# zhoubin-me/agent0

Measured on AMD Instinct MI355X. Metric: env-frames/sec (learner FPS: transitions collected and saved to replay per second with the learner running, pre-frameskip), higher is better.
Workload: dtype f32

## Files before the change

agent0_amd/csrc/conv1_wgrad.hip:

```cpp
#include "a0_internal.h"

#include <cstdint>

typedef __bf16 a0w_bf16x8 __attribute__((ext_vector_type(8)));
typedef uint32_t a0w_u32x4 __attribute__((ext_vector_type(4)));
typedef float a0w_acc4 __attribute__((ext_vector_type(4)));

constexpr int A0W_THREADS = 512;
constexpr int A0W_XP_ROW = 24, A0W_XP_PLANE = 21 * 24;
constexpr int A0W_XP_ELEMS = 64 * A0W_XP_PLANE;
constexpr int A0W_T_PITCH = 488, A0W_T_TERM = 32 * A0W_T_PITCH;
constexpr int A0W_GROUPS = 60;
constexpr int A0W_STEPS = 15;

struct a0_c1w_args {
    const uint8_t* frames; const int* slot; long long sample_stride; int chan_off;
    const float* d1;
    float* slabs;
    int B;
};

A0_D uint32_t a0w_trunc(float f) { return __float_as_uint(f) >> 16; }
A0_D float a0w_up(uint32_t h) { return __uint_as_float(h << 16); }

__global__ __launch_bounds__(A0W_THREADS) void a0_conv1_wgrad_fused_kernel(a0_c1w_args P) {
    extern __shared__ __attribute__((aligned(16))) unsigned char smem[];
    uint16_t* Xp = (uint16_t*)smem;
    uint16_t* T = Xp + A0W_XP_ELEMS;
    const int tid = threadIdx.x, lane = tid & 63;
    const int wave = __builtin_amdgcn_readfirstlane(tid >> 6);
    const int q = lane >> 4, r16 = lane & 15;
    for (int i = tid; i < (A0W_XP_ELEMS + 3 * A0W_T_TERM) / 2; i += A0W_THREADS) ((uint32_t*)smem)[i] = 0u;
    int bbase[2], bshift[2];
#pragma unroll
    for (int t = 0; t < 2; ++t) {
        const int k = (2 * wave + t) * 16 + r16;
        const int c = k >> 6, kh = (k >> 3) & 7, kw = k & 7;
        const int plane = (c * 4 + (kh & 3)) * 4 + (kw & 3);
        bbase[t] = plane * A0W_XP_PLANE + (kh >> 2) * A0W_XP_ROW;
        bshift[t] = 2 * (kw >> 2);
    }
    a0w_acc4 acc[2][2];
#pragma unroll
    for (int i = 0; i < 2; ++i)
#pragma unroll
        for (int t = 0; t < 2; ++t) acc[i][t] = a0w_acc4{0.f, 0.f, 0.f, 0.f};
    float bsum = 0.f;
    __syncthreads();
    constexpr int NDW = 4 * 84 * 21, TR = (NDW + A0W_THREADS - 1) / A0W_THREADS;
    constexpr int GT = (A0W_GROUPS + A0W_THREADS / 32 - 1) / (A0W_THREADS / 32);
    uint32_t w[TR];
    float v[GT][8];
    auto load_raw = [&](int b) {
        const long long s = P.slot ? (long long)P.slot[b] : (long long)b;
        const uint32_t* src = (const uint32_t*)(P.frames + s * P.sample_stride + P.chan_off);
#pragma unroll
        for (int j = 0; j < TR; ++j) { const int i = tid + j * A0W_THREADS; w[j] = src[i < NDW ? i : NDW - 1]; }
        const float* g = P.d1 + (long long)b * 400 * 32 + (tid & 31);
#pragma unroll
        for (int t = 0; t < GT; ++t) {
            int G = (tid >> 5) + t * (A0W_THREADS / 32);
            G = G < A0W_GROUPS ? G : A0W_GROUPS - 1;
            const int oh = G / 3, ow0 = 8 * (G - 3 * oh);
#pragma unroll
            for (int j = 0; j < 8; ++j) { const int m = oh * 20 + ow0 + j; v[t][j] = g[(m < 400 ? m : 399) * 32]; }
        }
    };
    load_raw(blockIdx.x);
    for (int b = blockIdx.x; b < P.B; b += gridDim.x) {
#pragma unroll
        for (int j = 0; j < TR; ++j) {
            int i = tid + j * A0W_THREADS;
            i = i < NDW ? i : NDW - 1;
            const int c = i / (84 * 21), rem = i - c * (84 * 21), y = rem / 21, xc = rem - y * 21;
            uint16_t* d = Xp + ((c * 4 + (y & 3)) * 4) * A0W_XP_PLANE + (y >> 2) * A0W_XP_ROW + xc;
            d[0 * A0W_XP_PLANE] = (uint16_t)(__float_as_uint((float)(w[j] & 0xffu)) >> 16);
            d[1 * A0W_XP_PLANE] = (uint16_t)(__float_as_uint((float)((w[j] >> 8) & 0xffu)) >> 16);
            d[2 * A0W_XP_PLANE] = (uint16_t)(__float_as_uint((float)((w[j] >> 16) & 0xffu)) >> 16);
            d[3 * A0W_XP_PLANE] = (uint16_t)(__float_as_uint((float)(w[j] >> 24)) >> 16);
        }
        {
            const int n = tid & 31;
#pragma unroll
            for (int t = 0; t < GT; ++t) {
                const int G = (tid >> 5) + t * (A0W_THREADS / 32);
                if (G < A0W_GROUPS) {
                    const int oh = G / 3, ow0 = 8 * (G - 3 * oh);
                    uint32_t t0[4], t1[4], t2[4];
#pragma unroll
                    for (int j = 0; j < 8; j += 2) {
                        uint32_t h[2], m[2], l[2];
#pragma unroll
                        for (int e = 0; e < 2; ++e) {
                            const float x = (ow0 + j + e < 20) ? v[t][j + e] : 0.f;
                            bsum += x;
                            h[e] = a0w_trunc(x);
                            const float r1 = x - a0w_up(h[e]);
                            m[e] = a0w_trunc(r1);
                            l[e] = a0w_trunc(r1 - a0w_up(m[e]));
                        }
                        t0[j >> 1] = h[0] | (h[1] << 16); t1[j >> 1] = m[0] | (m[1] << 16); t2[j >> 1] = l[0] | (l[1] << 16);
                    }
                    uint16_t* d = T + n * A0W_T_PITCH + 8 * G;
                    *(uint4*)(d) = uint4{t0[0], t0[1], t0[2], t0[3]};
                    *(uint4*)(d + A0W_T_TERM) = uint4{t1[0], t1[1], t1[2], t1[3]};
                    *(uint4*)(d + 2 * A0W_T_TERM) = uint4{t2[0], t2[1], t2[2], t2[3]};
                }
            }
        }
        __syncthreads();
        if (b + (int)gridDim.x < P.B) load_raw(b + gridDim.x);
        {
            const uint16_t* ap = T + r16 * A0W_T_PITCH + 8 * q;
            const uint16_t* bp0 = Xp + bbase[0] + 8 * q;
            const uint16_t* bp1 = Xp + bbase[1] + 8 * q;
#pragma unroll 3
            for (int st = 0; st < A0W_STEPS; ++st) {
                a0w_u32x4 a[2][3], bf[2];
#pragma unroll
                for (int i = 0; i < 2; ++i)
#pragma unroll
                    for (int s3 = 0; s3 < 3; ++s3) {
                        const uint4 x = *(const uint4*)(ap + s3 * A0W_T_TERM + i * 16 * A0W_T_PITCH + 32 * st);
                        a[i][s3] = a0w_u32x4{x.x, x.y, x.z, x.w};
                    }
#pragma unroll
                for (int t = 0; t < 2; ++t) {
                    const uint16_t* bp = (t == 0 ? bp0 : bp1) + 32 * st;
                    const uint4 lo = *(const uint4*)bp;
                    const uint32_t hi = *(const uint32_t*)(bp + 8);
                    const int sh = bshift[t];
                    bf[t] = a0w_u32x4{__builtin_amdgcn_alignbyte(lo.y, lo.x, sh), __builtin_amdgcn_alignbyte(lo.z, lo.y, sh),
                                      __builtin_amdgcn_alignbyte(lo.w, lo.z, sh), __builtin_amdgcn_alignbyte(hi, lo.w, sh)};
                }
#pragma unroll
                for (int s3 = 0; s3 < 3; ++s3)
#pragma unroll
                    for (int i = 0; i < 2; ++i)
#pragma unroll
                        for (int t = 0; t < 2; ++t)
                            acc[i][t] = __builtin_amdgcn_mfma_f32_16x16x32_bf16(__builtin_bit_cast(a0w_bf16x8, a[i][s3]), __builtin_bit_cast(a0w_bf16x8, bf[t]), acc[i][t], 0, 0, 0);
            }
        }
        __syncthreads();
    }
    float* out = P.slabs + (long long)blockIdx.x * (32 * 256 + 32);
#pragma unroll
    for (int i = 0; i < 2; ++i)
#pragma unroll
        for (int t = 0; t < 2; ++t) {
            const int k = (2 * wave + t) * 16 + r16;
#pragma unroll
            for (int r = 0; r < 4; ++r) out[(i * 16 + 4 * q + r) * 256 + k] = acc[i][t][r] / 255.0f;
        }
    float* red = (float*)smem;
    red[tid] = bsum;
    __syncthreads();
    if (tid < 32) {
        float s = 0.f;
#pragma unroll
        for (int j = 0; j < A0W_THREADS / 32; ++j) s += red[j * 32 + tid];
        out[32 * 256 + tid] = s;
    }
}

int a0_conv1_wgrad_fused_launch(const a0_frames_arg* f, int C, int H, int W, int B, const float* d1, float* slabs, hipStream_t st) {
    if (C != 4 || H != 84 || W != 84 || B < 1 || (f->sample_stride & 3) || (f->chan_off & 3) || (((uintptr_t)f->frames) & 3)) return 0;
    a0_c1w_args P;
    P.frames = f->frames; P.slot = f->slot; P.sample_stride = f->sample_stride; P.chan_off = f->chan_off;
    P.d1 = d1; P.slabs = slabs; P.B = B;
    const int grid = B < 256 ? B : 256;
    const size_t lds = (size_t)(A0W_XP_ELEMS + 3 * A0W_T_TERM) * 2;
    static bool configured = false;
    if (!configured) {
        A0_HIP_THROW(hipFuncSetAttribute((const void*)a0_conv1_wgrad_fused_kernel, hipFuncAttributeMaxDynamicSharedMemorySize, (int)lds));
        configured = true;
    }
    hipLaunchKernelGGL(a0_conv1_wgrad_fused_kernel, dim3(grid), dim3(A0W_THREADS), lds, st, P);
    A0_HIP_THROW(hipGetLastError());
    return grid;
}
```

agent0_amd/csrc/encoder_fused.hip:

```cpp
#include "a0_internal.h"
#include "net_tables.h"
#include "operands.h"

#include <cstdlib>
#include <type_traits>

#ifndef A0_X9_MAXORD
#define A0_X9_MAXORD 4
#endif
typedef float a0_acc4 __attribute__((ext_vector_type(4)));

struct a0_fused_args {
    const uint8_t* frames; const int* slot; long long sample_stride; int chan_off;
    const float *wt1, *wt2, *wt3;
    const float *wx2, *wx3;
    const float *b1, *b2, *b3;
    float *act1, *act2, *act3;
    int B;
    int C, H, W, H1, W1, H2, W2, H3, W3;
    int off_act1, off_act2, off_end;
    int rp1, rp2;
};

#ifndef A0_FUSED_WAVES_D
#define A0_FUSED_WAVES_D 8
#endif
constexpr int A0_FUSED_WAVES = A0_FUSED_WAVES_D;
constexpr int A0_WMG1 = A0_FUSED_WAVES / 2;
constexpr int A0_FUSED_THREADS = 64 * A0_FUSED_WAVES;
constexpr int A0_P1 = 33;
constexpr int A0_P2 = 66;

struct AF2 {
    const float* act; int RP1, W2;
    A0_D int row(int m) const { const int oh = m / W2, ow = m - oh * W2; return (2 * oh) * RP1 + 2 * ow * A0_P1; }
    A0_D int chunk_off(int c) const { const int cell = c >> 1; return (cell >> 2) * RP1 + (cell & 3) * A0_P1 + 16 * (c & 1); }
    A0_D int step_off(int s) const { return 4 * s; }
    typedef float Raw;
    A0_D Raw load(int addr) const { return act[addr]; }
    static A0_D float value(Raw r) { return r; }
};
struct AF3 {
    const float* act; int RP2, W3;
    A0_D int row(int m) const { const int oh = m / W3, ow = m - oh * W3; return oh * RP2 + ow * A0_P2; }
    A0_D int chunk_off(int c) const { const int cell = c >> 2; return (cell / 3) * RP2 + (cell % 3) * A0_P2 + 16 * (c & 3); }
    A0_D int step_off(int s) const { return 4 * s; }
    typedef float Raw;
    A0_D Raw load(int addr) const { return act[addr]; }
    static A0_D float value(Raw r) { return r; }
};

template <int N, int WN, int R>
struct a0_wring {
    static constexpr int NBW = N / 16 / WN;
    a0_f4 v[R][NBW];
    const float* base;
    const float* p;
    int nch, left;
    A0_D void init(const float* wp, int K) {
        const int lane = threadIdx.x & 63, wave = __builtin_amdgcn_readfirstlane(threadIdx.x >> 6);
        const int n = (wave % WN) * (NBW * 16) + (lane & 15), q = lane >> 4;
        base = wp + (n * 4 + q) * 4;
        nch = K >> 4;
    }
    A0_D void fill(int slot) {
#pragma unroll
        for (int j = 0; j < NBW; ++j) v[slot][j] = *(const a0_f4*)(p + j * 256);
        const bool more = left > 1;
        p += more ? N * 16 : 0;
        left -= more ? 1 : 0;
    }
    A0_D void prologue() {
        p = base; left = nch;
#pragma unroll
        for (int u = 0; u < R; ++u) fill(u);
    }
};
A0_D float a0_f4_get(const a0_f4& v, int j) { return j == 0 ? v.x : j == 1 ? v.y : j == 2 ? v.z : v.w; }

template <int OWC>
struct EpiFwd {
    static constexpr bool PER_ELEM = false;
    static constexpr bool TR = false;
    const float* bias; float* lds; int pitch, rp, ow; float* glb; int N;
    A0_D float pre_col(int n) const { return bias[n]; }
    A0_D float pre_elem(int, int) const { return 0.f; }
    A0_D void emit(int m, int n, float acc, float pre) const {
        float v = acc + pre;
        v = (v < 0.f) ? 0.f : v;
        if (lds) {
            const int w_ = OWC > 0 ? OWC : ow, oh = m / w_;
            lds[oh * rp + (m - oh * w_) * pitch + n] = v;
        }
        if (glb) glb[(unsigned)(m * N + n)] = v;
    }
    static constexpr bool ROW4 = OWC > 0 && (OWC % 4) == 0;
    A0_D void emit4(int m0, int n, const a0_acc4& acc, float pre) const {
        constexpr int OWD = OWC > 0 ? OWC : 1;
        const int oh = m0 / OWD, ow0 = m0 - oh * OWD;
        float* l = lds ? lds + oh * rp + ow0 * pitch + n : nullptr;
        const unsigned go = (unsigned)(m0 * N + n);
#pragma unroll
        for (int r = 0; r < 4; ++r) {
            float v = acc[r] + pre;
            v = (v < 0.f) ? 0.f : v;
            if (l) l[r * pitch] = v;
            if (glb) glb[go + (unsigned)(r * N)] = v;
        }
    }
};

template <int N, int WN, int MBW, class EPI>
struct a0_pre {
    static constexpr int NBW = N / 16 / WN, WMG = A0_FUSED_WAVES / WN;
    float pc[NBW][EPI::TR ? 4 : 1], pe[EPI::PER_ELEM ? MBW : 1][NBW][4];
    A0_D void load(const EPI& epi, int M) {
        const int lane = threadIdx.x & 63, wave = __builtin_amdgcn_readfirstlane(threadIdx.x >> 6);
        const int wn = wave % WN, wmg = wave / WN, q = lane >> 4, r16 = lane & 15;
#pragma unroll
        for (int j = 0; j < NBW; ++j) {
            if constexpr (EPI::TR) {
                const int n0 = (wn * NBW + j) * 16 + 4 * q;
#pragma unroll
                for (int r = 0; r < 4; ++r) pc[j][r] = epi.pre_col(n0 + r);
                if constexpr (EPI::PER_ELEM) {
#pragma unroll
                    for (int i = 0; i < MBW; ++i) {
                        const int m = (wmg + i * WMG) * 16 + r16;
                        const a0_f4 v = epi.pre_elem4(m < M ? m : M - 1, n0);
                        pe[i][j][0] = v.x; pe[i][j][1] = v.y; pe[i][j][2] = v.z; pe[i][j][3] = v.w;
                    }
                }
            } else {
                const int n = (wn * NBW + j) * 16 + r16;
                pc[j][0] = epi.pre_col(n);
                if constexpr (EPI::PER_ELEM) {
#pragma unroll
                    for (int i = 0; i < MBW; ++i)
#pragma unroll
                        for (int r = 0; r < 4; ++r) {
                            const int m = (wmg + i * WMG) * 16 + 4 * q + r;
                            pe[i][j][r] = epi.pre_elem(m < M ? m : M - 1, n);
                        }
                }
            }
        }
    }
};

template <int N, int WN, int MBW, int PD, int R, int MBWP, class AF, class EPI, class Between>
A0_D void a0_conv_stage(const AF& af, int M, int K, a0_wring<N, WN, R>& ring, const EPI& epi, const a0_pre<N, WN, MBWP, EPI>& pre, Between&& between) {
    static_assert(MBWP >= MBW, "prefetched epilogue values cover the wave's blocks");
    constexpr int NB = N / 16, NBW = NB / WN, WMG = A0_FUSED_WAVES / WN, RS = PD + 1;
// ... 198 lines not shown
        p += more ? stride : 0;
        left -= more ? 1 : 0;
    }
    A0_D void prologue() {
        p = base; left = nst;
#pragma unroll
        for (int u = 0; u < R; ++u) fill(u);
    }
};
template <int TERM>
struct AF2X {
    static constexpr int term = TERM;
    const uint16_t* planes; int RP, W2, P;
    A0_D int row(int m) const { const int oh = m / W2, ow = m - oh * W2; return (2 * oh) * RP + 2 * ow * P; }
    A0_D int step_off(int st) const { return (st >> 2) * RP + (st & 3) * P; }
};
template <int TERM>
struct AF3X {
    static constexpr int term = TERM;
    const uint16_t* planes; int RP, W3, P;
    A0_D int row(int m) const { const int oh = m / W3, ow = m - oh * W3; return oh * RP + ow * P; }
    A0_D int step_off(int st) const { const int tap = st >> 1; return (tap / 3) * RP + (tap % 3) * P + 32 * (st & 1); }
};
A0_D void a0_split4(const float (&v)[4], uint2& hi, uint2& mid, uint2& lo) {
    uint32_t h[4], m[4], l[4];
#pragma unroll
    for (int r = 0; r < 4; ++r) {
        h[r] = __float_as_uint(v[r]);
        const float r1 = v[r] - __uint_as_float(h[r] & 0xffff0000u);
        m[r] = __float_as_uint(r1);
        l[r] = __float_as_uint(r1 - __uint_as_float(m[r] & 0xffff0000u));
    }
    hi = uint2{__builtin_amdgcn_perm(h[1], h[0], 0x07060302u), __builtin_amdgcn_perm(h[3], h[2], 0x07060302u)};
    mid = uint2{__builtin_amdgcn_perm(m[1], m[0], 0x07060302u), __builtin_amdgcn_perm(m[3], m[2], 0x07060302u)};
    lo = uint2{__builtin_amdgcn_perm(l[1], l[0], 0x07060302u), __builtin_amdgcn_perm(l[3], l[2], 0x07060302u)};
}
template <int OWC, int P, int RP, int term>
struct EpiFwdX {
    static constexpr bool PER_ELEM = false;
    static constexpr bool ROW4 = false;
    static constexpr bool TR = true;
    static_assert(OWC > 0 && (P % 4) == 0 && (RP % 4) == 0 && (term % 4) == 0, "output width known at compile time; 8-byte aligned plane writes");
    const float* bias; uint16_t* planes; float* glb; int N;
    A0_D float pre_col(int) const { return 0.f; }
    A0_D void emit_n4(int m, int n0, const a0_acc4& acc, const float*) const {
        const a0_f4 bv = *(const a0_f4*)(bias + n0);
        float v[4] = {acc[0] + bv.x, acc[1] + bv.y, acc[2] + bv.z, acc[3] + bv.w};
#pragma unroll
        for (int r = 0; r < 4; ++r) v[r] = (v[r] < 0.f) ? 0.f : v[r];
        if (glb) *(a0_f4*)(glb + (unsigned)(m * N + n0)) = a0_f4{v[0], v[1], v[2], v[3]};
        uint2 hi, mid, lo;
        a0_split4(v, hi, mid, lo);
        const int oh = m / OWC;
        uint16_t* d = planes + oh * RP + (m - oh * OWC) * P + n0;
        *(uint2*)d = hi; *(uint2*)(d + term) = mid; *(uint2*)(d + 2 * term) = lo;
    }
};
struct EpiFwdT {
    static constexpr bool PER_ELEM = false;
    static constexpr bool ROW4 = false;
    static constexpr bool TR = true;
    const float* bias; float* glb; int N;
    A0_D float pre_col(int) const { return 0.f; }
    A0_D void emit_n4(int m, int n0, const a0_acc4& acc, const float*) const {
        const a0_f4 bv = *(const a0_f4*)(bias + n0);
        float v[4] = {acc[0] + bv.x, acc[1] + bv.y, acc[2] + bv.z, acc[3] + bv.w};
#pragma unroll
        for (int r = 0; r < 4; ++r) v[r] = (v[r] < 0.f) ? 0.f : v[r];
        *(a0_f4*)(glb + (unsigned)(m * N + n0)) = a0_f4{v[0], v[1], v[2], v[3]};
    }
};

template <int ORD, int N, int WN, int MBW, int R, int MBWP, class AFX, class EPI, class Between>
A0_D void a0_conv_stage_x9(const AFX& af, int M, a0_wring9<N, WN, R>& ring, const EPI& epi, const a0_pre<N, WN, MBWP, EPI>& pre, Between&& between) {
    constexpr int NB = N / 16, NBW = NB / WN, WMG = A0_FUSED_WAVES / WN;
    static_assert(NBW >= 1 && (R % 2) == 0 && MBWP >= MBW, "tile shape");
    const int tid = threadIdx.x, lane = tid & 63;
    const int wave = __builtin_amdgcn_readfirstlane(tid >> 6);
    const int wn = wave % WN, wmg = wave / WN;
    const int q = lane >> 4, r16 = lane & 15;
    const int MB = (M + 15) >> 4, NST = ring.nst;
    int rows[MBW];
#pragma unroll
    for (int i = 0; i < MBW; ++i) {
        const int m = (wmg + i * WMG) * 16 + r16;
        rows[i] = af.row(m < M ? m : 0) + 8 * q;
    }
    a0_acc4 acc[MBW][NBW];
#pragma unroll
    for (int i = 0; i < MBW; ++i)
#pragma unroll
        for (int j = 0; j < NBW; ++j) acc[i][j] = a0_acc4{0.f, 0.f, 0.f, 0.f};
    uint4 a[2][MBW][3];
    auto fetch = [&](int slot, int off) {
#pragma unroll
        for (int i = 0; i < MBW; ++i)
#pragma unroll
            for (int t = 0; t < 3; ++t) a[slot][i][t] = *(const uint4*)(af.planes + rows[i] + off + t * AFX::term);
    };
    fetch(0, af.step_off(0));
    __builtin_amdgcn_s_waitcnt(0x0F70);
#pragma unroll 1
    for (int tb = 0; tb < NST; tb += R) {
#pragma unroll
        for (int u = 0; u < R; ++u) {
            const int nxt = tb + u + 1;
            fetch((u + 1) & 1, af.step_off(nxt < NST ? nxt : NST - 1));
            __builtin_amdgcn_sched_barrier(0);
#pragma unroll
            for (int ta = 0; ta < 3; ++ta)
#pragma unroll
                for (int tw = 0; tw < 3; ++tw)
#pragma unroll
                    for (int i = 0; i < MBW; ++i)
#pragma unroll
                        for (int jn = 0; jn < NBW; ++jn) {
                            if (ta + tw > ORD) continue;
                            const a0_u32x4 av = {a[u & 1][i][ta].x, a[u & 1][i][ta].y, a[u & 1][i][ta].z, a[u & 1][i][ta].w};
                            const a0_u32x4 bv = {ring.v[u][jn][tw].x, ring.v[u][jn][tw].y, ring.v[u][jn][tw].z, ring.v[u][jn][tw].w};
                            if constexpr (EPI::TR) acc[i][jn] = __builtin_amdgcn_mfma_f32_16x16x32_bf16(__builtin_bit_cast(a0_bf16x8, bv), __builtin_bit_cast(a0_bf16x8, av), acc[i][jn], 0, 0, 0);
                            else acc[i][jn] = __builtin_amdgcn_mfma_f32_16x16x32_bf16(__builtin_bit_cast(a0_bf16x8, av), __builtin_bit_cast(a0_bf16x8, bv), acc[i][jn], 0, 0, 0);
                        }
            __builtin_amdgcn_sched_barrier(0);
            ring.fill(u);
            __builtin_amdgcn_sched_barrier(0);
        }
    }
    between();
#pragma unroll
    for (int i = 0; i < MBW; ++i) {
        const int mb = wmg + i * WMG;
        if (mb < MB) {
            if constexpr (EPI::TR) {
                const int m = mb * 16 + r16;
                if (m < M) {
#pragma unroll
                    for (int j = 0; j < NBW; ++j) epi.emit_n4(m, (wn * NBW + j) * 16 + 4 * q, acc[i][j], EPI::PER_ELEM ? pre.pe[EPI::PER_ELEM ? i : 0][j] : pre.pc[j]);
                }
            } else {
#pragma unroll
                for (int j = 0; j < NBW; ++j) {
                    const int n = (wn * NBW + j) * 16 + r16;
#pragma unroll
                    for (int r = 0; r < 4; ++r) {
                        const int m = mb * 16 + 4 * q + r;
                        if (m < M) epi.emit(m, n, acc[i][j][r], EPI::PER_ELEM ? pre.pe[EPI::PER_ELEM ? i : 0][j][r] : pre.pc[j][0]);
                    }
                }
            }
        }
    }
    __syncthreads();
}
template <int ORD, int N, int WN, int MBT, int R, int LR, class AFX, class EPI, class Between>
A0_D void a0_conv_stage_x9k(const AFX& af, int M, a0_wring9<N, WN, R, A0_FUSED_WAVES / WN>& ring, const EPI& epi, float* xch0, float* xch1, Between&& between) {
    constexpr int WK = A0_FUSED_WAVES / WN, HB0 = (MBT + 1) / 2, HB1 = MBT / 2;
    static_assert(WK == 2 && N == 16 * WN && HB1 >= 1 && EPI::TR && LR >= 1 && LR <= 16, "tile shape");
    const int tid = threadIdx.x, lane = tid & 63;
    const int wave = __builtin_amdgcn_readfirstlane(tid >> 6);
    const int wn = wave % WN, wk = wave / WN;
    const int q = lane >> 4, r16 = lane & 15;
    const int MB = (M + 15) >> 4, NSTW = ring.nst;
    int rows[MBT];
#pragma unroll
    for (int i = 0; i < MBT; ++i) {
        const int m = i * 16 + r16;
        rows[i] = af.row(m < M ? m : 0) + 8 * q;
    }
    a0_acc4 acc[MBT];
#pragma unroll
    for (int i = 0; i < MBT; ++i) acc[i] = a0_acc4{0.f, 0.f, 0.f, 0.f};
    uint4 a[2][HB0][3];
    auto fetch = [&](int slot, int h, int off) {
#pragma unroll
        for (int i = 0; i < HB0; ++i)
            if (h * HB0 + i < MBT) {
#pragma unroll
                for (int t = 0; t < 3; ++t) a[slot][i][t] = *(const uint4*)(af.planes + rows[h * HB0 + i] + off + t * AFX::term);
            }
    };
    fetch(0, 0, af.step_off(wk));
    __builtin_amdgcn_s_waitcnt(0x0F70);
#pragma unroll 1
    for (int tb = 0; tb < NSTW; tb += R) {
#pragma unroll
        for (int u = 0; u < R; ++u) {
            const int st = wk + WK * (tb + u);
            const int off = af.step_off(st), offn = af.step_off(tb + u + 1 < NSTW ? st + WK : st);
#pragma unroll
            for (int h = 0; h < 2; ++h) {
                if (h == 0) fetch(1, 1, off);
                else fetch(0, 0, offn);
                __builtin_amdgcn_sched_barrier(0);
#pragma unroll
                for (int ta = 0; ta < 3; ++ta)
#pragma unroll
                    for (int tw = 0; tw < 3; ++tw)
#pragma unroll
                        for (int i = 0; i < HB0; ++i) {
                            if (ta + tw > ORD || h * HB0 + i >= MBT) continue;
                            const a0_u32x4 av = {a[h][i][ta].x, a[h][i][ta].y, a[h][i][ta].z, a[h][i][ta].w};
                            const a0_u32x4 bv = {ring.v[u][0][tw].x, ring.v[u][0][tw].y, ring.v[u][0][tw].z, ring.v[u][0][tw].w};
                            acc[h * HB0 + i] = __builtin_amdgcn_mfma_f32_16x16x32_bf16(__builtin_bit_cast(a0_bf16x8, bv), __builtin_bit_cast(a0_bf16x8, av), acc[h * HB0 + i], 0, 0, 0);
                        }
                __builtin_amdgcn_sched_barrier(0);
            }
            ring.fill(u);
            __builtin_amdgcn_sched_barrier(0);
        }
    }
    between();
    a0_acc4* x0 = (a0_acc4*)xch0;
    a0_acc4* x1 = (a0_acc4*)xch1;
    constexpr int P1 = (HB1 - 1) * 64 + 4 * LR;
    const int last = q * LR + r16;
    const int n0 = wn * 16 + 4 * q;
    float pe[EPI::PER_ELEM ? HB0 : 1][4];
    auto send = [&](auto mine) {
        constexpr int H = decltype(mine)::value;
        if constexpr (EPI::PER_ELEM) {
#pragma unroll
            for (int i = 0; i < (H == 0 ? HB0 : HB1); ++i) {
                const int m = (H * HB0 + i) * 16 + r16;
                const a0_f4 v = epi.pre_elem4(m < M ? m : M - 1, n0);
                pe[i][0] = v.x; pe[i][1] = v.y; pe[i][2] = v.z; pe[i][3] = v.w;
            }
        }
        if constexpr (H == 1) {
#pragma unroll
            for (int i = 0; i < HB0; ++i) x0[(wn * HB0 + i) * 64 + lane] = acc[i];
        } else {
#pragma unroll
            for (int i = 0; i < HB1; ++i) {
                if (i < HB1 - 1) x1[wn * P1 + i * 64 + lane] = acc[HB0 + i];
                else if (r16 < LR) x1[wn * P1 + (HB1 - 1) * 64 + last] = acc[HB0 + i];
            }
        }
    };
    auto recv = [&](auto mine) {
        constexpr int H = decltype(mine)::value;
#pragma unroll
        for (int i = 0; i < (H == 0 ? HB0 : HB1); ++i) {
            const int mb = H * HB0 + i;
            const int m = mb * 16 + r16;
            if constexpr (H == 0) acc[mb] += x0[(wn * HB0 + i) * 64 + lane];
            else {
                if (i < HB1 - 1) acc[mb] += x1[wn * P1 + i * 64 + lane];
                else if (r16 < LR) acc[mb] += x1[wn * P1 + (HB1 - 1) * 64 + last];
            }
            if (mb < MB && m < M) epi.emit_n4(m, n0, acc[mb], EPI::PER_ELEM ? pe[EPI::PER_ELEM ? i : 0] : nullptr);
        }
    };
    if (wk == 0) send(std::integral_constant<int, 0>{});
    else send(std::integral_constant<int, 1>{});
    __syncthreads();
    if (wk == 0) recv(std::integral_constant<int, 0>{});
    else recv(std::integral_constant<int, 1>{});
    __syncthreads();
}
constexpr int A0_P1X = 40, A0_P2X = 80;
#ifndef A0_PADS
#define A0_PADS 1
#endif
constexpr int A0_RP1X = 20 * A0_P1X + (A0_PADS ? 8 : 0);
constexpr int A0_RP2X = 9 * A0_P2X + (A0_PADS ? 96 : 0);
#ifndef A0_RX2_D
#define A0_RX2_D 4
#endif
#ifndef A0_RX3_D
#define A0_RX3_D 6
#endif
[[maybe_unused]] constexpr int A0_RX2 = A0_RX2_D, A0_RX3 = A0_RX3_D;
#ifndef A0_KSPLIT_D
#define A0_KSPLIT_D 1
#endif
#ifndef A0_KSPLIT
#define A0_KSPLIT 1
#endif
#ifndef A0_WNX
#define A0_WNX 4
#endif

constexpr int A0_R1 = 4, A0_R2 = 4, A0_R3 = 6;

#ifndef A0_FUSED_MINWAVES
#define A0_FUSED_MINWAVES 1
#endif
template <int MBW1, int MBW2, int MBW3, int WC, bool X9, bool LOOP = false, int ORD = 4>
__global__ __launch_bounds__(A0_FUSED_THREADS, A0_FUSED_MINWAVES) void a0_encoder_fused_kernel(a0_fused_args P);

constexpr int A0_X9_BIAS_OFF = 2 * 4 * 84 * 84 + 3 * 20 * A0_RP1X * 2;
#ifndef A0_RK2_D
#define A0_RK2_D 2
#endif
#ifndef A0_RK3_D
#define A0_RK3_D 3
#endif
constexpr int A0_RK2 = A0_RK2_D, A0_RK3 = A0_RK3_D;
constexpr int A0_X9_XCH0 = 3 * 9 * A0_RP2X * 2;
constexpr int A0_X9_XCH1 = A0_X9_BIAS_OFF + 160 * 4;
static_assert(A0_X9_XCH0 + 4 * 3 * 1024 <= 2 * 4 * 84 * 84, "conv2 exchange region 0 fits into the image");
constexpr int A0_X9_LDS_BYTES = A0_X9_XCH1 + (A0_KSPLIT ? 4 * (2 * 64 + 4) * 16 : 0);
static_assert(A0_X9_LDS_BYTES <= 160 * 1024, "LDS");
#if A0_KSPLIT
typedef a0_wring9<64, 4, A0_RK2, 2> a0_ring2_t;
typedef a0_wring9<64, 4, A0_RK3, 2> a0_ring3_t;
#else
typedef a0_wring9<64, A0_WNX, A0_RX2> a0_ring2_t;
typedef a0_wring9<64, A0_WNX, A0_RX3> a0_ring3_t;
#endif
template <int ORD, int MBW2, int MBW3, bool LOOP>
A0_D void a0_x9_conv23(const a0_fused_args& P, int b, unsigned char* smem, float* bias_lds, a0_wring1<A0_R1>& ring1, a0_ring2_t& ring2, a0_ring3_t& ring3) {
    const int obs_bytes = P.C * P.H * P.W;
    const int M2 = P.H2 * P.W2, M3 = P.H3 * P.W3;
    uint16_t* a1p = (uint16_t*)(smem + 2 * obs_bytes);
    constexpr int term1 = 20 * A0_RP1X, term2 = 9 * A0_RP2X;
    uint16_t* a2p = (uint16_t*)smem;
    typedef EpiFwdX<9, A0_P2X, A0_RP2X, term2> E2X;
    constexpr int WNX = A0_WNX, WMGX = A0_FUSED_WAVES / WNX;
    constexpr int MBW2X = (6 + WMGX - 1) / WMGX, MBW3X = (4 + WMGX - 1) / WMGX;
    static_assert(MBW2X <= MBW2 * 2 && MBW3X <= MBW3 * 2, "84x84 geometry");
#if !A0_KSPLIT
    a0_pre<64, WNX, MBW2X, E2X> pre2;
    a0_pre<64, WNX, MBW3X, EpiFwdT> pre3;
#endif
    (void)a1p; (void)term1;
    {
        const AF2X<term1> f2{a1p, A0_RP1X, P.W2, A0_P1X};
        const E2X e2{bias_lds + 32, a2p, P.act2 ? P.act2 + (long long)b * M2 * 64 : nullptr, 64};
#if A0_KSPLIT
        const AF3X<term2> f3k{a2p, A0_RP2X, P.W3, A0_P2X};
        const EpiFwdT e3k{bias_lds + 96, P.act3 + (long long)b * M3 * 64, 64};
        a0_conv_stage_x9k<ORD, 64, 4, 6, A0_RK2, 1>(f2, M2, ring2, e2, (float*)(smem + A0_X9_XCH0), (float*)(smem + A0_X9_XCH1), [&] { ring3.prologue(); });
        a0_conv_stage_x9k<ORD, 64, 4, 4, A0_RK3, 16>(f3k, M3, ring3, e3k, (float*)a1p, (float*)a1p + 4 * 2 * 256, [&] { if (LOOP) ring1.prologue(); });
#else
        const int wmgx = __builtin_amdgcn_readfirstlane(threadIdx.x >> 6) / WNX;
        constexpr bool uneven2 = MBW2X > 1 && MBW2X * WMGX > 6, uneven3 = MBW3X > 1 && MBW3X * WMGX > 4;
        if (uneven2 && wmgx + (MBW2X - 1) * WMGX >= 6)
            a0_conv_stage_x9<ORD, 64, WNX, (MBW2X > 1 ? MBW2X - 1 : 1), A0_RX2>(f2, M2, ring2, e2, pre2, [&] { ring3.prologue(); });
        else
            a0_conv_stage_x9<ORD, 64, WNX, MBW2X, A0_RX2>(f2, M2, ring2, e2, pre2, [&] { ring3.prologue(); });
        const AF3X<term2> f3{a2p, A0_RP2X, P.W3, A0_P2X};
        const EpiFwdT e3{bias_lds + 96, P.act3 + (long long)b * M3 * 64, 64};
        if (uneven3 && wmgx + (MBW3X - 1) * WMGX >= 4)
            a0_conv_stage_x9<ORD, 64, WNX, (MBW3X > 1 ? MBW3X - 1 : 1), A0_RX3>(f3, M3, ring3, e3, pre3, [&] { if (LOOP) ring1.prologue(); });
        else
            a0_conv_stage_x9<ORD, 64, WNX, MBW3X, A0_RX3>(f3, M3, ring3, e3, pre3, [&] { if (LOOP) ring1.prologue(); });
#endif
    }
}

template <int ORD, int MBW1, int MBW2, int MBW3, bool LOOP>
A0_D void a0_encoder_fused_x9_body(const a0_fused_args& P, int bid, int nblk) {
    extern __shared__ __attribute__((aligned(16))) unsigned char smem[];
    uint16_t* img = (uint16_t*)smem;
    const int obs_bytes = P.C * P.H * P.W;
    const int M1 = P.H1 * P.W1;
    uint16_t* a1p = (uint16_t*)(smem + 2 * obs_bytes);
    constexpr int term1 = 20 * A0_RP1X;
    typedef EpiFwdX<20, A0_P1X, A0_RP1X, term1> E1X;
    constexpr int WNX = A0_WNX, WMGX = A0_FUSED_WAVES / WNX;
    constexpr int MBW2X = (6 + WMGX - 1) / WMGX, MBW3X = (4 + WMGX - 1) / WMGX;
    static_assert(MBW2X <= MBW2 * 2 && MBW3X <= MBW3 * 2, "84x84 geometry");
    a0_wring1<A0_R1> ring1;
#if A0_KSPLIT
    static_assert(WNX == 4 && A0_FUSED_WAVES == 8, "N-stationary stages: four waves along N, two along K");
#endif
    a0_ring2_t ring2;
    a0_ring3_t ring3;
    ring1.init(P.wt1, P.C);
    ring2.init(P.wx2, 512);
    ring3.init(P.wx3, 576);
    ring1.prologue();
    constexpr int MBW1X = (25 + A0_WMG1 - 1) / A0_WMG1;
    static_assert(A0_FUSED_WAVES != 8 || MBW1X == MBW1, "84x84 geometry");
    a0_pre<32, 2, MBW1X, E1X> pre1;
    float* bias_lds = (float*)(smem + A0_X9_BIAS_OFF);
    if (threadIdx.x < 160) bias_lds[threadIdx.x] = threadIdx.x < 32 ? P.b1[threadIdx.x] : threadIdx.x < 96 ? P.b2[threadIdx.x - 32] : P.b3[threadIdx.x - 96];
    for (int b = bid; b < P.B; b += nblk) {
        const long long s = P.slot ? (long long)P.slot[b] : (long long)b;
        const uint4* src = (const uint4*)(P.frames + s * P.sample_stride + P.chan_off);
        constexpr int TRIPS = 4;
        const int n16 = obs_bytes >> 4;
        for (int i0 = threadIdx.x; i0 < n16; i0 += TRIPS * A0_FUSED_THREADS) {
            uint4 v[TRIPS];
#pragma unroll
            for (int j = 0; j < TRIPS; ++j) {
                const int i = i0 + j * A0_FUSED_THREADS;
                v[j] = src[i < n16 ? i : n16 - 1];
            }
#pragma unroll
            for (int j = 0; j < TRIPS; ++j) {
                int i = i0 + j * A0_FUSED_THREADS;
                i = i < n16 ? i : n16 - 1;
                const uint32_t w[4] = {v[j].x, v[j].y, v[j].z, v[j].w};
                uint32_t o[8];
#pragma unroll
                for (int k = 0; k < 4; ++k) {
                    const uint32_t f0 = __float_as_uint((float)(w[k] & 0xffu)), f1 = __float_as_uint((float)((w[k] >> 8) & 0xffu));
                    const uint32_t f2 = __float_as_uint((float)((w[k] >> 16) & 0xffu)), f3 = __float_as_uint((float)(w[k] >> 24));
                    o[2 * k] = __builtin_amdgcn_perm(f1, f0, 0x07060302u);
                    o[2 * k + 1] = __builtin_amdgcn_perm(f3, f2, 0x07060302u);
                }
                ((uint4*)img)[2 * i] = uint4{o[0], o[1], o[2], o[3]};
                ((uint4*)img)[2 * i + 1] = uint4{o[4], o[5], o[6], o[7]};
            }
        }
        __syncthreads();
        const E1X e1{bias_lds, a1p, P.act1 ? P.act1 + (long long)b * M1 * 32 : nullptr, 32};
        const int wmg1 = __builtin_amdgcn_readfirstlane(threadIdx.x >> 6) / 2;
        if (MBW1X > 1 && wmg1 + (MBW1X - 1) * A0_WMG1 >= ((M1 + 15) >> 4))
// ... 405 lines not shown
    const float *d3, *act1, *act2;
    float *d2, *d1;
    const float *wd3, *wd2;
    int B;
};
constexpr int A0_RPDA = 11 * A0_P2X + (A0_PADS ? 96 : 0), A0_RPDB = 11 * A0_P2X + (A0_PADS ? 48 : 0);
constexpr int A0_DTERMA = 11 * A0_RPDA, A0_DTERMB = 11 * A0_RPDB;
struct AFD3X {
    static constexpr int term = A0_DTERMA;
    const uint16_t* planes;
    A0_D int row(int m) const { const int oh = m / 9, ow = m - oh * 9; return oh * A0_RPDA + ow * A0_P2X; }
    A0_D int step_off(int st) const { const int tap = st >> 1; return (tap / 3) * A0_RPDA + (tap % 3) * A0_P2X + 32 * (st & 1); }
};
struct AFD2X {
    static constexpr int term = A0_DTERMB;
    const uint16_t* planes;
    A0_D int row(int m) const { const int oh = m / 10, ow = m - oh * 10; return oh * A0_RPDB + ow * A0_P2X; }
    A0_D int step_off(int st) const { const int cell = st >> 1; return (cell >> 1) * A0_RPDB + (cell & 1) * A0_P2X + 32 * (st & 1); }
};
struct EpiBwd3X {
    static constexpr bool PER_ELEM = true;
    static constexpr bool ROW4 = false;
    static constexpr bool TR = true;
    const float* mask; float* dst; uint16_t* planes;
    A0_D float pre_col(int) const { return 0.f; }
    A0_D a0_f4 pre_elem4(int m, int n0) const { return *(const a0_f4*)(mask + (unsigned)(m * 64 + n0)); }
    A0_D void emit_n4(int m, int n0, const a0_acc4& acc, const float* pre) const {
        float v[4];
#pragma unroll
        for (int r = 0; r < 4; ++r) v[r] = pre[r] > 0.f ? acc[r] : 0.f;
        *(a0_f4*)(dst + (unsigned)(m * 64 + n0)) = a0_f4{v[0], v[1], v[2], v[3]};
        uint2 hi, mid, lo;
        a0_split4(v, hi, mid, lo);
        const int oh = m / 9, ow = m - oh * 9;
        uint16_t* d = planes + (oh + 1) * A0_RPDB + (ow + 1) * A0_P2X + n0;
        *(uint2*)d = hi; *(uint2*)(d + A0_DTERMB) = mid; *(uint2*)(d + 2 * A0_DTERMB) = lo;
    }
};
static_assert((A0_RPDB % 4) == 0 && (A0_DTERMB % 4) == 0 && (A0_P2X % 4) == 0, "8-byte aligned plane writes");
template <int OW, int S>
struct EpiBwdT {
    static constexpr bool PER_ELEM = true;
    static constexpr bool ROW4 = false;
    static constexpr bool TR = true;
    const float* mask; float* dst; int Wfull, ph, pw, N;
    A0_D unsigned gi(int m, int n) const { const int oh = m / OW, ow = m - oh * OW; return (unsigned)(((oh * S + ph) * Wfull + ow * S + pw) * N + n); }
    A0_D float pre_col(int) const { return 0.f; }
    A0_D a0_f4 pre_elem4(int m, int n0) const { return *(const a0_f4*)(mask + gi(m, n0)); }
    A0_D void emit_n4(int m, int n0, const a0_acc4& acc, const float* pre) const {
        *(a0_f4*)(dst + gi(m, n0)) = a0_f4{pre[0] > 0.f ? acc[0] : 0.f, pre[1] > 0.f ? acc[1] : 0.f, pre[2] > 0.f ? acc[2] : 0.f, pre[3] > 0.f ? acc[3] : 0.f};
    }
};
struct EpiBwdPair {
    static constexpr bool PER_ELEM = true;
    static constexpr bool ROW4 = false;
    static constexpr bool TR = true;
    const float* mask; float* dst; int p0;
    A0_D unsigned gi(int m, int n0) const {
        const int p = p0 + (n0 >> 5), oh = m / 10, ow = m - oh * 10;
        return (unsigned)(((oh * 2 + (p >> 1)) * 20 + ow * 2 + (p & 1)) * 32 + (n0 & 31));
    }
    A0_D float pre_col(int) const { return 0.f; }
    A0_D a0_f4 pre_elem4(int m, int n0) const { return *(const a0_f4*)(mask + gi(m, n0)); }
    A0_D void emit_n4(int m, int n0, const a0_acc4& acc, const float* pre) const {
        *(a0_f4*)(dst + gi(m, n0)) = a0_f4{pre[0] > 0.f ? acc[0] : 0.f, pre[1] > 0.f ? acc[1] : 0.f, pre[2] > 0.f ? acc[2] : 0.f, pre[3] > 0.f ? acc[3] : 0.f};
    }
};
constexpr int A0_RXD3 = 6, A0_RXD2 = 4;

template <int ORD>
__global__ __launch_bounds__(A0_FUSED_THREADS) void a0_encoder_dgrad_fused_x9_kernel(a0_dgrad_args P) {
    extern __shared__ __attribute__((aligned(16))) unsigned char smem[];
    uint16_t* plA = (uint16_t*)smem;
    uint16_t* plB = plA + 3 * A0_DTERMA;
    for (int i = threadIdx.x; i < 3 * (A0_DTERMA + A0_DTERMB) / 2; i += A0_FUSED_THREADS) ((uint32_t*)smem)[i] = 0u;
#if A0_KSPLIT_D
    float* const xch0 = (float*)(smem + 3 * (A0_DTERMA + A0_DTERMB) * 2);
    float* const xch1 = xch0 + 4 * 4 * 256;
    {
        const int lane = threadIdx.x & 63, wave = __builtin_amdgcn_readfirstlane(threadIdx.x >> 6), wn = wave & 3, wk = wave >> 2;
        a0_wring9<64, 4, 3, 2> ring3;
        a0_wring9<64, 4, 2, 2> ringq[2];
        ring3.init(P.wd3, 576);
        ring3.prologue();
        const uint4* const wq = (const uint4*)P.wd2 + (((wn & 1) * 16 + (lane & 15)) * 4 + (lane >> 4)) * 3 + (wn >> 1) * 3072 + wk * 384;
        __syncthreads();
        for (int b = blockIdx.x; b < P.B; b += gridDim.x) {
            const a0_f4* src = (const a0_f4*)(P.d3 + (long long)b * 49 * 64);
            for (int i = threadIdx.x; i < 49 * 16; i += A0_FUSED_THREADS) {
                const a0_f4 v = src[i];
                const int pos = i >> 4, c4 = (i & 15) * 4, h = pos / 7, w = pos - h * 7;
                const float x[4] = {v.x, v.y, v.z, v.w};
                uint2 hi, mid, lo;
                a0_split4(x, hi, mid, lo);
                uint16_t* d = plA + (h + 2) * A0_RPDA + (w + 2) * A0_P2X + c4;
                *(uint2*)(d) = hi; *(uint2*)(d + A0_DTERMA) = mid; *(uint2*)(d + 2 * A0_DTERMA) = lo;
            }
            __syncthreads();
            const AFD3X f3{plA};
            const AFD2X f2{plB};
            const EpiBwd3X e3{P.act2 + (long long)b * 81 * 64, P.d2 + (long long)b * 81 * 64, plB};
            const EpiBwdPair e2a{P.act1 + (long long)b * 400 * 32, P.d1 + (long long)b * 400 * 32, 0};
            const EpiBwdPair e2b{P.act1 + (long long)b * 400 * 32, P.d1 + (long long)b * 400 * 32, 2};
            a0_conv_stage_x9k<ORD, 64, 4, 6, 3, 1>(f3, 81, ring3, e3, xch0, xch1, [&] { ringq[0].init_at(wq, 4, 768); ringq[0].prologue(); });
            a0_conv_stage_x9k<ORD, 64, 4, 7, 2, 4>(f2, 100, ringq[0], e2a, xch0, xch1, [&] { ringq[1].init_at(wq + 2 * 3072, 4, 768); ringq[1].prologue(); });
            a0_conv_stage_x9k<ORD, 64, 4, 7, 2, 4>(f2, 100, ringq[1], e2b, xch0, xch1, [&] { ring3.prologue(); });
        }
        return;
    }
#endif
    a0_wring9<64, 4, A0_RXD3> ring3;
    a0_wring9<32, 2, A0_RXD2> ringp[2];
    ring3.init(P.wd3, 576);
    ring3.prologue();
    typedef EpiBwd3X E3;
    typedef EpiBwdT<10, 2> E2;
    a0_pre<64, 4, 3, E3> pre3;
    a0_pre<32, 2, 2, E2> prep[2];
    auto epi3 = [&](int b) { return E3{P.act2 + (long long)b * 81 * 64, P.d2 + (long long)b * 81 * 64, plB}; };
    auto epi2 = [&](int b, int ph, int pw) { return E2{P.act1 + (long long)b * 400 * 32, P.d1 + (long long)b * 400 * 32, 20, ph, pw, 32}; };
    if ((int)blockIdx.x < P.B) pre3.load(epi3(blockIdx.x), 81);
    __syncthreads();
    for (int b = blockIdx.x; b < P.B; b += gridDim.x) {
        const a0_f4* src = (const a0_f4*)(P.d3 + (long long)b * 49 * 64);
        for (int i = threadIdx.x; i < 49 * 16; i += A0_FUSED_THREADS) {
            const a0_f4 v = src[i];
            const int pos = i >> 4, c4 = (i & 15) * 4, h = pos / 7, w = pos - h * 7;
            const float x[4] = {v.x, v.y, v.z, v.w};
            uint32_t hh[4], mm[4], ll[4];
#pragma unroll
            for (int e = 0; e < 4; ++e) {
                hh[e] = __float_as_uint(x[e]);
                const float r1 = x[e] - __uint_as_float(hh[e] & 0xffff0000u);
                mm[e] = __float_as_uint(r1);
                ll[e] = __float_as_uint(r1 - __uint_as_float(mm[e] & 0xffff0000u));
            }
            uint16_t* d = plA + (h + 2) * A0_RPDA + (w + 2) * A0_P2X + c4;
            *(uint2*)(d) = uint2{__builtin_amdgcn_perm(hh[1], hh[0], 0x07060302u), __builtin_amdgcn_perm(hh[3], hh[2], 0x07060302u)};
            *(uint2*)(d + A0_DTERMA) = uint2{__builtin_amdgcn_perm(mm[1], mm[0], 0x07060302u), __builtin_amdgcn_perm(mm[3], mm[2], 0x07060302u)};
            *(uint2*)(d + 2 * A0_DTERMA) = uint2{__builtin_amdgcn_perm(ll[1], ll[0], 0x07060302u), __builtin_amdgcn_perm(ll[3], ll[2], 0x07060302u)};
        }
        __syncthreads();
        const AFD3X f3{plA};
        const AFD2X f2{plB};
        const int bn = b + gridDim.x < P.B ? b + gridDim.x : b;
        a0_conv_stage_x9<ORD, 64, 4, 3, A0_RXD3>(f3, 81, ring3, epi3(b), pre3, [&] { ringp[0].init(P.wd2, 256); ringp[0].prologue(); prep[0].load(epi2(b, 0, 0), 100); });
        a0_conv_stage_x9<ORD, 32, 2, 2, A0_RXD2>(f2, 100, ringp[0], epi2(b, 0, 0), prep[0], [&] { ringp[1].init(P.wd2 + 1 * 12288, 256); ringp[1].prologue(); prep[1].load(epi2(b, 0, 1), 100); });
        a0_conv_stage_x9<ORD, 32, 2, 2, A0_RXD2>(f2, 100, ringp[1], epi2(b, 0, 1), prep[1], [&] { ringp[0].init(P.wd2 + 2 * 12288, 256); ringp[0].prologue(); prep[0].load(epi2(b, 1, 0), 100); });
        a0_conv_stage_x9<ORD, 32, 2, 2, A0_RXD2>(f2, 100, ringp[0], epi2(b, 1, 0), prep[0], [&] { ringp[1].init(P.wd2 + 3 * 12288, 256); ringp[1].prologue(); prep[1].load(epi2(b, 1, 1), 100); });
        a0_conv_stage_x9<ORD, 32, 2, 2, A0_RXD2>(f2, 100, ringp[1], epi2(b, 1, 1), prep[1], [&] { ring3.prologue(); pre3.load(epi3(bn), 81); });
    }
}

A0_HD uint32_t a0_bf16_trunc(float f) { return __float_as_uint(f) >> 16; }
A0_HD float a0_bf16_up(uint32_t h) { return __uint_as_float(h << 16); }
__global__ void a0_conv_wt_kernel(const float* __restrict__ w1, const float* __restrict__ w2, const float* __restrict__ w3, float* __restrict__ wt, int K1,
                                  float* __restrict__ wt2, const int* __restrict__ state, int* __restrict__ commit) {
    const bool mirror = wt2 != nullptr && state[4] != 0;
    if (commit != nullptr && blockIdx.x == 0 && threadIdx.x == 0) { commit[1] = commit[5]; commit[0] = 0; }
    const int n1 = 48 * K1, n2 = 64 * 512, n3 = 64 * 576, n4 = 64 * 576, n5 = 4 * 32 * 256;
    const int n6 = 96 * 512, n7 = 96 * 576;
    int i = blockIdx.x * blockDim.x + threadIdx.x;
    float* dst = wt + i;
    if (i < n1) {
        const int pair = i & 3, f = i >> 2, s = f % 3, q = (f / 3) & 3, n = (f / 12) & 31, t = f / 384;
        uint32_t out = 0;
        for (int h = 0; h < 2; ++h) {
            const int k = 32 * t + 8 * q + 2 * pair + h;
            const float w = w1[n * K1 + k] / 255.0f;
            const uint32_t hi = a0_bf16_trunc(w);
            const float r1 = w - a0_bf16_up(hi);
            const uint32_t mid = a0_bf16_trunc(r1);
            const float r2 = r1 - a0_bf16_up(mid);
            const uint32_t lo = a0_bf16_trunc(r2);
            out |= (s == 0 ? hi : s == 1 ? mid : lo) << (16 * h);
        }
        { *(uint32_t*)dst = out; if (mirror) *(uint32_t*)(wt2 + (dst - wt)) = out; }
        return;
    }
    i -= n1;
    {
        const int j6 = i - (n2 + n3 + n4 + n5);
        if (j6 >= 0) {
            if (j6 >= n6 + n7) {
                const int j8 = j6 - (n6 + n7), n8 = 96 * 576, n9p = 48 * 256;
                if (j8 >= n8 + 4 * n9p) return;
                const bool d2 = j8 >= n8;
                const int phase = d2 ? (j8 - n8) / n9p : 0;
                const int jj = d2 ? (j8 - n8) - phase * n9p : j8, N = d2 ? 32 : 64;
                const int pair = jj & 3, f = jj >> 2, s = f % 3, q = (f / 3) & 3, n = (f / 12) % N, t = f / (12 * N);
                uint32_t out = 0;
                for (int h = 0; h < 2; ++h) {
                    const int k = 32 * t + 8 * q + 2 * pair + h, cell = k >> 6, co = k & 63;
                    float w;
                    if (!d2) { const int kh = 2 - cell / 3, kw = 2 - cell % 3; w = w3[co * 576 + (kh * 3 + kw) * 64 + n]; }
                    else { const int kh = (phase >> 1) + 2 * (1 - (cell >> 1)), kw = (phase & 1) + 2 * (1 - (cell & 1)); w = w2[co * 512 + (kh * 4 + kw) * 32 + n]; }
                    const uint32_t hi = a0_bf16_trunc(w);
                    const float r1 = w - a0_bf16_up(hi);
                    const uint32_t mid = a0_bf16_trunc(r1);
                    const uint32_t lo = a0_bf16_trunc(r1 - a0_bf16_up(mid));
                    out |= (s == 0 ? hi : s == 1 ? mid : lo) << (16 * h);
                }
                { *(uint32_t*)dst = out; if (mirror) *(uint32_t*)(wt2 + (dst - wt)) = out; }
                return;
            }
            const bool c3 = j6 >= n6;
            const int jj = c3 ? j6 - n6 : j6, K = c3 ? 576 : 512;
            const float* wsrc = c3 ? w3 : w2;
            const int pair = jj & 3, f = jj >> 2, s = f % 3, q = (f / 3) & 3, n = (f / 12) & 63, t = f / 768;
            uint32_t out = 0;
            for (int h = 0; h < 2; ++h) {
                const float w = wsrc[n * K + 32 * t + 8 * q + 2 * pair + h];
                const uint32_t hi = a0_bf16_trunc(w);
                const float r1 = w - a0_bf16_up(hi);
                const uint32_t mid = a0_bf16_trunc(r1);
                const uint32_t lo = a0_bf16_trunc(r1 - a0_bf16_up(mid));
                out |= (s == 0 ? hi : s == 1 ? mid : lo) << (16 * h);
            }
            { *(uint32_t*)dst = out; if (mirror) *(uint32_t*)(wt2 + (dst - wt)) = out; }
            return;
        }
    }
    int N, seg;
    if (i < n2) { seg = 2; N = 64; }
    else if ((i -= n2) < n3) { seg = 3; N = 64; }
    else if ((i -= n3) < n4) { seg = 4; N = 64; }
    else if ((i -= n4) < n5) { seg = 5; N = 32; }
    else return;
    const int phase = seg == 5 ? i / 8192 : 0;
    if (seg == 5) i -= phase * 8192;
    const int j = i & 3, q = (i >> 2) & 3, n = (i >> 4) % N, c = (i >> 4) / N;
    const int k = 16 * c + 4 * j + q;
    float v;
    if (seg == 2) v = w2[n * 512 + k];
    else if (seg == 3) v = w3[n * 576 + k];
    else if (seg == 4) {
        const int cell = k >> 6, co = k & 63, kh = 2 - cell / 3, kw = 2 - cell % 3;
        v = w3[co * 576 + (kh * 3 + kw) * 64 + n];
    } else {
        const int cell = k >> 6, co = k & 63, kh = (phase >> 1) + 2 * (1 - (cell >> 1)), kw = (phase & 1) + 2 * (1 - (cell & 1));
        v = w2[co * 512 + (kh * 4 + kw) * 32 + n];
    }
    *dst = v;
    if (mirror) wt2[dst - wt] = v;
}

extern "C" long long a0_net_conv_wt_floats(int C) {
    return 48LL * C * 64 + 64LL * 512 + 64LL * 576 + 64LL * 576 + 4LL * 32 * 256 + 96LL * 512 + 96LL * 576 + 96LL * 576 + 4LL * 48 * 256;
}

extern "C" int a0_net_conv_wt_refresh(const a0_encoder_weights* w, int C, float* wt, void* stream) {
    if (!w || !w->w1 || !w->w2 || !w->w3 || !wt || C < 1) return a0_fail(A0_EINVAL, "a0_net_conv_wt_refresh: bad argument");
    const long long n = a0_net_conv_wt_floats(C);
    hipLaunchKernelGGL(a0_conv_wt_kernel, dim3((unsigned)((n + 255) / 256)), dim3(256), 0, (hipStream_t)stream, w->w1, w->w2, w->w3, wt, C * 64, (float*)nullptr,
                       (const int*)nullptr, (int*)nullptr);
    return a0_fail_hip((int)hipGetLastError(), "a0_net_conv_wt_refresh");
}

extern "C" int a0_net_conv_wt_refresh_sync(const a0_encoder_weights* w, int C, float* wt, float* wt_target, const int* state, void* stream) {
    if (!w || !w->w1 || !w->w2 || !w->w3 || !wt || !wt_target || !state || C < 1) return a0_fail(A0_EINVAL, "a0_net_conv_wt_refresh_sync: bad argument");
    const long long n = a0_net_conv_wt_floats(C);
    hipLaunchKernelGGL(a0_conv_wt_kernel, dim3((unsigned)((n + 255) / 256)), dim3(256), 0, (hipStream_t)stream, w->w1, w->w2, w->w3, wt, C * 64, wt_target, state, (int*)nullptr);
    return a0_fail_hip((int)hipGetLastError(), "a0_net_conv_wt_refresh_sync");
}

int a0_conv_wt_refresh_commit(const a0_encoder_weights* w, int C, float* wt, float* wt_target, int* state, hipStream_t st) {
    if (!w || !w->w1 || !w->w2 || !w->w3) return a0_fail(A0_EINVAL, "a0_adam_step_sync_wt: encoder weights missing");
    const long long n = a0_net_conv_wt_floats(C);
    hipLaunchKernelGGL(a0_conv_wt_kernel, dim3((unsigned)((n + 255) / 256)), dim3(256), 0, st, w->w1, w->w2, w->w3, wt, C * 64, wt_target, (const int*)state, state);
    return a0_fail_hip((int)hipGetLastError(), "a0_adam_step_sync_wt");
}

static bool a0_fused_layout(int C, int H, int W, a0_fused_args& P, size_t& lds_bytes) {
    a0_net_core n;
    if (!a0_net_core_init(n, C, H, W)) return false;
    const int M1 = n.H1 * n.W1, M2 = n.H2 * n.W2, M3 = n.H3 * n.W3;
    if (M1 > 7 * 4 * 16 || M2 > 4 * 2 * 16 || M3 > 2 * 2 * 16) return false;
    if ((C * 2) % A0_R1 || (W & 3)) return false;
    const int obs_bytes = C * H * W;
    if (obs_bytes % 16) return false;
    P.C = C; P.H = H; P.W = W; P.H1 = n.H1; P.W1 = n.W1; P.H2 = n.H2; P.W2 = n.W2; P.H3 = n.H3; P.W3 = n.W3;
    P.rp1 = n.W1 * A0_P1;
    while ((P.rp1 - n.W2) & 15) ++P.rp1;
    P.rp2 = n.W2 * A0_P2;
    while ((P.rp2 - 2 * n.W3) & 31) ++P.rp2;
    P.off_act1 = obs_bytes / 2;
    P.off_act2 = P.off_act1 + ((n.H1 * P.rp1 + 3) & ~3);
    P.off_end = P.off_act2 + ((n.H2 * P.rp2 + 3) & ~3);
    lds_bytes = (size_t)P.off_end * 4;
    return lds_bytes <= 160 * 1024;
}

extern "C" int a0_net_encoder_fused_supported(int C, int H, int W) {
    a0_fused_args P; size_t lds;
    return a0_fused_layout(C, H, W, P, lds) ? 1 : 0;
}

extern "C" int a0_net_encoder_fwd_fused(int C, int H, int W, const float* wt, const a0_encoder_weights* w, const a0_frames_arg* f, int B,
                                        float* act1, float* act2, float* act3, void* stream) {
    A0_TRY
    if (!wt || !w || !w->b1 || !w->b2 || !w->b3 || !f || !f->frames || !act3 || B < 1) return a0_fail(A0_EINVAL, "a0_net_encoder_fwd_fused: bad argument");
    a0_fused_args P;
    size_t lds = 0;
    if (!a0_fused_layout(C, H, W, P, lds)) return a0_fail(A0_EINVAL, "a0_net_encoder_fwd_fused: observation shape not supported by the fused kernel");
    if ((f->sample_stride % 16) || (f->chan_off % 16) || (((uintptr_t)f->frames) % 16)) return a0_fail(A0_EINVAL, "a0_net_encoder_fwd_fused: frames must be 16-byte aligned");
    P.frames = f->frames; P.slot = f->slot; P.sample_stride = f->sample_stride; P.chan_off = f->chan_off;
    P.wt1 = wt; P.wt2 = wt + 48LL * C * 64; P.wt3 = P.wt2 + 64LL * 512;
    P.wx2 = P.wt3 + 64LL * 576 + 64LL * 576 + 4LL * 32 * 256; P.wx3 = P.wx2 + 96LL * 512;
    P.b1 = w->b1; P.b2 = w->b2; P.b3 = w->b3;
    P.act1 = act1; P.act2 = act2; P.act3 = act3; P.B = B;
    const int mb1 = (P.H1 * P.W1 + 15) / 16, mb2 = (P.H2 * P.W2 + 15) / 16, mb3 = (P.H3 * P.W3 + 15) / 16;
    const bool standard = ((mb1 + 3) / 4 == 7) && ((mb2 + 1) / 2 == 3) && ((mb3 + 1) / 2 == 2) && W == 84;
    const bool x9 = standard && H == 84 && C == 4;
    int which = x9 ? 2 : (standard ? 1 : 0);
    if (x9) lds = A0_X9_LDS_BYTES;
    static_assert(3 * 9 * A0_RP2X * 2 <= 2 * 4 * 84 * 84, "the act2 term planes fit into the dead image");
    const int gridx = (which == 2 && B > 256) ? 256 : B;
    if (which == 2 && gridx < B) which = 3;
    static size_t configured[6] = {0, 0, 0, 0, 0, 0};
    const int six = a0_x9_products_now() == 6;
    if (six && which >= 2) which += 2;
    typedef void (*a0_enc_kern)(a0_fused_args);
    const a0_enc_kern fn = which == 5 ? a0_encoder_fused_kernel<7, 3, 2, 84, true, true, 2> : which == 4 ? a0_encoder_fused_kernel<7, 3, 2, 84, true, false, 2>
                         : which == 3 ? a0_encoder_fused_kernel<7, 3, 2, 84, true, true> : which == 2 ? a0_encoder_fused_kernel<7, 3, 2, 84, true>
                         : which == 1 ? a0_encoder_fused_kernel<7, 3, 2, 84, false> : a0_encoder_fused_kernel<7, 4, 2, 0, false>;
    if (lds > configured[which]) {
        A0_HIP_THROW(hipFuncSetAttribute((const void*)fn, hipFuncAttributeMaxDynamicSharedMemorySize, (int)lds));
        configured[which] = lds;
    }
    const double per_obs = 2.0 * ((double)P.H1 * P.W1 * 32 * (P.C * 64) + (double)P.H2 * P.W2 * 64 * 512 + (double)P.H3 * P.W3 * 64 * 576);
    A0_LAUNCH_PROBED(A0_TAG_ENCODER_FUSED, per_obs * B, fn, dim3((which == 3 || which == 5) ? gridx : B), dim3(A0_FUSED_THREADS), lds, (hipStream_t)stream, P);
    A0_HIP_THROW(hipGetLastError());
    return A0_OK;
    A0_CATCH
}

extern "C" int a0_net_encoder_fwd_fused_multi(int C, int H, int W, int n, const a0_encoder_pass* pass, void* stream) {
    A0_TRY
    if (n < 1 || n > 3 || !pass) return a0_fail(A0_EINVAL, "a0_net_encoder_fwd_fused_multi: 1 to 3 passes");
    if (!(C == 4 && H == 84 && W == 84)) return a0_fail(A0_EINVAL, "a0_net_encoder_fwd_fused_multi: 4 x 84 x 84 observations on the split-operand kernel only");
    a0_fused_multi_args M;
    size_t lds = 0;
    long long total = 0;
    for (int i = 0; i < n; ++i) {
        const a0_encoder_pass& q = pass[i];
        if (!q.wt || !q.w || !q.w->b1 || !q.w->b2 || !q.w->b3 || !q.f || !q.f->frames || !q.act3 || q.B < 1) return a0_fail(A0_EINVAL, "a0_net_encoder_fwd_fused_multi: bad pass");
        if ((q.f->sample_stride % 16) || (q.f->chan_off % 16) || (((uintptr_t)q.f->frames) % 16)) return a0_fail(A0_EINVAL, "a0_net_encoder_fwd_fused_multi: frames must be 16-byte aligned");
        a0_fused_args& P = M.p[i];
        if (!a0_fused_layout(C, H, W, P, lds)) return a0_fail(A0_EINVAL, "a0_net_encoder_fwd_fused_multi: observation shape");
        P.frames = q.f->frames; P.slot = q.f->slot; P.sample_stride = q.f->sample_stride; P.chan_off = q.f->chan_off;
        P.wt1 = q.wt; P.wt2 = q.wt + 48LL * C * 64; P.wt3 = P.wt2 + 64LL * 512;
        P.wx2 = P.wt3 + 64LL * 576 + 64LL * 576 + 4LL * 32 * 256; P.wx3 = P.wx2 + 96LL * 512;
        P.b1 = q.w->b1; P.b2 = q.w->b2; P.b3 = q.w->b3;
        P.act1 = q.act1; P.act2 = q.act2; P.act3 = q.act3; P.B = q.B;
        total += q.B;
    }
    for (int i = n; i < 3; ++i) M.p[i] = M.p[0];
    int grid = (int)(total < 256 ? total : 256), used = 0;
    if (grid < n) grid = n;
    for (int i = 0; i < n; ++i) {
        M.first[i] = used;
        int share = (i == n - 1) ? grid - used : (int)((long long)grid * pass[i].B / total);
        if (share < 1) share = 1;
        if (share > pass[i].B) share = pass[i].B;
        used += share;
    }
    for (int i = n; i <= 3; ++i) M.first[i] = 0x7fffffff;
    M.first[n] = used;
    lds = A0_X9_LDS_BYTES;
    const int six = a0_x9_products_now() == 6;
    auto kern = six ? a0_encoder_fused_multi_kernel<2> : a0_encoder_fused_multi_kernel<4>;
    static bool configured[2] = {false, false};
    if (!configured[six]) {
        A0_HIP_THROW(hipFuncSetAttribute((const void*)kern, hipFuncAttributeMaxDynamicSharedMemorySize, (int)lds));
        configured[six] = true;
    }
    const a0_fused_args& P0 = M.p[0];
    const double per_obs = 2.0 * ((double)P0.H1 * P0.W1 * 32 * (P0.C * 64) + (double)P0.H2 * P0.W2 * 64 * 512 + (double)P0.H3 * P0.W3 * 64 * 576);
    A0_LAUNCH_PROBED(A0_TAG_ENCODER_FUSED, per_obs * (double)total, kern, dim3(used), dim3(A0_FUSED_THREADS), lds, (hipStream_t)stream, M);
    A0_HIP_THROW(hipGetLastError());
    return A0_OK;
    A0_CATCH
}

extern "C" int a0_net_encoder_dgrad_fused_supported(int C, int H, int W) { return (C >= 1 && H == 84 && W == 84) ? 1 : 0; }

extern "C" int a0_net_encoder_dgrad_fused(int C, int H, int W, const float* wt, const float* d3, const float* act1, const float* act2, int B, float* d2,
                                          float* d1, void* stream) {
    A0_TRY
    if (!wt || !d3 || !act1 || !act2 || !d2 || !d1 || B < 1) return a0_fail(A0_EINVAL, "a0_net_encoder_dgrad_fused: bad argument");
    if (!a0_net_encoder_dgrad_fused_supported(C, H, W)) return a0_fail(A0_EINVAL, "a0_net_encoder_dgrad_fused: 84x84 observations only");
    a0_dgrad_args P;
    P.d3 = d3; P.act1 = act1; P.act2 = act2; P.d2 = d2; P.d1 = d1; P.B = B;
    P.wd3 = wt + 48LL * C * 64 + 64LL * 512 + 64LL * 576 + 64LL * 576 + 4LL * 32 * 256 + 96LL * 512 + 96LL * 576;
    P.wd2 = P.wd3 + 96LL * 576;
    const size_t lds = (size_t)3 * (A0_DTERMA + A0_DTERMB) * 2 + (A0_KSPLIT_D ? (4 * 4 + 4 * 3) * 1024 : 0);
    static bool configured[2] = {false, false};
    const int six = a0_x9_products_now() == 6;
    auto fn = six ? a0_encoder_dgrad_fused_x9_kernel<2> : a0_encoder_dgrad_fused_x9_kernel<4>;
    if (!configured[six]) {
        A0_HIP_THROW(hipFuncSetAttribute((const void*)fn, hipFuncAttributeMaxDynamicSharedMemorySize, (int)lds));
        configured[six] = true;
    }
    const int gridx = B > 256 ? 256 : B;
    A0_LAUNCH_PROBED(A0_TAG_ENCODER_DGRAD_FUSED, 2.0 * (81.0 * 64 * 576 + 400.0 * 32 * 256) * B, fn, dim3(gridx), dim3(A0_FUSED_THREADS), lds, (hipStream_t)stream, P);
    A0_HIP_THROW(hipGetLastError());
    return A0_OK;
    A0_CATCH
}
```

agent0_amd/csrc/learner.hip:

```cpp
#include "learner_state.h"

extern "C" int a0_learner_create(const a0_learner_desc* d, a0_learner** out) { return a0_learner_create_on(d, nullptr, out); }

extern "C" int a0_learner_set_rng(a0_learner* L, int stream_id, unsigned long long offset) {
    if (!L || stream_id < 0 || stream_id > 7 || (offset & 3)) return a0_fail(A0_EINVAL, "a0_learner_set_rng: stream 0..7, offset a multiple of four");
    L->rng.off[stream_id] = offset;
    return A0_OK;
}

extern "C" int a0_learner_create_on(const a0_learner_desc* d, const a0_learner_buffers* bufs, a0_learner** out) {
    A0_TRY
    if (!d || !out) return a0_fail(A0_EINVAL, "a0_learner_create: null argument");
    const a0_learner_buffers none{};
    const a0_learner_buffers& U = bufs ? *bufs : none;
    if (U.loss_ring && U.loss_ring_cap < 1) return a0_fail(A0_EINVAL, "a0_learner_create_on: loss_ring_cap");
    if (d->A < 1 || d->B < 1 || d->n_step < 1 || !(d->discount > 0.0) || !(d->lr >= 0.0) || d->target_update_freq < 1 ||
        (d->algo != A0_ALGO_DQN && d->algo != A0_ALGO_C51 && d->algo != A0_ALGO_IQN && d->algo != A0_ALGO_FQF && d->algo != A0_ALGO_QR && d->algo != A0_ALGO_MDQN))
        return a0_fail(A0_EINVAL, "a0_learner_create: bad description");
    if (d->algo == A0_ALGO_QR && (d->num_atoms < 1 || d->num_atoms > 1024)) return a0_fail(A0_EINVAL, "a0_learner_create: qr needs 1 <= num_atoms <= 1024");
    if (d->algo == A0_ALGO_MDQN && !(d->mdqn_tau > 0.0)) return a0_fail(A0_EINVAL, "a0_learner_create: mdqn needs tau > 0");
    if (d->algo == A0_ALGO_FQF && (d->fqf_F < 2 || d->fqf_F > 32 || d->A + (d->dueling ? 1 : 0) > 32))
        return a0_fail(A0_EINVAL, "a0_learner_create: fqf needs 2 <= F <= 32, A + dueling <= 32");
    if (d->algo == A0_ALGO_IQN && (d->iqn_K < 1 || d->iqn_N < 1 || d->iqn_N_dash < 1 || d->A + (d->dueling ? 1 : 0) > 32))
        return a0_fail(A0_EINVAL, "a0_learner_create: iqn needs K, N, N' >= 1, A + dueling <= 32");
// ... 411 lines not shown
        A0_HIP_THROW(hipMemsetAsync(L->qo.dq, 0, (size_t)L->qo.R * A * 4, (hipStream_t)stream));
        A0_CHECK(a0_loss_quantile_huber(L->qo.q, (long long)N * A, A, 1, L->y, L->t_on, N, act, wgt, B, N, Nd, L->loss, L->qo.dq, L->state, stream));
    } else if (L->d.algo == A0_ALGO_C51 || L->d.algo == A0_ALGO_QR) {
        a0_encoder_pass passes[3];
        int np = 0;
        passes[np++] = a0_encoder_pass{L->wt_tg, &w_tg, &f_next, B, nullptr, nullptr, L->act3_t};
        if (dq) passes[np++] = a0_encoder_pass{L->wt_on, &w_on, &f_next, B, nullptr, nullptr, L->act3_s};
        passes[np++] = a0_encoder_pass{L->wt_on, &w_on, &f_obs, B, L->act1, L->act2, L->act3_o};
        A0_CHECK(a0_net_encoder_fwd_fused_multi(L->C, L->H, L->W, np, passes, stream));
        const int npass = dq ? 3 : 2;
        int ns_on = L->ns_on, ns_tg = L->ns_fc1, nh_on = L->nh_on, nh_tg = L->nh_tg;
        const bool grouped = a0_dense_fwd_partial_multi_ok(npass, B, 512, L->feat) && a0_dense_fwd_partial_multi_ok(npass, B, L->Npad, 512);
        if (grouped) {
            const float* Xs[3] = {L->act3_on, dq ? L->act3_s : L->act3_t, L->act3_t};
            const float* Ws[3] = {L->Wf(false), dq ? L->Wf(false) : L->Wf(true), L->Wf(true)};
            float* sl[3] = {L->fc1_on, dq ? L->fc1_on + (long long)B * 512 : L->fc1_tg, L->fc1_tg};
            const long long st[3] = {(long long)L->R_on * 512, dq ? (long long)L->R_on * 512 : (long long)B * 512, (long long)B * 512};
            A0_CHECK(a0_dense_fwd_partial_multi(npass, Xs, L->feat, Ws, B, 512, L->feat, sl, st, stream));
            ns_on = ns_tg = a0_dense_fwd_partial_multi_slabs(npass, B, 512, L->feat);
        } else {
            A0_CHECK(a0_dense_fwd_partial(L->act3_t, L->feat, L->Wf(true), B, 512, L->feat, L->fc1_tg, stream));
            A0_CHECK(a0_dense_fwd_partial(L->act3_on, L->feat, L->Wf(false), L->R_on, 512, L->feat, L->fc1_on, stream));
        }
        {
            const float* sl[2] = {L->fc1_on, L->fc1_tg};
            const long long st[2] = {(long long)L->R_on * 512, (long long)B * 512};
            const int ns[2] = {ns_on, ns_tg}, rows[2] = {L->R_on, B};
            const float* bias[2] = {L->bf(false), L->bf(true)};
            float* out[2] = {L->h_on, L->h_tg};
            A0_CHECK(a0_reduce_bias_act_multi(2, sl, st, ns, bias, out, rows, 512, 1, stream));
        }
        if (grouped) {
            const float* Xs[3] = {L->h_on, dq ? L->h_on + (long long)B * 512 : L->h_tg, L->h_tg};
            const float* Ws[3] = {L->Wh(false), dq ? L->Wh(false) : L->Wh(true), L->Wh(true)};
            float* sl[3] = {L->hs_on, dq ? L->hs_on + (long long)B * L->Npad : L->hs_tg, L->hs_tg};
            const long long st[3] = {(long long)L->R_on * L->Npad, dq ? (long long)L->R_on * L->Npad : (long long)B * L->Npad, (long long)B * L->Npad};
            A0_CHECK(a0_dense_fwd_partial_multi(npass, Xs, 512, Ws, B, L->Npad, 512, sl, st, stream));
            nh_on = nh_tg = a0_dense_fwd_partial_multi_slabs(npass, B, L->Npad, 512);
        } else {
            A0_CHECK(a0_dense_fwd_partial(L->h_on, 512, L->Wh(false), L->R_on, L->Npad, 512, L->hs_on, stream));
            A0_CHECK(a0_dense_fwd_partial(L->h_tg, 512, L->Wh(true), B, L->Npad, 512, L->hs_tg, stream));
        }
        if (L->d.algo == A0_ALGO_QR)
            A0_CHECK(a0_qr_head_loss_slabs(L->hs_on, (long long)L->R_on * L->Npad, nh_on, L->R_on, L->hs_tg, (long long)B * L->Npad, nh_tg, dq ? B : -1, L->bh(false), L->bh(true),
                                           L->Npad, A, L->T, L->d.dueling ? 1 : 0, act, rew, done, wgt, L->qr_taus, L->gamma_n, B, L->loss, L->draw, L->q_o, L->q_t, L->a_star,
                                           L->state, stream));
        else
        A0_CHECK(a0_c51_head_loss_slabs(L->hs_on, (long long)L->R_on * L->Npad, nh_on, L->R_on, L->hs_tg, (long long)B * L->Npad, nh_tg, dq ? B : -1, L->bh(false), L->bh(true),
                                        L->Npad, A, L->T, L->d.dueling ? 1 : 0, act, rew, done, wgt, L->atoms, L->gamma_n, (float)L->d.vmin, (float)L->d.vmax, B, L->loss, L->draw,
                                        L->q_o, L->q_t, L->m_proj, L->a_star, L->state, stream));
        if (a0_dense_dgrad_wgrad_ok2(B, L->Npad, 512)) {
            A0_CHECK(a0_dense_dgrad_wgrad(L->draw, L->Wh(false), L->h, 512, L->dh, L->grads + L->head.off, B, L->Npad, 512, stream));
            head_wgrad_done = true;
        } else
        A0_CHECK(a0_dense_dgrad(L->draw, L->Wh(false), L->h, L->dh, B, L->Npad, 512, stream));
    } else {
    const bool mdqn = L->d.algo == A0_ALGO_MDQN;
    a0_encoder_pass passes[3];
    int np = 0;
    passes[np++] = a0_encoder_pass{L->wt_tg, &w_tg, &f_next, B, nullptr, nullptr, L->act3_t};
    if (mdqn) passes[np++] = a0_encoder_pass{L->wt_tg, &w_tg, &f_obs, B, nullptr, nullptr, L->act3_s};
    else if (dq) passes[np++] = a0_encoder_pass{L->wt_on, &w_on, &f_next, B, nullptr, nullptr, L->act3_s};
    passes[np++] = a0_encoder_pass{L->wt_on, &w_on, &f_obs, B, L->act1, L->act2, L->act3_o};
    A0_CHECK(a0_net_encoder_fwd_fused_multi(L->C, L->H, L->W, np, passes, stream));
    int ns = L->ns_fc1;
    const bool third = mdqn || dq;
    const int n_fc1 = third ? 3 : 2;
    const float* W3 = mdqn ? L->Wf(true) : L->Wf(false);
    if (a0_dense_fwd_partial_multi_ok(n_fc1, B, 512, L->feat)) {
        const float* Xs[3] = {L->act3_o, L->act3_t, L->act3_s};
        const float* Ws[3] = {L->Wf(false), L->Wf(true), W3};
        A0_CHECK(a0_dense_fwd_partial_multi(n_fc1, Xs, L->feat, Ws, B, 512, L->feat, L->fc1_slabs, nullptr, stream));
        ns = a0_dense_fwd_partial_multi_slabs(n_fc1, B, 512, L->feat);
    } else {
        A0_CHECK(a0_dense_fwd_partial(L->act3_t, L->feat, L->Wf(true), B, 512, L->feat, L->fc1_slabs[1], stream));
        if (third) A0_CHECK(a0_dense_fwd_partial(L->act3_s, L->feat, W3, B, 512, L->feat, L->fc1_slabs[2], stream));
        A0_CHECK(a0_dense_fwd_partial(L->act3_o, L->feat, L->Wf(false), B, 512, L->feat, L->fc1_slabs[0], stream));
    }
    if (mdqn)
        A0_CHECK(a0_mdqn_head_loss_slabs(L->fc1_slabs[0], L->fc1_slabs[1], L->fc1_slabs[2], (long long)B * 512, ns, L->bf(false), L->bf(true), L->h, L->Wh(false), L->bh(false),
                                         L->Wh(true), L->bh(true), A, L->d.dueling ? 1 : 0, L->Npad, act, rew, done, wgt, L->gamma_n, (float)L->d.mdqn_tau, (float)L->d.mdqn_lo, B,
                                         L->loss, L->q_o, L->q_t, L->q_cur, L->draw, L->state, L->dh, stream));
    else
    A0_CHECK(a0_dqn_head_loss_slabs(L->fc1_slabs[0], L->fc1_slabs[1], dq ? L->fc1_slabs[2] : nullptr, (long long)B * 512, ns, L->bf(false), L->bf(true), L->h,
                                    L->Wh(false), L->bh(false), L->Wh(true), L->bh(true), A, L->d.dueling ? 1 : 0, L->Npad, act, rew, done, wgt, L->gamma_n, B,
                                    L->loss, L->q_o, L->q_t, L->draw, L->state, L->dh, stream));
    }
    const bool quantile = L->d.algo == A0_ALGO_IQN || L->d.algo == A0_ALGO_FQF;
    if (quantile) {
        const int N = L->qo.n_tau;
        const int R = (int)L->qo.R;
        A0_CHECK(a0_dueling_bwd(L->qo.dq, L->draw, L->Npad, R, A, 1, L->d.dueling ? 1 : 0, stream));
        A0_CHECK(a0_dense_dgrad(L->draw, L->Wh(false), L->qo.h, L->dh, R, L->Npad, 512, stream));
        if (a0_dense_dgrad_hadamard_ok(R, 512, L->feat, N)) {
            A0_CHECK(a0_dense_dgrad_hadamard(L->dh, L->Wf(false), L->qo.emb, L->act3_o, L->qo.demb, L->d3, R, 512, L->feat, N, stream));
        } else {
            A0_CHECK(a0_dense_dgrad(L->dh, L->Wf(false), nullptr, L->qo.dx, R, 512, L->feat, stream));
            A0_CHECK(a0_hadamard_bwd(L->qo.dx, L->qo.emb, L->act3_o, L->qo.demb, L->d3, B, N, L->feat, stream));
        }
        {
            const float* dY[3] = {L->draw, L->dh, L->qo.demb};
            const float* X[3] = {L->qo.h, L->qo.x, L->qo.cosx};
            const int ldx[3] = {512, L->feat, 64}, Rr[3] = {R, R, R}, Nn[3] = {L->Npad, 512, L->feat}, Kk[3] = {512, L->feat, 64};
            float* G[3] = {L->grads + L->head.off, L->grads + L->fc1.off, L->grads + L->cos.off};
            A0_CHECK(a0_dense_wgrad_multi(3, dY, X, ldx, G, Rr, Nn, Kk, L->slabs, L->slab_off3, pp, stream));
        }
    }
    if (!quantile) {
        const float* dY[2] = {L->draw, L->dh};
        const float* X[2] = {L->h, L->act3_o};
        const int ldx[2] = {512, L->feat}, R[2] = {B, B}, N[2] = {L->Npad, 512}, K[2] = {512, L->feat};
        float* G[2] = {L->grads + L->head.off, L->grads + L->fc1.off};
        if (head_wgrad_done) {
            if (a0_dense_dgrad_wgrad_ok(B, 512, L->feat)) {
                A0_CHECK(a0_dense_dgrad_wgrad(L->dh, L->Wf(false), L->act3_o, L->feat, L->d3, G[1], B, 512, L->feat, stream));
            } else {
                A0_CHECK(a0_dense_dgrad(L->dh, L->Wf(false), L->act3_o, L->d3, B, 512, L->feat, stream));
                A0_CHECK(a0_dense_wgrad_multi(1, dY + 1, X + 1, ldx + 1, G + 1, R + 1, N + 1, K + 1, L->slabs, L->slab_off + 1, pp, stream));
            }
        } else if (a0_dense_dgrad_wgrad2_ok(B, 512, L->feat, L->Npad, 512)) {
            A0_CHECK(a0_dense_dgrad_wgrad2(L->dh, L->Wf(false), L->act3_o, L->feat, L->d3, G[1], B, 512, L->feat, L->draw, L->h, 512, G[0], L->Npad, 512, stream));
        } else if (a0_dense_dgrad_wgrad_ok(B, 512, L->feat)) {
            A0_CHECK(a0_dense_dgrad_wgrad(L->dh, L->Wf(false), L->act3_o, L->feat, L->d3, G[1], B, 512, L->feat, stream));
            A0_CHECK(a0_dense_wgrad_multi(1, dY, X, ldx, G, R, N, K, L->slabs, L->slab_off, pp, stream));
        } else {
            A0_CHECK(a0_dense_dgrad(L->dh, L->Wf(false), L->act3_o, L->d3, B, 512, L->feat, stream));
            A0_CHECK(a0_dense_wgrad_multi(2, dY, X, ldx, G, R, N, K, L->slabs, L->slab_off, pp, stream));
        }
    }
    auto sigma_grads = [&]() -> int {
        const float *gmu[3], *nin[3], *nw[3], *nb[3];
        float* gs[3];
        int N[3], K[3], r0[3], r1[3];
        for (int k = 0; k < L->n_mods; ++k) {
            const a0_noise_mod& m = L->mods[k];
            const Blk &bm = m.block ? L->head : L->fc1, &bs = m.block ? L->head_sigma : L->fc1_sigma;
            gmu[k] = L->grads + bm.off; gs[k] = L->grads + bs.off; N[k] = bm.N; K[k] = bm.K; r0[k] = m.r0; r1[k] = m.r1;
            nin[k] = L->noise + m.off_in; nw[k] = L->noise + m.off_w; nb[k] = L->noise + m.off_b;
        }
        return a0_noisy_multi(1, L->n_mods, gmu, nullptr, gs, N, K, r0, r1, nin, nw, nb, stream);
    };
    const long long conv_end = L->fc1.off;
    if (dp) {
        if (L->d.noisy) A0_CHECK(sigma_grads());
        A0_CHECK(a0_nan_flag_export(L->state, L->grads + L->n_pad, stream));
        if (dp_inline) {
            A0_CHECK(a0_dp_allreduce(L->dp_comm, L->grads + conv_end, L->n_pad + 1 - conv_end, stream));
        } else {
            A0_HIP_THROW(hipEventRecord(L->dp_ev[0], (hipStream_t)stream));
            A0_HIP_THROW(hipStreamWaitEvent(L->dp_side, L->dp_ev[0], 0));
            A0_CHECK(a0_dp_allreduce(L->dp_comm, L->grads + conv_end, L->n_pad + 1 - conv_end, L->dp_side));
        }
    }
    A0_CHECK(a0_net_encoder_dgrad_fused(L->C, L->H, L->W, L->wt_on, L->d3, L->act1, L->act2, B, L->d2, L->d1, stream));
    A0_CHECK(a0_net_encoder_wgrad(L->net, &w_on, &f_obs, B, L->act1, L->act2, L->d3, L->d2, L->d1, L->grads + L->conv1.off, L->grads + L->conv2.off, L->grads + L->conv3.off,
                                  L->slabs + L->enc_slab_off, &pend, stream));
    if (dp) {
        if (dp_inline) {
            A0_CHECK(a0_dp_allreduce(L->dp_comm, L->grads, conv_end, stream));
        } else {
            A0_HIP_THROW(hipEventRecord(L->dp_ev[1], (hipStream_t)stream));
            A0_HIP_THROW(hipStreamWaitEvent(L->dp_side, L->dp_ev[1], 0));
            A0_CHECK(a0_dp_allreduce(L->dp_comm, L->grads, conv_end, L->dp_side));
            A0_HIP_THROW(hipEventRecord(L->dp_ev[2], L->dp_side));
            A0_HIP_THROW(hipStreamWaitEvent((hipStream_t)stream, L->dp_ev[2], 0));
        }
    } else if (L->d.noisy) {
        A0_CHECK(sigma_grads());
    }
    if (loss_out) A0_HIP_THROW(hipMemcpyAsync(loss_out, L->loss, (size_t)B * 4, hipMemcpyDeviceToDevice, (hipStream_t)stream));
    if (L->d.algo == A0_ALGO_FQF)
        A0_CHECK(a0_rmsprop_step(on + L->frac.off, L->grads + L->frac.off, L->rms_sq, L->frac.size(), L->d.lr / 2e4, 0.95, 1e-5, L->d.max_grad_norm > 0.0 ? L->d.max_grad_norm : -1.0, L->clip, stream));
    const double eps = L->d.adam_eps > 0.0 ? L->d.adam_eps : 1e-2 / (double)B;
    A0_CHECK(a0_adam_step_sync_wt(on, L->grads, L->m, L->v, L->n_adam, L->state, L->scalars, L->d.lr, 0.9, 0.999, eps, L->d.target_update_freq, tg, L->n_pad, dp ? L->grads + L->n_pad : nullptr, &w_on, L->C,
                                  L->wt_on, L->wt_tg, L->loss, B, L->loss_ring, L->loss_ring_cap, stream));
    return A0_OK;
    A0_CATCH
}
```

agent0_amd/csrc/net.hip:

```cpp
#include "igemm_x9.h"
#include "short_k_fwd.h"
#include "a0_internal.h"
#include "net_impl.h"

#include <vector>

__global__ __launch_bounds__(256) void a0_reduce_slabs_kernel(const float* __restrict__ slabs, long long slab_stride, int nslab,
                                                               float* __restrict__ out, long long count) {
    __shared__ float red[8][33];
    const int c = threadIdx.x & 31, g = threadIdx.x >> 5;
    const long long i = (long long)blockIdx.x * 32 + c;
    float s = 0.f;
    if (i < count)
        for (int z = g; z < nslab; z += 8) s += slabs[(long long)z * slab_stride + i];
    red[g][c] = s;
    __syncthreads();
    if (g == 0 && i < count) {
        float t = 0.f;
#pragma unroll
        for (int j = 0; j < 8; ++j) t += red[j][c];
        out[i] = t;
    }
}

// ... 641 lines not shown
    EpiSlab::Params ep{scratch, (long long)E * 512, 512};
    bk.tag = A0_TAG_DENSE_FWD;
    a0_fc1_partial_launch(bk, a, bw, ep, E, 512, K, splits);
    a0_qenv_args P;
    P.slabs = scratch; P.slab_stride = (long long)E * 512; P.nslab = splits; P.b1 = b1; P.W2 = W2; P.b2 = b2; P.A = A; P.dueling = dueling; P.E = E;
    P.rng_seed = seed; P.stream_a = stream_a; P.stream_u = stream_u; P.off_a = off_a; P.off_u = off_u; P.eps = eps; P.ctrl = ctrl; P.eps_ptr = eps_ptr;
    P.action = action; P.qmax = qmax;
    P.env_seed = env_seed; P.rank = rank; P.g = g; P.obs_in = obs_in; P.obs_out = obs_out; P.ep_ret = ep_ret; P.final_mask = final_mask; P.final_ret = final_ret;
    P.n = n; P.steps = steps; P.gamma = gamma; P.ring_act = ring_act; P.ring_rew = ring_rew; P.ring_done = ring_done; P.obs0 = obs0; P.frames = frames;
    P.cap = cap; P.start = start_slot % cap; P.r_act = r_act; P.r_rew = r_rew; P.r_done = r_done; P.task = task;
    return a0_actor_step_enc_launch(P, wt, w, act3_next, (hipStream_t)stream);
    A0_CATCH
}

__global__ __launch_bounds__(256) void a0_mean_rows_kernel(const float* __restrict__ x, int E, float* __restrict__ out) {
    __shared__ float red[256];
    const float* p = x + (long long)blockIdx.x * E;
    float s = 0.f;
    for (int e = threadIdx.x; e < E; e += 256) s += p[e];
    red[threadIdx.x] = s;
    __syncthreads();
    for (int o = 128; o > 0; o >>= 1) { if ((int)threadIdx.x < o) red[threadIdx.x] += red[threadIdx.x + o]; __syncthreads(); }
    if (threadIdx.x == 0) out[blockIdx.x] = red[0] / (float)E;
}

extern "C" int a0_mean_rows(const float* x, int T, int E, float* out, void* stream) {
    if (!x || !out || T < 1 || E < 1) return a0_fail(A0_EINVAL, "a0_mean_rows: bad argument");
    hipLaunchKernelGGL(a0_mean_rows_kernel, dim3(T), dim3(256), 0, (hipStream_t)stream, x, E, out);
    return a0_fail_hip((int)hipGetLastError(), "a0_mean_rows");
}

extern "C" int a0_dense_dgrad(const float* dY, const float* W, const float* act_mask, float* dX, int R, int N, int K, void* stream) {
    A0_TRY
    if (!dY || !W || !dX || R < 1 || (N & 3) || (K & 3)) return a0_fail(A0_EINVAL, "a0_dense_dgrad: bad shape");
    a0_hip_backend bk{(hipStream_t)stream};
    a0_dense_dgrad_impl(bk, dY, W, act_mask, dX, R, N, K);
    return A0_OK;
    A0_CATCH
}

extern "C" int a0_dense_dgrad_hadamard_ok(int R, int N, int K, int n) {
    return (g_gemm_x9 != 0 && (n == 32 || n == 64) && R >= 4096 && !(R & 255) && !(R % n) && !(N & 15) && N >= 64 && !(K & 3) && K >= 128) ? 1 : 0;
}
extern "C" int a0_dense_dgrad_hadamard(const float* dY, const float* W, const float* emb, const float* feat, float* demb, float* d3, int R, int N, int K, int n, void* stream) {
    A0_TRY
    if (!dY || !W || !emb || !feat || !demb || !d3 || !a0_dense_dgrad_hadamard_ok(R, N, K, n)) return a0_fail(A0_EINVAL, "a0_dense_dgrad_hadamard: shapes a0_dense_dgrad_hadamard_ok accepts");
    const a0_mat_src a{dY, N};
    const a0_mat_src bw{W, K};
    const EpiHadamard::Params e{emb, feat, demb, d3, K, n};
    hipEvent_t e0 = nullptr, e1 = nullptr;
    const bool probe = a0_probe_events(A0_TAG_DENSE_DGRAD, &e0, &e1);
    A0_HIP_THROW((a0_igemm_x9_launch<OpMatKC, OpMatXC, EpiHadamard, 4, 2, 2, 2, 1>((hipStream_t)stream, a, bw, e, R, K, N, 1, e0, e1)));
    if (probe) a0_probe_commit(2.0 * (double)R * (double)N * (double)K);
    return A0_OK;
    A0_CATCH
}

extern "C" int a0_dense_dgrad_wgrad_ok(int R, int N, int K) {
    const long long b128 = (long long)((R + 127) / 128) * ((K + 63) / 64), b64 = (long long)((N + 63) / 64) * ((K + 63) / 64);
    return (g_gemm_x9 != 0 && g_probe.tag == 0 && R == N && R >= 1 && R <= 1024 && !(N & 3) && !(K & 3) && b128 < 256 && b64 >= 256 && N >= 512 &&
            (long long)((R + 127) / 128) * ((K + 127) / 128) < A0_X9_BIG_TILES) ? 1 : 0;
}
static int a0_dense_dgrad_wgrad_small_ok(int R, int N, int K) {
    const long long t1 = (long long)((R + 63) / 64) * ((K + 63) / 64), t2 = (long long)((N + 63) / 64) * ((K + 63) / 64);
    return (g_gemm_x9 != 0 && g_probe.tag == 0 && R >= 64 && R <= 1024 && N >= 64 && !(N & 3) && !(K & 3) && t1 + t2 <= 256 && t2 >= 16) ? 1 : 0;
}
extern "C" int a0_dense_dgrad_wgrad_ok2(int R, int N, int K) { return (a0_dense_dgrad_wgrad_ok(R, N, K) || a0_dense_dgrad_wgrad_small_ok(R, N, K)) ? 1 : 0; }
extern "C" int a0_dense_dgrad_wgrad(const float* dY, const float* W, const float* X, int ldx, float* dX, float* grad, int R, int N, int K, void* stream) {
    A0_TRY
    if (!dY || !W || !X || !dX || !grad || ldx < K || (ldx & 3) || !a0_dense_dgrad_wgrad_ok2(R, N, K)) return a0_fail(A0_EINVAL, "a0_dense_dgrad_wgrad: shapes a0_dense_dgrad_wgrad_ok2 accepts");
    a0_mat_src a1{dY, N}, b1{W, K};
    EpiMaskMat::Params e1{dX, X, K};
    a0_mat_src a2{dY, N}, b2{X, ldx};
    EpiWgradSlab::Params e2{grad, 0, K, (long long)N * K};
    if (!a0_dense_dgrad_wgrad_ok(R, N, K)) {
        A0_HIP_THROW((a0_igemm_x9_pair_launch<OpMatKC, OpMatXC, EpiMaskMat, OpMatXC, OpMatXC, EpiWgradSlab, 2, 2, 1, 1>((hipStream_t)stream, a1, b1, e1, R, K, N, a2, b2, e2, N, K, R)));
        return A0_OK;
    }
    A0_HIP_THROW((a0_igemm_x9_pair_launch<OpMatKC, OpMatXC, EpiMaskMat, OpMatXC, OpMatXC, EpiWgradSlab, 4, 2, 1, 1>((hipStream_t)stream, a1, b1, e1, R, K, N, a2, b2, e2, N, K, R)));
    return A0_OK;
    A0_CATCH
}

extern "C" int a0_dense_dgrad_wgrad2_ok(int R, int N, int K, int N2, int K2) {
    return (a0_dense_dgrad_wgrad_ok(R, N, K) && N2 >= 4 && !(N2 & 3) && K2 >= 4 && !(K2 & 3) &&
            (long long)((N2 + 127) / 128) * ((K2 + 63) / 64) <= 8) ? 1 : 0;
}
extern "C" int a0_dense_dgrad_wgrad2(const float* dY, const float* W, const float* X, int ldx, float* dX, float* grad, int R, int N, int K,
                                     const float* dY2, const float* X2, int ldx2, float* grad2, int N2, int K2, void* stream) {
    A0_TRY
    if (!dY || !W || !X || !dX || !grad || ldx < K || (ldx & 3) || !a0_dense_dgrad_wgrad_ok(R, N, K)) return a0_fail(A0_EINVAL, "a0_dense_dgrad_wgrad2: shapes a0_dense_dgrad_wgrad_ok accepts");
    if (!dY2 || !X2 || !grad2 || N2 < 4 || (N2 & 3) || K2 < 4 || (K2 & 3) || ldx2 < K2 || (ldx2 & 3) ||
        (long long)((N2 + 127) / 128) * ((K2 + 63) / 64) > (long long)((R + 127) / 128) * ((K + 63) / 64))
        return a0_fail(A0_EINVAL, "a0_dense_dgrad_wgrad2: the second layer's weight gradient must have no more 128 x 64 tiles than the first layer's data gradient");
    a0_mat_src a1{dY, N}, b1{W, K};
    EpiMaskMat::Params e1{dX, X, K};
    a0_mat_src a2{dY, N}, b2{X, ldx};
    EpiWgradSlab::Params e2{grad, 0, K, (long long)N * K};
    a0_mat_src a3{dY2, N2}, b3{X2, ldx2};
    EpiWgradSlab::Params e3{grad2, 0, K2, (long long)N2 * K2};
    A0_HIP_THROW((a0_igemm_x9_trio_launch<OpMatKC, OpMatXC, EpiMaskMat, OpMatXC, OpMatXC, EpiWgradSlab, 4, 2, 1, 1>((hipStream_t)stream, a1, b1, e1, R, K, N, a2, b2, e2, N, K, R,
                                                                                                                  a3, b3, e3, N2, K2, R)));
    return A0_OK;
    A0_CATCH
}

extern "C" long long a0_dense_wgrad_scratch(int R, int N, int K) { return a0_dense_wgrad_scratch_impl(R, N, K); }

extern "C" int a0_dense_wgrad(const float* dY, const float* X, int ldx, float* grad, int R, int N, int K, float* slabs, void* stream) {
    A0_TRY
    if (!dY || !X || !grad || R < 1 || (N & 3) || (K & 3) || (ldx & 3)) return a0_fail(A0_EINVAL, "a0_dense_wgrad: bad shape");
    if (a0_dense_wgrad_scratch_impl(R, N, K) > 0 && !slabs) return a0_fail(A0_EINVAL, "a0_dense_wgrad: needs slab scratch");
    a0_hip_backend bk{(hipStream_t)stream};
    a0_dense_wgrad_impl(bk, dY, X, ldx, grad, R, N, K, slabs);
    return A0_OK;
    A0_CATCH
}

extern "C" int a0_dense_wgrad_multi(int n, const float* const* dY, const float* const* X, const int* ldx, float* const* grad, const int* R, const int* N, const int* K,
                                    float* slabs, const long long* slab_off, a0_pending_reduce* pend, void* stream) {
    A0_TRY
    if (n < 1 || n > 4 || !dY || !X || !ldx || !grad || !R || !N || !K || !slab_off) return a0_fail(A0_EINVAL, "a0_dense_wgrad_multi: 1..4 layers");
    a0_hip_backend bk{(hipStream_t)stream};
    a0_reduce_seg segs[4];
    int nseg = 0;
    for (int i = 0; i < n; ++i) {
        if (!dY[i] || !X[i] || !grad[i] || R[i] < 1 || (N[i] & 3) || (K[i] & 3) || (ldx[i] & 3)) return a0_fail(A0_EINVAL, "a0_dense_wgrad_multi: bad shape");
        if (a0_dense_wgrad_scratch_impl(R[i], N[i], K[i]) > 0 && !slabs) return a0_fail(A0_EINVAL, "a0_dense_wgrad_multi: needs slab scratch");
        a0_reduce_seg seg;
        a0_dense_wgrad_impl(bk, dY[i], X[i], ldx[i], grad[i], R[i], N[i], K[i], slabs ? slabs + slab_off[i] : nullptr, &seg);
        if (seg.nslab > 0) segs[nseg++] = seg;
    }
    if (pend) {
        if (pend->n < 0 || pend->n + nseg > 4) return a0_fail(A0_EINVAL, "a0_dense_wgrad_multi: more than four pending reductions");
        for (int k = 0; k < nseg; ++k) pend->seg[pend->n++] = segs[k];
    } else if (nseg > 0) bk.reduce_segments(segs, nseg);
    return A0_OK;
    A0_CATCH
}

extern "C" int a0_net_encoder_wgrad(const a0_net* n, const a0_encoder_weights* w, const a0_frames_arg* f, int B, const float* act1, const float* act2,
                                    const float* d3, const float* d2, const float* d1, float* g1, float* g2, float* g3, float* slabs, const a0_pending_reduce* pend,
                                    void* stream) {
    A0_TRY
    if (!n || !w || !f || !f->frames || !act1 || !act2 || !d3 || !d2 || !d1 || !g1 || !g2 || !g3 || B < 1) return a0_fail(A0_EINVAL, "a0_net_encoder_wgrad: null argument");
    if (a0_encoder_bwd_scratch_impl(n->core, B) > 0 && !slabs) return a0_fail(A0_EINVAL, "a0_net_encoder_wgrad: needs slab scratch");
    if (pend && (pend->n < 0 || pend->n > 4)) return a0_fail(A0_EINVAL, "a0_net_encoder_wgrad: bad pending reductions");
    a0_hip_backend bk{(hipStream_t)stream};
    a0_encoder_bwd_impl(bk, n->core, *w, *f, B, act1, act2, d3, const_cast<float*>(d2), const_cast<float*>(d1), g1, g2, g3, slabs, false, pend);
    return A0_OK;
    A0_CATCH
}

extern "C" long long a0_net_encoder_bwd_scratch(const a0_net* n, int B) { return n ? a0_encoder_bwd_scratch_impl(n->core, B) : 0; }

extern "C" int a0_net_encoder_bwd(const a0_net* n, const a0_encoder_weights* w, const a0_frames_arg* f, int B,
                                  const float* act1, const float* act2, const float* d3, float* d2, float* d1,
                                  float* g1, float* g2, float* g3, float* slabs, void* stream) {
    A0_TRY
    if (!n || !w || !f || !f->frames || !act1 || !act2 || !d3 || !d2 || !d1 || !g1 || !g2 || !g3 || B < 1) return a0_fail(A0_EINVAL, "a0_net_encoder_bwd: null argument");
    if (a0_encoder_bwd_scratch_impl(n->core, B) > 0 && !slabs) return a0_fail(A0_EINVAL, "a0_net_encoder_bwd: needs slab scratch");
    a0_hip_backend bk{(hipStream_t)stream};
    a0_encoder_bwd_impl(bk, n->core, *w, *f, B, act1, act2, d3, d2, d1, g1, g2, g3, slabs);
    return A0_OK;
    A0_CATCH
}
```

agent0_amd/csrc/net_impl.h:

```cpp
#pragma once
#include <cstdlib>
#include "net_tables.h"
#include "operands.h"
#include "../../include/agent0_hip.h"

enum { A0_TAG_NONE = 0, A0_TAG_CONV1_FWD = 1, A0_TAG_CONV2_FWD = 2, A0_TAG_CONV3_FWD = 3, A0_TAG_DENSE_FWD = 4, A0_TAG_DENSE_DGRAD = 5,
       A0_TAG_DENSE_WGRAD = 6, A0_TAG_CONV3_WGRAD = 7, A0_TAG_CONV3_DGRAD = 8, A0_TAG_CONV2_WGRAD = 9, A0_TAG_CONV2_DGRAD = 10, A0_TAG_CONV1_WGRAD = 11 };


struct EpiWgradSlab {
    static constexpr bool ROWSUM_A = true;
    struct Params { float* out; long long slab_stride; int ld; long long bias_off; };
    A0_HD static void store_rowsum(const Params& P, int x, float v, int z) { P.out[(long long)z * P.slab_stride + P.bias_off + x] = v; }
    A0_HD static void store(const Params& P, int x, int y, float v, int z) {
        P.out[(long long)z * P.slab_stride + (long long)x * P.ld + y] = v;
    }
};

static inline a0_frames_src a0_frames(const a0_net_core& n, const a0_frames_arg& f) {
    a0_frames_src s;
    s.frames = f.frames; s.slot = f.slot;
    s.g.Hin = n.H; s.g.Win = n.W; s.g.C = n.C;
    s.g.Hout = n.H1; s.g.Wout = n.W1; s.g.stride = 4; s.g.pad = 0; s.g.HWout = n.H1 * n.W1;
    s.g.hw_magic = a0_udiv_magic((unsigned)s.g.HWout); s.g.w_magic = a0_udiv_magic((unsigned)s.g.Wout);
// ... 70 lines not shown
    return K <= 64 && N >= 256 && R >= 4096;
}
static inline int a0_dense_wgrad_splits(int R, int N, int K) {
    if (a0_wgrad_narrow_deep(R, N, K)) {
        const int tiles = ((N + 63) / 64) * ((K + 63) / 64);
        int sp = 512 / tiles;
        const int maxs = R / 512;
        if (sp > maxs) sp = maxs;
        if (sp > 32) sp = 32;
        return sp < 1 ? 1 : sp;
    }
    const int deep = a0_wgrad_splits_deep(N, K, R);
    return deep > 0 ? deep : a0_wgrad_splits((N + 63) / 64, (K + 127) / 128, R);
}

static inline long long a0_dense_wgrad_scratch_impl(int R, int N, int K) {
    int s = a0_dense_wgrad_splits(R, N, K);
    return s > 1 ? (long long)s * ((long long)N * K + N) : 0;
}

static inline bool a0_c23w_plan(const a0_net_core& n, int B, int* G2, int* G3) {
    const int gmax = ((2 * 256) / 7) / 8 * 8;
    if (B < 1 || n.H1 != 20 || n.W1 != 20 || n.H2 != 9 || n.W2 != 9 || n.H3 != 7 || n.W3 != 7) return false;
    const int g = B < gmax ? B : gmax;
    *G2 = g; *G3 = g;
    return g >= 1;
}

struct a0_enc_slab_plan { long long off[3], total; int splits[3]; };

static inline a0_enc_slab_plan a0_encoder_slab_plan(const a0_net_core& n, int B) {
    a0_enc_slab_plan p;
    const int M[3] = {B * n.H1 * n.W1, B * n.H2 * n.W2, B * n.H3 * n.W3};
    const int N[3] = {32, 64, 64};
    const int K[3] = {n.K1, n.K2, n.K3};
    long long off = 0;
    int g23[3] = {0, 0, 0};
    if (!a0_c23w_plan(n, B, &g23[1], &g23[2])) g23[1] = g23[2] = 0;
    for (int l = 2; l >= 0; --l) {
        p.splits[l] = l == 0 ? a0_wgrad_splits(1, (K[l] + 127) / 128, M[l]) : a0_conv_wgrad_splits(K[l], M[l]);
        int slabs = p.splits[l] > 1 ? p.splits[l] : 0;
        if (l == 0) { const int fused = B < 256 ? B : 256; if (fused > slabs) slabs = fused; }
        else if (g23[l] > slabs) slabs = g23[l];
        p.off[l] = off;
        off += (long long)slabs * ((long long)N[l] * K[l] + N[l]);
    }
    p.total = off;
    return p;
}

static inline long long a0_encoder_bwd_scratch_impl(const a0_net_core& n, int B) { return a0_encoder_slab_plan(n, B).total; }

template <class BK>
static void a0_encoder_fwd_impl(BK& bk, const a0_net_core& n, const a0_encoder_weights& w, const a0_frames_arg& f, int B,
                                float* act1, float* act2, float* act3) {
    {
        a0_frames_src a = a0_frames(n, f);
        a0_mat_src b{w.w1, n.K1};
        EpiBiasAct::Params e{act1, w.b1, 32, 1};
        bk.tag = A0_TAG_CONV1_FWD;
        bk.template igemm<OpFramesKC, OpMatKC, EpiBiasAct, 4, 1, 1, 1>(a, b, e, B * n.H1 * n.W1, 32, n.K1, 1);
    }
    {
        a0_act_src a = a0_act(act1, n.H1, n.W1, 32, n.H2, n.W2, 2, 0, n.ktab2);
        a0_mat_src b{w.w2, n.K2};
        EpiBiasAct::Params e{act2, w.b2, 64, 1};
        bk.tag = A0_TAG_CONV2_FWD;
        bk.template igemm<OpActKC, OpMatKC, EpiBiasAct, 4, 1, 1, 2>(a, b, e, B * n.H2 * n.W2, 64, n.K2, 1);
    }
    {
        a0_act_src a = a0_act(act2, n.H2, n.W2, 64, n.H3, n.W3, 1, 0, n.ktab3);
        a0_mat_src b{w.w3, n.K3};
        EpiBiasAct::Params e{act3, w.b3, 64, 1};
        const int M = B * n.H3 * n.W3;
        bk.tag = A0_TAG_CONV3_FWD;
        if (M <= 128 * 160)
            bk.template igemm<OpActKC, OpMatKC, EpiBiasAct, 2, 2, 1, 1>(a, b, e, M, 64, n.K3, 1);
        else
            bk.template igemm<OpActKC, OpMatKC, EpiBiasAct, 4, 1, 1, 2>(a, b, e, M, 64, n.K3, 1);
    }
}

static inline bool a0_short_k_shape(int R, int N, int K, int ldx) {
    return K == 64 && (ldx & 3) == 0 && ldx >= 64 && N >= 64 && R >= 256;
}

template <class BK>
static void a0_dense_fwd_impl(BK& bk, const float* X, int ldx, const float* W, const float* b, float* Y, int R, int N, int K,
                              int relu, float* scratch, int splits_in = 0) {
    bk.tag = A0_TAG_DENSE_FWD;
    if (splits_in <= 1 && a0_short_k_shape(R, N, K, ldx)) { bk.short_k_fwd(X, ldx, W, b, nullptr, 1, Y, nullptr, R, N, relu); return; }
    a0_mat_src a{X, ldx};
    a0_mat_src bw{W, K};
    const int splits = splits_in > 0 ? splits_in : a0_fwd_splits((R + 127) / 128, (N + 63) / 64, K);
    const bool narrow = (N <= 32);
    bk.tag = A0_TAG_DENSE_FWD;
    if (splits == 1) {
        EpiBiasAct::Params e{Y, b, N, relu};
        if (narrow) bk.template igemm<OpMatKC, OpMatKC, EpiBiasAct, 4, 1, 1, 1>(a, bw, e, R, N, K, 1);
        else bk.template igemm<OpMatKC, OpMatKC, EpiBiasAct, 4, 1, 1, 2>(a, bw, e, R, N, K, 1);
    } else {
        EpiSlab::Params e{scratch, (long long)R * N, N};
        if (narrow) bk.template igemm<OpMatKC, OpMatKC, EpiSlab, 4, 1, 1, 1>(a, bw, e, R, N, K, splits);
        else bk.template igemm<OpMatKC, OpMatKC, EpiSlab, 4, 1, 1, 2>(a, bw, e, R, N, K, splits);
        bk.reduce_bias_act(scratch, (long long)R * N, splits, b, Y, R, N, relu);
    }
}

template <class BK>
static void a0_dense_dgrad_impl(BK& bk, const float* dY, const float* W, const float* act_mask, float* dX, int R, int N, int K) {
    a0_mat_src a{dY, N};
    a0_mat_src bw{W, K};
    bk.tag = A0_TAG_DENSE_DGRAD;
    if (act_mask) {
        EpiMaskMat::Params e{dX, act_mask, K};
        const long long blocks = (long long)((R + 127) / 128) * ((K + 63) / 64);
        if (blocks < 256) bk.template igemm<OpMatKC, OpMatXC, EpiMaskMat, 2, 2, 1, 1>(a, bw, e, R, K, N, 1);
        else bk.template igemm<OpMatKC, OpMatXC, EpiMaskMat, 4, 1, 1, 2>(a, bw, e, R, K, N, 1);
    } else {
        EpiSlab::Params e{dX, 0, K};
        bk.template igemm<OpMatKC, OpMatXC, EpiSlab, 4, 1, 1, 2>(a, bw, e, R, K, N, 1);
    }
}

template <class BK>
static void a0_finish_wgrad(BK& bk, int N, long long wcount, float* grad, float* slabs, int splits) {
    if (splits > 1) bk.reduce_slabs(slabs, wcount + N, splits, grad, wcount + N);
}

template <class BK>
static void a0_dense_wgrad_impl(BK& bk, const float* dY, const float* X, int ldx, float* grad, int R, int N, int K, float* slabs, a0_reduce_seg* defer = nullptr) {
    const long long wcount = (long long)N * K;
    a0_mat_src a{dY, N};
    a0_mat_src b{X, ldx};
    bk.tag = A0_TAG_DENSE_WGRAD;
    if (defer) *defer = a0_reduce_seg{nullptr, 0, 0, nullptr, 0};
    const long long blocks64 = (long long)((N + 63) / 64) * ((K + 63) / 64);
    if (blocks64 >= 256 && R <= 1024) {
        EpiWgradSlab::Params e{grad, 0, K, wcount};
        bk.template igemm<OpMatXC, OpMatXC, EpiWgradSlab, 2, 2, 1, 1>(a, b, e, N, K, R, 1);
        return;
    }
    const int splits = a0_dense_wgrad_splits(R, N, K);
    EpiWgradSlab::Params e{splits > 1 ? slabs : grad, splits > 1 ? wcount + N : 0, K, wcount};
    if (a0_wgrad_narrow_deep(R, N, K)) bk.template igemm<OpMatXC, OpMatXC, EpiWgradSlab, 2, 2, 1, 1>(a, b, e, N, K, R, splits);
    else bk.template igemm<OpMatXC, OpMatXC, EpiWgradSlab, 2, 2, 1, 2>(a, b, e, N, K, R, splits);
    if (defer && splits > 1) *defer = a0_reduce_seg{slabs, wcount + N, splits, grad, wcount + N};
    else a0_finish_wgrad(bk, N, wcount, grad, slabs, splits);
}

template <class BK>
static void a0_encoder_bwd_impl(BK& bk, const a0_net_core& n, const a0_encoder_weights& w, const a0_frames_arg& f, int B,
                                const float* act1, const float* act2, const float* d3, float* d2, float* d1,
                                float* g1, float* g2, float* g3, float* slabs, bool with_dgrad = true, const a0_pending_reduce* pend = nullptr) {
    const int M3 = B * n.H3 * n.W3, M2 = B * n.H2 * n.W2, M1 = B * n.H1 * n.W1;
    const a0_enc_slab_plan plan = a0_encoder_slab_plan(n, B);
    a0_reduce_seg segs[8];
    int nseg = 0;
    if (pend) for (int k = 0; k < pend->n && k < 4; ++k) segs[nseg++] = pend->seg[k];
    int G2 = 0, G3 = 0;
    const bool fused23 = !with_dgrad && a0_c23w_plan(n, B, &G2, &G3) &&
                         bk.conv23_wgrad_fused(n, B, act1, act2, d2, d3, slabs + plan.off[1], slabs + plan.off[2]);
    if (fused23) {
        segs[nseg++] = a0_reduce_seg{slabs + plan.off[2], 64LL * n.K3 + 64, G3, g3, 64LL * n.K3 + 64};
        segs[nseg++] = a0_reduce_seg{slabs + plan.off[1], 64LL * n.K2 + 64, G2, g2, 64LL * n.K2 + 64};
    }
    if (!fused23) {
        const int splits = plan.splits[2];
        const long long wc = 64LL * n.K3;
        float* sl = slabs + plan.off[2];
        a0_mat_src a{d3, 64};
        a0_act_src b = a0_act(act2, n.H2, n.W2, 64, n.H3, n.W3, 1, 0, n.ktab3);
        EpiWgradSlab::Params e{splits > 1 ? sl : g3, splits > 1 ? wc + 64 : 0, n.K3, wc};
        bk.tag = A0_TAG_CONV3_WGRAD;
        bk.template igemm<OpMatXC, OpActXC, EpiWgradSlab, 2, 2, 1, 1>(a, b, e, 64, n.K3, M3, splits);
        if (splits > 1) segs[nseg++] = a0_reduce_seg{sl, wc + 64, splits, g3, wc + 64};
    }
    if (with_dgrad) {
        a0_act_src a = a0_act(d3, n.H3, n.W3, 64, n.H2, n.W2, 1, 2, n.ktab_d3);
        a0_wtab_src b{w.w3, n.wtab_d3};
        EpiDgrad::Params e{d2, act2, n.H2 * n.W2, n.W2, n.H2, n.W2, 64, 1, 0, 0, (long long)n.H2 * n.W2 * 64};
        bk.tag = A0_TAG_CONV3_DGRAD;
        bk.template igemm<OpActKC, OpWtabXC, EpiDgrad, 4, 1, 1, 2>(a, b, e, M2, 64, 9 * 64, 1);
    }
    if (!fused23) {
        const int splits = plan.splits[1];
        const long long wc = 64LL * n.K2;
        float* sl = slabs + plan.off[1];
        a0_mat_src a{d2, 64};
        a0_act_src b = a0_act(act1, n.H1, n.W1, 32, n.H2, n.W2, 2, 0, n.ktab2);
        EpiWgradSlab::Params e{splits > 1 ? sl : g2, splits > 1 ? wc + 64 : 0, n.K2, wc};
        bk.tag = A0_TAG_CONV2_WGRAD;
        bk.template igemm<OpMatXC, OpActXC, EpiWgradSlab, 2, 2, 1, 1>(a, b, e, 64, n.K2, M2, splits);
        if (splits > 1) segs[nseg++] = a0_reduce_seg{sl, wc + 64, splits, g2, wc + 64};
    }
    for (int ph = 0; ph < 2 && with_dgrad; ++ph)
        for (int pw = 0; pw < 2; ++pw) {
            const int Hv = (n.H1 - ph + 1) / 2, Wv = (n.W1 - pw + 1) / 2;
            if (Hv < 1 || Wv < 1) continue;
            a0_act_src a = a0_act(d2, n.H2, n.W2, 64, Hv, Wv, 1, 1, n.ktab_d2);
            a0_wtab_src b{w.w2, n.wtab_d2[ph * 2 + pw]};
            EpiDgrad::Params e{d1, act1, Hv * Wv, Wv, n.H1, n.W1, 32, 2, ph, pw, (long long)n.H1 * n.W1 * 32};
            bk.tag = A0_TAG_CONV2_DGRAD;
            bk.template igemm<OpActKC, OpWtabXC, EpiDgrad, 4, 1, 1, 1>(a, b, e, B * Hv * Wv, 32, 4 * 64, 1);
        }
    {
        const long long wc = 32LL * n.K1;
        float* sl = slabs + plan.off[0];
        bk.tag = A0_TAG_CONV1_WGRAD;
        const int fused_slabs = bk.conv1_wgrad_fused(n, f, B, d1, sl);
        if (fused_slabs > 0) {
            segs[nseg++] = a0_reduce_seg{sl, wc + 32, fused_slabs, g1, wc + 32};
        } else {
            const int splits = plan.splits[0];
            a0_mat_src a{d1, 32};
            a0_frames_src b = a0_frames(n, f);
            EpiWgradSlab::Params e{splits > 1 ? sl : g1, splits > 1 ? wc + 32 : 0, n.K1, wc};
            bk.template igemm<OpMatXC, OpFramesXC, EpiWgradSlab, 1, 4, 1, 1>(a, b, e, 32, n.K1, M1, splits);
            if (splits > 1) segs[nseg++] = a0_reduce_seg{sl, wc + 32, splits, g1, wc + 32};
        }
    }
    if (nseg > 0) bk.reduce_segments(segs, nseg);
}
```

agent0_amd/ops.py:

```python
from __future__ import annotations

import ctypes as C
from typing import Optional

import torch

from . import _abi
from ._abi import A0Error, EncoderPass, EncoderWeights, FramesArg, LearnerDesc, NetDesc, check


def _stream() -> int:
    return torch._C._cuda_getCurrentRawStream(torch._C._cuda_getDevice())


def _req(t: Optional[torch.Tensor], dtype, min_numel: int, name: str, optional: bool = False):
    if t is None:
        if optional:
            return None
        raise A0Error(f"{name}: tensor required")
    if not t.is_cuda:
        raise A0Error(f"{name}: expected a HIP device tensor (got {t.device}); agent0_amd has no CPU path")
    if t.dtype != dtype:
        raise A0Error(f"{name}: expected {dtype}, got {t.dtype}")
    if not t.is_contiguous():
# ... 51 lines not shown
    def set_params(self, online, target=None):
        check(self.lib.a0_learner_set_params(self.h, _req(online, torch.float32, self.n, "online"), _req(target, torch.float32, self.n, "target", optional=True), _stream()),
              "a0_learner_set_params")

    def get(self):
        dev = torch.device("cuda", torch.cuda.current_device())
        on, tg, m, v = (torch.empty(self.n, device=dev) for _ in range(4))
        st = torch.zeros(8, dtype=torch.int32, device=dev)
        check(self.lib.a0_learner_get(self.h, on.data_ptr(), tg.data_ptr(), m.data_ptr(), v.data_ptr(), st.data_ptr(), _stream()), "a0_learner_get")
        return on, tg, m, v, st

    def update(self, frames, slot, row_bytes, act, rew, done, wgt, loss_out=None):
        B = self.B
        check(self.lib.a0_learner_update(self.h, _req(frames, torch.uint8, row_bytes, "frames"), _req(slot, torch.int32, B, "slot", optional=True), int(row_bytes),
                                         _req(act, torch.int32, B, "act"), _req(rew, torch.float32, B, "rew"), _req(done, torch.float32, B, "done"), _req(wgt, torch.float32, B, "wgt"),
                                         _req(loss_out, torch.float32, B, "loss_out", optional=True), _stream()), "a0_learner_update")

    def close(self):
        if self.h is not None:
            self.lib.a0_learner_destroy(self.h)
            self.h = None

    def __del__(self):
        try:
            self.close()
        except Exception:
            pass


class _TraceRange:
    def __init__(self, lib, name: bytes):
        self.lib, self.name = lib, name

    def __enter__(self):
        self.lib.a0_trace_push(self.name)

    def __exit__(self, *exc):
        self.lib.a0_trace_pop()
        return False


class _NoRange:
    def __enter__(self):
        return None

    def __exit__(self, *exc):
        return False


_NO_RANGE = _NoRange()


class HipOps:
    name = "hip"

    def __init__(self):
        if not torch.cuda.is_available():
            raise A0Error("agent0_amd needs an AMD GPU visible to PyTorch-ROCm (torch.cuda.is_available() is False)")
        self.lib = _abi.load()
        self.device = torch.device("cuda", torch.cuda.current_device())

    def empty(self, *shape, dtype=torch.float32):
        return torch.empty(*shape, dtype=dtype, device=self.device)

    def zeros(self, *shape, dtype=torch.float32):
        return torch.zeros(*shape, dtype=dtype, device=self.device)

    def net(self, C_, H, W) -> Net:
        return Net(self.lib, C_, H, W)

    def native_learner(self, **kw) -> NativeLearner:
        return NativeLearner(self.lib, **kw)

    def _frames(self, net, frames, slot, sample_stride, chan_off, B):
        hw = net.H * net.W
        need_rows = B if slot is None else 1
        fp = _req(frames, torch.uint8, need_rows * sample_stride if slot is None else chan_off + net.C * hw, "frames")
        if chan_off + net.C * hw > sample_stride:
            raise A0Error("frames: chan_off + C*H*W exceeds sample_stride")
        sp = _req(slot, torch.int32, B, "slot", optional=True)
        return FramesArg(fp, sp, sample_stride, chan_off)

    @staticmethod
    def _enc_w(w):
        return EncoderWeights(*[w[k].data_ptr() for k in ("w1", "b1", "w2", "b2", "w3", "b3")])

    def encoder_fwd(self, net, w, frames, slot, sample_stride, chan_off, B, act1, act2, act3):
        fa = self._frames(net, frames, slot, sample_stride, chan_off, B)
        ew = self._enc_w(w)
        a1 = _req(act1, torch.float32, B * net.H1 * net.W1 * 32, "act1")
        a2 = _req(act2, torch.float32, B * net.H2 * net.W2 * 64, "act2")
        a3 = _req(act3, torch.float32, B * net.feat, "act3")
        check(self.lib.a0_net_encoder_fwd(net.h, C.addressof(ew), C.addressof(fa), B, a1, a2, a3, _stream()), "a0_net_encoder_fwd")

    def fused_supported(self, C_, H, W) -> bool:
        return bool(self.lib.a0_net_encoder_fused_supported(C_, H, W))

    def conv_wt_floats(self, C_) -> int:
        return int(self.lib.a0_net_conv_wt_floats(C_))

    def conv_wt_refresh(self, w, C_, wt):
        ew = self._enc_w(w)
        check(self.lib.a0_net_conv_wt_refresh(C.addressof(ew), C_, _req(wt, torch.float32, self.conv_wt_floats(C_), "wt"), _stream()), "a0_net_conv_wt_refresh")

    def conv_wt_refresh_sync(self, w, C_, wt, wt_target, state):
        ew = self._enc_w(w)
        n = self.conv_wt_floats(C_)
        check(self.lib.a0_net_conv_wt_refresh_sync(C.addressof(ew), C_, _req(wt, torch.float32, n, "wt"), _req(wt_target, torch.float32, n, "wt_target"),
                                                   _req(state, torch.int32, 8, "state"), _stream()), "a0_net_conv_wt_refresh_sync")

    def encoder_fwd_fused(self, net, wt, w, frames, slot, sample_stride, chan_off, B, act1, act2, act3):
        fa = self._frames(net, frames, slot, sample_stride, chan_off, B)
        ew = self._enc_w(w)
        check(self.lib.a0_net_encoder_fwd_fused(net.C, net.H, net.W, _req(wt, torch.float32, self.conv_wt_floats(net.C), "wt"), C.addressof(ew), C.addressof(fa), B,
                                                _req(act1, torch.float32, B * net.H1 * net.W1 * 32, "act1", optional=True),
                                                _req(act2, torch.float32, B * net.H2 * net.W2 * 64, "act2", optional=True),
                                                _req(act3, torch.float32, B * net.feat, "act3"), _stream()), "a0_net_encoder_fwd_fused")

    def encoder_fwd_fused_multi(self, net, passes):
        keep = []
        arr = (EncoderPass * len(passes))()
        for i, (wt, w, frames, slot, sample_stride, chan_off, B, act1, act2, act3) in enumerate(passes):
            fa, ew = self._frames(net, frames, slot, sample_stride, chan_off, B), self._enc_w(w)
            keep += [fa, ew]
            arr[i] = EncoderPass(_req(wt, torch.float32, self.conv_wt_floats(net.C), "wt"), C.addressof(ew), C.addressof(fa), B,
                                 _req(act1, torch.float32, B * net.H1 * net.W1 * 32, "act1", optional=True), _req(act2, torch.float32, B * net.H2 * net.W2 * 64, "act2", optional=True),
                                 _req(act3, torch.float32, B * net.feat, "act3"))
        check(self.lib.a0_net_encoder_fwd_fused_multi(net.C, net.H, net.W, len(passes), C.addressof(arr), _stream()), "a0_net_encoder_fwd_fused_multi")

    def encoder_bwd_scratch(self, net, B) -> int:
        return int(self.lib.a0_net_encoder_bwd_scratch(net.h, B))

    def encoder_bwd(self, net, w, frames, slot, sample_stride, chan_off, B, act1, act2, d3, d2, d1, g1, g2, g3, slabs):
        fa = self._frames(net, frames, slot, sample_stride, chan_off, B)
        ew = self._enc_w(w)
        need = self.encoder_bwd_scratch(net, B)
        check(self.lib.a0_net_encoder_bwd(
            net.h, C.addressof(ew), C.addressof(fa), B,
            _req(act1, torch.float32, B * net.H1 * net.W1 * 32, "act1"), _req(act2, torch.float32, B * net.H2 * net.W2 * 64, "act2"),
            _req(d3, torch.float32, B * net.feat, "d3"), _req(d2, torch.float32, B * net.H2 * net.W2 * 64, "d2"),
            _req(d1, torch.float32, B * net.H1 * net.W1 * 32, "d1"),
            _req(g1, torch.float32, 32 * net.K1 + 32, "g1"), _req(g2, torch.float32, 64 * net.K2 + 64, "g2"), _req(g3, torch.float32, 64 * net.K3 + 64, "g3"),
            _req(slabs, torch.float32, need, "slabs", optional=(need == 0)), _stream()), "a0_net_encoder_bwd")

    def dgrad_fused_supported(self, C_, H, W) -> bool:
        return bool(self.lib.a0_net_encoder_dgrad_fused_supported(C_, H, W))

    def encoder_dgrad_fused(self, net, wt, d3, act1, act2, B, d2, d1):
        check(self.lib.a0_net_encoder_dgrad_fused(net.C, net.H, net.W, _req(wt, torch.float32, self.conv_wt_floats(net.C), "wt"),
                                                  _req(d3, torch.float32, B * net.feat, "d3"), _req(act1, torch.float32, B * net.H1 * net.W1 * 32, "act1"),
                                                  _req(act2, torch.float32, B * net.H2 * net.W2 * 64, "act2"), B,
                                                  _req(d2, torch.float32, B * net.H2 * net.W2 * 64, "d2"), _req(d1, torch.float32, B * net.H1 * net.W1 * 32, "d1"),
                                                  _stream()), "a0_net_encoder_dgrad_fused")

    def pending_reduce(self):
        from ._abi import PendingReduce
        p = PendingReduce()
        p.n = 0
        return p

    def encoder_wgrad(self, net, w, frames, slot, sample_stride, chan_off, B, act1, act2, d3, d2, d1, g1, g2, g3, slabs, pend=None):
        fa = self._frames(net, frames, slot, sample_stride, chan_off, B)
        ew = self._enc_w(w)
        need = self.encoder_bwd_scratch(net, B)
        check(self.lib.a0_net_encoder_wgrad(
            net.h, C.addressof(ew), C.addressof(fa), B,
            _req(act1, torch.float32, B * net.H1 * net.W1 * 32, "act1"), _req(act2, torch.float32, B * net.H2 * net.W2 * 64, "act2"),
            _req(d3, torch.float32, B * net.feat, "d3"), _req(d2, torch.float32, B * net.H2 * net.W2 * 64, "d2"),
            _req(d1, torch.float32, B * net.H1 * net.W1 * 32, "d1"),
            _req(g1, torch.float32, 32 * net.K1 + 32, "g1"), _req(g2, torch.float32, 64 * net.K2 + 64, "g2"), _req(g3, torch.float32, 64 * net.K3 + 64, "g3"),
            _req(slabs, torch.float32, need, "slabs", optional=(need == 0)), None if pend is None else C.addressof(pend), _stream()), "a0_net_encoder_wgrad")

    def dense_fwd_scratch(self, R, N, K) -> int:
        return int(self.lib.a0_dense_fwd_scratch(R, N, K))

    def dense_wgrad_scratch(self, R, N, K) -> int:
        return int(self.lib.a0_dense_wgrad_scratch(R, N, K))

    def dense_fwd(self, X, ldx, W, b, Y, R, N, K, relu, scratch):
        need = self.dense_fwd_scratch(R, N, K)
        check(self.lib.a0_dense_fwd(_req(X, torch.float32, (R - 1) * ldx + K, "X"), ldx, _req(W, torch.float32, N * K, "W"), _req(b, torch.float32, N, "b"),
                                    _req(Y, torch.float32, R * N, "Y"), R, N, K, int(relu),
                                    _req(scratch, torch.float32, need, "scratch", optional=(need == 0)), _stream()), "a0_dense_fwd")

    def dense_fwd_splits(self, R, N, K) -> int:
        return int(self.lib.a0_dense_fwd_splits(R, N, K))

    def dense_fwd_n(self, X, ldx, W, b, Y, R, N, K, relu, splits, scratch):
        need = splits * R * N if splits > 1 else 0
        check(self.lib.a0_dense_fwd_n(_req(X, torch.float32, (R - 1) * ldx + K, "X"), ldx, _req(W, torch.float32, N * K, "W"), _req(b, torch.float32, N, "b"),
                                      _req(Y, torch.float32, R * N, "Y"), R, N, K, int(relu), int(splits),
                                      _req(scratch, torch.float32, need, "scratch", optional=(need == 0)), _stream()), "a0_dense_fwd_n")

    def dense_dgrad_hadamard_ok(self, R, N, K, n) -> bool:
        return bool(self.lib.a0_dense_dgrad_hadamard_ok(R, N, K, n))

    def dense_dgrad_hadamard(self, dY, W, emb, feat, demb, d3, R, N, K, n):
        check(self.lib.a0_dense_dgrad_hadamard(_req(dY, torch.float32, R * N, "dY"), _req(W, torch.float32, N * K, "W"), _req(emb, torch.float32, R * K, "emb"),
                                               _req(feat, torch.float32, (R // n) * K, "feat"), _req(demb, torch.float32, R * K, "demb"), _req(d3, torch.float32, (R // n) * K, "d3"),
                                               R, N, K, n, _stream()), "a0_dense_dgrad_hadamard")

    def weight_planes_words(self, N, K) -> int:
        return int(self.lib.a0_weight_planes_words(N, K))

    def split_planes(self, W, planes, N, K):
        check(self.lib.a0_split_planes(_req(W, torch.float32, N * K, "W"), _req(planes, torch.int32, self.weight_planes_words(N, K), "planes"), N, K, _stream()), "a0_split_planes")

    def dense_fwd_wplanes_ok(self, R, N, K) -> bool:
        return bool(self.lib.a0_dense_fwd_wplanes_ok(R, N, K))

    def dense_fwd_wplanes(self, X, ldx, planes, b, Y, R, N, K, relu):
        check(self.lib.a0_dense_fwd_wplanes(_req(X, torch.float32, (R - 1) * ldx + K, "X"), ldx, _req(planes, torch.int32, self.weight_planes_words(N, K), "planes"),
                                            _req(b, torch.float32, N, "b"), _req(Y, torch.float32, R * N, "Y"), R, N, K, int(relu), _stream()), "a0_dense_fwd_wplanes")

    def dense_fwd_mul(self, X, ldx, W, b, M, group, Y, R, N, K, relu):
        check(self.lib.a0_dense_fwd_mul(_req(X, torch.float32, (R - 1) * ldx + K, "X"), ldx, _req(W, torch.float32, N * K, "W"), _req(b, torch.float32, N, "b"),
                                        _req(M, torch.float32, ((R - 1) // group + 1) * N, "M"), group, _req(Y, torch.float32, R * N, "Y"), R, N, K, int(relu), _stream()),
              "a0_dense_fwd_mul")

    def dense_fwd_mul_keep_ok(self, R, N, K, ldx) -> bool:
        return bool(self.lib.a0_dense_fwd_mul_keep_ok(R, N, K, ldx))

    def dense_fwd_mul_keep(self, X, ldx, W, b, M, group, E, Y, R, N, K, relu):
        check(self.lib.a0_dense_fwd_mul_keep(_req(X, torch.float32, (R - 1) * ldx + K, "X"), ldx, _req(W, torch.float32, N * K, "W"), _req(b, torch.float32, N, "b"),
                                             _req(M, torch.float32, ((R - 1) // group + 1) * N, "M"), group, _req(E, torch.float32, R * N, "E"),
                                             _req(Y, torch.float32, R * N, "Y"), R, N, K, int(relu), _stream()), "a0_dense_fwd_mul_keep")

    def dense_dgrad(self, dY, W, mask, dX, R, N, K):
        check(self.lib.a0_dense_dgrad(_req(dY, torch.float32, R * N, "dY"), _req(W, torch.float32, N * K, "W"),
                                      _req(mask, torch.float32, R * K, "mask", optional=True), _req(dX, torch.float32, R * K, "dX"), R, N, K, _stream()), "a0_dense_dgrad")

    def dense_wgrad(self, dY, X, ldx, grad, R, N, K, slabs):
        need = self.dense_wgrad_scratch(R, N, K)
        check(self.lib.a0_dense_wgrad(_req(dY, torch.float32, R * N, "dY"), _req(X, torch.float32, (R - 1) * ldx + K, "X"), ldx,
                                      _req(grad, torch.float32, N * K + N, "grad"), R, N, K,
                                      _req(slabs, torch.float32, need, "slabs", optional=(need == 0)), _stream()), "a0_dense_wgrad")

    def dueling_fwd(self, raw, ld, q, R, A, T, dueling):
        check(self.lib.a0_dueling_fwd(_req(raw, torch.float32, R * ld, "raw"), ld, _req(q, torch.float32, R * A * T, "q"), R, A, T, int(dueling), _stream()), "a0_dueling_fwd")

    def dueling_bwd(self, dq, draw, ld, R, A, T, dueling):
        check(self.lib.a0_dueling_bwd(_req(dq, torch.float32, R * A * T, "dq"), _req(draw, torch.float32, R * ld, "draw"), ld, R, A, T, int(dueling), _stream()), "a0_dueling_bwd")

    def select_action(self, x, sb, sa, st, B, A, T, mode, aux, a_star, qsel, qmax):
        span = (B - 1) * sb + (A - 1) * sa + (T - 1) * st + 1
        check(self.lib.a0_select_action(_req(x, torch.float32, span, "x"), sb, sa, st, B, A, T, mode,
                                        _req(aux, torch.float32, T if mode == 2 else (B * (T + 1) if mode == 3 else 0), "aux", optional=mode < 2),
                                        _req(a_star, torch.int32, B, "a_star", optional=True), _req(qsel, torch.float32, B * A, "qsel", optional=True),
                                        _req(qmax, torch.float32, B, "qmax", optional=True), _stream()), "a0_select_action")

    def loss_dqn(self, q, q_next, A, act, a_star, rew, done, wgt, gamma_n, B, loss, dq, state):
        check(self.lib.a0_loss_dqn(_req(q, torch.float32, B * A, "q"), _req(q_next, torch.float32, B * A, "q_next"), A, _req(act, torch.int32, B, "act"),
                                   _req(a_star, torch.int32, B, "a_star"), _req(rew, torch.float32, B, "rew"), _req(done, torch.float32, B, "done"),
                                   _req(wgt, torch.float32, B, "wgt"), gamma_n, B, _req(loss, torch.float32, B, "loss"), _req(dq, torch.float32, B * A, "dq"),
                                   _req(state, torch.int32, 8, "state"), _stream()), "a0_loss_dqn")

    def loss_mdqn(self, q, q_next, q_cur_tgt, A, act, rew, done, wgt, gamma_n, tau, lo, B, loss, dq, state):
        check(self.lib.a0_loss_mdqn(_req(q, torch.float32, B * A, "q"), _req(q_next, torch.float32, B * A, "q_next"), _req(q_cur_tgt, torch.float32, B * A, "q_cur_tgt"), A,
                                    _req(act, torch.int32, B, "act"), _req(rew, torch.float32, B, "rew"), _req(done, torch.float32, B, "done"),
                                    _req(wgt, torch.float32, B, "wgt"), gamma_n, tau, lo, B, _req(loss, torch.float32, B, "loss"), _req(dq, torch.float32, B * A, "dq"),
                                    _req(state, torch.int32, 8, "state"), _stream()), "a0_loss_mdqn")

    def loss_c51(self, logits, tgt_logits, A, T, act, a_star, rew, done, wgt, atoms, gamma_n, vmin, vmax, B, loss, dlogits, m_out, state):
        check(self.lib.a0_loss_c51(_req(logits, torch.float32, B * A * T, "logits"), _req(tgt_logits, torch.float32, B * A * T, "tgt_logits"), A, T,
                                   _req(act, torch.int32, B, "act"), _req(a_star, torch.int32, B, "a_star"), _req(rew, torch.float32, B, "rew"),
                                   _req(done, torch.float32, B, "done"), _req(wgt, torch.float32, B, "wgt"), _req(atoms, torch.float32, T, "atoms"),
                                   gamma_n, vmin, vmax, B, _req(loss, torch.float32, B, "loss"), _req(dlogits, torch.float32, B * A * T, "dlogits"),
                                   _req(m_out, torch.float32, B * T, "m_out", optional=True), _req(state, torch.int32, 8, "state"), _stream()), "a0_loss_c51")

    def quantile_target(self, q_next, sb, sj, sa, a_star, rew, done, gamma_n, B, Nd, y):
        check(self.lib.a0_quantile_target(_req(q_next, torch.float32, (B - 1) * sb + (Nd - 1) * sj + 1, "q_next"), sb, sj, sa, _req(a_star, torch.int32, B, "a_star"),
                                          _req(rew, torch.float32, B, "rew"), _req(done, torch.float32, B, "done"), gamma_n, B, Nd,
                                          _req(y, torch.float32, B * Nd, "y"), _stream()), "a0_quantile_target")

    def loss_quantile_huber(self, q, sb, si, sa, y, taus, tb, act, wgt, B, N, Nd, loss, dq, state):
        span = (B - 1) * sb + (N - 1) * si + 1
        check(self.lib.a0_loss_quantile_huber(_req(q, torch.float32, span, "q"), sb, si, sa, _req(y, torch.float32, B * Nd, "y"),
                                              _req(taus, torch.float32, (B - 1) * tb + N, "taus"), tb, _req(act, torch.int32, B, "act"),
                                              _req(wgt, torch.float32, B, "wgt"), B, N, Nd, _req(loss, torch.float32, B, "loss"),
                                              _req(dq, torch.float32, span, "dq"), _req(state, torch.int32, 8, "state"), _stream()), "a0_loss_quantile_huber")

    def cos_features(self, taus, out, R, D):
        check(self.lib.a0_cos_features(_req(taus, torch.float32, R, "taus"), _req(out, torch.float32, R * D, "out"), R, D, _stream()), "a0_cos_features")

    def tau_cos_features(self, seed, stream_id, offset, taus, out, R, D, ctrl=None, ctrl_idx=0):
        check(self.lib.a0_tau_cos_features(seed, stream_id, offset, _req(ctrl, torch.int64, 8, "ctrl", optional=True), int(ctrl_idx), _req(taus, torch.float32, R, "taus"),
                                           _req(out, torch.float32, R * D, "out"), R, D, _stream()), "a0_tau_cos_features")

    def fqf_taus_cos(self, logits, ld, taus, tau_hat, cos_out, D, B, F):
        check(self.lib.a0_fqf_taus_cos(_req(logits, torch.float32, B * ld, "logits"), ld, _req(taus, torch.float32, B * (F + 1), "taus"), _req(tau_hat, torch.float32, B * F, "tau_hat"),
                                       _req(cos_out, torch.float32, B * F * D, "cos_out"), D, B, F, _stream()), "a0_fqf_taus_cos")

    def hadamard_fwd(self, emb, feat, x, B, n, D):
        check(self.lib.a0_hadamard_fwd(_req(emb, torch.float32, B * n * D, "emb"), _req(feat, torch.float32, B * D, "feat"), _req(x, torch.float32, B * n * D, "x"), B, n, D, _stream()), "a0_hadamard_fwd")

    def hadamard_bwd(self, dx, emb, feat, demb, d3, B, n, D):
        check(self.lib.a0_hadamard_bwd(_req(dx, torch.float32, B * n * D, "dx"), _req(emb, torch.float32, B * n * D, "emb"), _req(feat, torch.float32, B * D, "feat"),
                                       _req(demb, torch.float32, B * n * D, "demb"), _req(d3, torch.float32, B * D, "d3"), B, n, D, _stream()), "a0_hadamard_bwd")

    def fqf_taus(self, logits, ld, taus, tau_hat, B, F):
        check(self.lib.a0_fqf_taus(_req(logits, torch.float32, B * ld, "logits"), ld, _req(taus, torch.float32, B * (F + 1), "taus"),
                                   _req(tau_hat, torch.float32, B * F, "tau_hat"), B, F, _stream()), "a0_fqf_taus")

    def fqf_inner_taus(self, taus, out, B, F):
        check(self.lib.a0_fqf_inner_taus(_req(taus, torch.float32, B * (F + 1), "taus"), _req(out, torch.float32, B * (F - 1), "out"), B, F, _stream()), "a0_fqf_inner_taus")

# ... 553 lines not shown
```

include/agent0_hip.h:

```cpp
#ifndef AGENT0_HIP_H
#define AGENT0_HIP_H

#include <stdint.h>

#ifdef __cplusplus
extern "C" {
#endif

#define A0_ABI_VERSION 1

#define A0_CTRL_ENV_STEP 0
#define A0_CTRL_ACTOR_STEPS 1
#define A0_CTRL_RNG_ACTION 2
#define A0_CTRL_RNG_UNIFORM 3
#define A0_CTRL_REPLAY_SLOT 4
#define A0_CTRL_RNG_TAUS 5
#define A0_CTRL_RNG_NOISE 6
#define A0_CTRL_WORDS 8

const char* a0_last_error(void);
int a0_abi_version(void);
const char* a0_build_info(void);
int a0_device_info(int* cu_count, long long* hbm_bytes, char* arch_name64);

typedef struct a0_net_desc {
    int C, H, W;
} a0_net_desc;

typedef struct a0_net a0_net;

typedef struct a0_frames_arg {
    const uint8_t* frames;
    const int* slot;
    long long sample_stride;
    int chan_off;
} a0_frames_arg;

typedef struct a0_reduce_seg { const float* slabs; long long slab_stride; int nslab; float* out; long long count; } a0_reduce_seg;
typedef struct a0_pending_reduce { a0_reduce_seg seg[4]; int n; } a0_pending_reduce;

typedef struct a0_encoder_weights {
    const float *w1, *b1, *w2, *b2, *w3, *b3;
} a0_encoder_weights;

typedef struct a0_encoder_pass {
    const float* wt; const a0_encoder_weights* w; const a0_frames_arg* f; int B;
    float *act1, *act2, *act3;
} a0_encoder_pass;

int a0_net_create(const a0_net_desc* desc, a0_net** out);
int a0_net_destroy(a0_net* net);
int a0_net_geometry(const a0_net* net, int* out8);

int a0_net_encoder_fwd(const a0_net* net, const a0_encoder_weights* w, const a0_frames_arg* frames, int B,
                       float* act1, float* act2, float* act3, void* stream);

int a0_net_encoder_fused_supported(int C, int H, int W);
long long a0_net_conv_wt_floats(int C);
int a0_net_conv_wt_refresh(const a0_encoder_weights* w, int C, float* wt, void* stream);
int a0_net_conv_wt_refresh_sync(const a0_encoder_weights* w, int C, float* wt, float* wt_target, const int* state, void* stream);
int a0_net_encoder_fwd_fused(int C, int H, int W, const float* wt, const a0_encoder_weights* w, const a0_frames_arg* frames, int B,
                             float* act1, float* act2, float* act3, void* stream);
int a0_net_encoder_fwd_fused_multi(int C, int H, int W, int n, const a0_encoder_pass* pass, void* stream);

int a0_net_encoder_dgrad_fused_supported(int C, int H, int W);
int a0_net_encoder_dgrad_fused(int C, int H, int W, const float* wt, const float* d3, const float* act1, const float* act2, int B, float* d2,
                               float* d1, void* stream);

long long a0_net_encoder_bwd_scratch(const a0_net* net, int B);
int a0_net_encoder_bwd(const a0_net* net, const a0_encoder_weights* w, const a0_frames_arg* frames, int B,
                       const float* act1, const float* act2, const float* d3, float* d2, float* d1,
                       float* g1, float* g2, float* g3, float* slabs, void* stream);

int a0_net_encoder_wgrad(const a0_net* net, const a0_encoder_weights* w, const a0_frames_arg* frames, int B, const float* act1, const float* act2,
                         const float* d3, const float* d2, const float* d1, float* g1, float* g2, float* g3, float* slabs, const a0_pending_reduce* pend,
                         void* stream);

long long a0_dense_fwd_scratch(int R, int N, int K);
int a0_dense_fwd(const float* X, int ldx, const float* W, const float* b, float* Y, int R, int N, int K, int relu,
                 float* scratch, void* stream);
int a0_dense_fwd_splits(int R, int N, int K);
int a0_dense_fwd_n(const float* X, int ldx, const float* W, const float* b, float* Y, int R, int N, int K, int relu, int splits, float* scratch, void* stream);
int a0_dense_dgrad(const float* dY, const float* W, const float* act_mask, float* dX, int R, int N, int K, void* stream);
int a0_dense_dgrad_wgrad_ok(int R, int N, int K);
int a0_dense_dgrad_wgrad_ok2(int R, int N, int K);
int a0_dense_dgrad_wgrad(const float* dY, const float* W, const float* X, int ldx, float* dX, float* grad_w_b, int R, int N, int K, void* stream);
int a0_dense_dgrad_wgrad2_ok(int R, int N, int K, int N2, int K2);
int a0_dense_dgrad_wgrad2(const float* dY, const float* W, const float* X, int ldx, float* dX, float* grad, int R, int N, int K,
                          const float* dY2, const float* X2, int ldx2, float* grad2, int N2, int K2, void* stream);
long long a0_dense_wgrad_scratch(int R, int N, int K);
int a0_dense_wgrad(const float* dY, const float* X, int ldx, float* grad_w_b, int R, int N, int K, float* slabs, void* stream);
int a0_dense_wgrad_multi(int n, const float* const* dY, const float* const* X, const int* ldx, float* const* grad_w_b, const int* R, const int* N, const int* K,
                         float* slabs, const long long* slab_off, a0_pending_reduce* pend, void* stream);

int a0_dense_fwd_mul(const float* X, int ldx, const float* W, const float* b, const float* M, int group, float* Y, int R, int N, int K, int relu, void* stream);

int a0_dense_fwd_mul_keep_ok(int R, int N, int K, int ldx);
int a0_dense_fwd_mul_keep(const float* X, int ldx, const float* W, const float* b, const float* M, int group, float* E, float* Y, int R, int N, int K, int relu, void* stream);

int a0_dense_fwd_partial_slabs(int R, int N, int K);
int a0_dense_fwd_partial(const float* X, int ldx, const float* W, int R, int N, int K, float* slabs, void* stream);
int a0_dense_fwd_partial_n(const float* X, int ldx, const float* W, int R, int N, int K, int splits, float* slabs, void* stream);
int a0_dense_fwd_partial_multi_ok(int n, int R, int N, int K);
int a0_dense_fwd_partial_multi_slabs(int n, int R, int N, int K);
int a0_dense_fwd_partial_multi(int n, const float* const* X, int ldx, const float* const* W, int R, int N, int K, float* const* slabs, const long long* slab_stride,
                               void* stream);
int a0_reduce_bias_act_multi(int n, const float* const* slabs, const long long* slab_stride, const int* nslab, const float* const* bias, float* const* out,
                             const int* rows, int N, int relu, void* stream);

int a0_probe_begin(int tag, int max_launches);
int a0_probe_end(double* host_out3);

int a0_trace_enabled(void);
int a0_trace_rank(int rank);
int a0_trace_push(const char* name);
int a0_trace_pop(void);

long long a0_weight_planes_words(int N, int K);
int a0_split_planes(const float* W, unsigned int* planes, int N, int K, void* stream);
int a0_dense_fwd_wplanes_ok(int R, int N, int K);
int a0_dense_fwd_wplanes(const float* X, int ldx, const unsigned int* Wplanes, const float* b, float* Y, int R, int N, int K, int relu, void* stream);

int a0_gemm_mode(int mode);

int a0_x9_products(int n);

int a0_dueling_fwd(const float* raw, int ld, float* q, int R, int A, int T, int dueling, void* stream);
int a0_dueling_bwd(const float* dq, float* draw, int ld, int R, int A, int T, int dueling, void* stream);

int a0_select_action(const float* x, long long sb, long long sa, long long st, int B, int A, int T, int mode,
                     const float* aux, int* a_star, float* qsel, float* qmax, void* stream);
int a0_actor_dist_tail(const float* slabs, long long slab_stride, int nslab, const float* bias, int ld, int A, int T, int dueling, int mode,
                       const float* atoms, int E, unsigned long long seed, unsigned int stream_a, unsigned int stream_u, unsigned long long off_a,
                       unsigned long long off_u, float eps, const long long* ctrl, const float* eps_ptr, int* action, float* qmax, void* stream);
int a0_actor_quantile_tail(const float* slabs, long long slab_stride, int nslab, const float* bias, int ld, int A, int T, int dueling, int mode,
                           const float* taus, int E, unsigned long long seed, unsigned int stream_a, unsigned int stream_u, unsigned long long off_a,
                           unsigned long long off_u, float eps, const long long* ctrl, const float* eps_ptr, int* action, float* qmax, void* stream);
int a0_actor_dist_tail_env_step(const float* slabs, long long slab_stride, int nslab, const float* bias, int ld, int A, int T, int dueling, int mode,
                                const float* atoms, int E, unsigned long long seed, unsigned int stream_a, unsigned int stream_u, unsigned long long off_a,
                                unsigned long long off_u, float eps, const long long* ctrl, const float* eps_ptr, int* action, float* qmax,
                                unsigned long long env_seed, unsigned int rank, unsigned int g, const uint8_t* obs_in, uint8_t* obs_out, float* ep_ret,
                                float* final_mask, float* final_ret, int n, long long steps, double gamma, int* ring_act, float* ring_rew, float* ring_done,
                                const uint8_t* obs0, uint8_t* frames, long long cap, long long start_slot, int* r_act, float* r_rew, float* r_done, int task, void* stream);

int a0_actor_quantile_tail_env_step(const float* slabs, long long slab_stride, int nslab, const float* bias, int ld, int A, int T, int dueling, int mode,
                                    const float* taus, int E, unsigned long long seed, unsigned int stream_a, unsigned int stream_u, unsigned long long off_a,
                                    unsigned long long off_u, float eps, const long long* ctrl, const float* eps_ptr, int* action, float* qmax,
                                    unsigned long long env_seed, unsigned int rank, unsigned int g, const uint8_t* obs_in, uint8_t* obs_out, float* ep_ret,
                                    float* final_mask, float* final_ret, int n, long long steps, double gamma, int* ring_act, float* ring_rew, float* ring_done,
                                    const uint8_t* obs0, uint8_t* frames, long long cap, long long start_slot, int* r_act, float* r_rew, float* r_done, int task, void* stream);

int a0_loss_dqn(const float* q, const float* q_next, int A, const int* act, const int* a_star, const float* rew,
                const float* done, const float* wgt, float gamma_n, int B, float* loss, float* dq, int* nan_flag, void* stream);
int a0_dqn_head_loss(const float* h_on, const float* h_tg, const float* h_sel, const float* W_on, const float* b_on, const float* W_tg,
                     const float* b_tg, int A, int dueling, int ld, const int* act, const float* rew, const float* done, const float* wgt,
                     float gamma_n, int B, float* loss, float* q_on_out, float* q_tg_out, float* draw, int* nan_flag, void* stream);
int a0_dqn_head_loss_slabs(const float* slabs_on, const float* slabs_tg, const float* slabs_sel, long long slab_stride, int nslab, const float* b1_on,
                           const float* b1_tg, float* h_on_out, const float* W_on, const float* b_on, const float* W_tg, const float* b_tg, int A,
                           int dueling, int ld, const int* act, const float* rew, const float* done, const float* wgt, float gamma_n, int B, float* loss,
                           float* q_on_out, float* q_tg_out, float* draw, int* nan_flag, float* dh_out, void* stream);

int a0_loss_mdqn(const float* q, const float* q_next, const float* q_cur_tgt, int A, const int* act, const float* rew, const float* done,
                 const float* wgt, float gamma_n, float tau, float lo, int B, float* loss, float* dq, int* nan_flag, void* stream);
int a0_mdqn_head_loss_slabs(const float* slabs_on, const float* slabs_tg, const float* slabs_cur, long long slab_stride, int nslab, const float* b1_on,
                            const float* b1_tg, float* h_on_out, const float* W_on, const float* b_on, const float* W_tg, const float* b_tg, int A,
                            int dueling, int ld, const int* act, const float* rew, const float* done, const float* wgt, float gamma_n, float tau, float lo,
                            int B, float* loss, float* q_on_out, float* q_tg_out, float* q_cur_out, float* draw, int* nan_flag, float* dh_out, void* stream);
int a0_c51_head_loss_slabs(const float* slabs_on, long long stride_on, int nslab_on, int rows_on, const float* slabs_tg, long long stride_tg, int nslab_tg,
                           int sel_off, const float* bias_on, const float* bias_tg, int ld, int A, int T, int dueling, const int* act, const float* rew,
                           const float* done, const float* wgt, const float* atoms, float gamma_n, float vmin, float vmax, int B, float* loss, float* draw,
                           float* q_on_out, float* q_tg_out, float* m_out, int* a_star_out, int* nan_flag, void* stream);
int a0_qr_head_loss_slabs(const float* slabs_on, long long stride_on, int nslab_on, int rows_on, const float* slabs_tg, long long stride_tg, int nslab_tg,
                          int sel_off, const float* bias_on, const float* bias_tg, int ld, int A, int T, int dueling, const int* act, const float* rew,
                          const float* done, const float* wgt, const float* taus, float gamma_n, int B, float* loss, float* draw, float* q_on_out,
                          float* q_tg_out, int* a_star_out, int* nan_flag, void* stream);
int a0_loss_c51(const float* logits, const float* tgt_logits, int A, int T, const int* act, const int* a_star,
                const float* rew, const float* done, const float* wgt, const float* atoms, float gamma_n,
                float vmin, float vmax, int B, float* loss, float* dlogits, float* m_out, int* nan_flag, void* stream);
int a0_quantile_target(const float* q_next, long long sb, long long sj, long long sa, const int* a_star, const float* rew,
                       const float* done, float gamma_n, int B, int Nd, float* y, void* stream);
int a0_loss_quantile_huber(const float* q, long long sb, long long si, long long sa, const float* y, const float* taus,
                           long long tb, const int* act, const float* wgt, int B, int N, int Nd, float* loss, float* dq,
                           int* nan_flag, void* stream);

int a0_cos_features(const float* taus, float* out, long long R, int D, void* stream);
int a0_tau_cos_features(unsigned long long seed, unsigned int stream, unsigned long long offset, const long long* ctrl, int ctrl_idx, float* taus, float* out,
                        long long R, int D, void* stream_h);
int a0_hadamard_fwd(const float* emb, const float* feat, float* x, int B, int n, int D, void* stream);
int a0_hadamard_bwd(const float* dx, const float* emb, const float* feat, float* demb, float* d3, int B, int n, int D, void* stream);
int a0_dense_dgrad_hadamard_ok(int R, int N, int K, int n);
int a0_dense_dgrad_hadamard(const float* dY, const float* W, const float* emb, const float* feat, float* demb, float* d3, int R, int N, int K, int n, void* stream);
int a0_fqf_taus(const float* logits, int ld, float* taus, float* tau_hat, int B, int F, void* stream);
int a0_fqf_taus_cos(const float* logits, int ld, float* taus, float* tau_hat, float* cos_out, int D, int B, int F, void* stream);
int a0_fqf_inner_taus(const float* taus, float* out, int B, int F, void* stream);
int a0_fqf_fraction_loss(const float* q, const float* qh, const float* taus, const int* act, const float* wgt, int B, int F, int A,
                         int ldl, float* loss, float* dlogits, const float* logits, void* stream);

int a0_adam_step(float* params, const float* grads, float* exp_avg, float* exp_avg_sq, long long n, int* state,
                 float* scalars2, double lr, double beta1, double beta2, double eps, int target_update_freq, void* stream);
int a0_adam_step_sync(float* params, const float* grads, float* exp_avg, float* exp_avg_sq, long long n, int* state, float* scalars2, double lr,
                      double beta1, double beta2, double eps, int target_update_freq, float* target, long long n_total, const float* extra_nan_flag,
                      void* stream);
int a0_adam_step_sync_wt(float* params, const float* grads, float* exp_avg, float* exp_avg_sq, long long n, int* state, float* scalars2, double lr,
                         double beta1, double beta2, double eps, int target_update_freq, float* target, long long n_total, const float* extra_nan_flag,
                         const a0_encoder_weights* w, int C, float* wt, float* wt_target, const float* loss, int loss_n, float* loss_ring, int ring_cap, void* stream);
#define A0_ALGO_DQN 0
#define A0_ALGO_C51 1
#define A0_ALGO_QR 4
#define A0_ALGO_MDQN 5
#define A0_ALGO_FQF 3
#define A0_ALGO_IQN 2
typedef struct a0_learner a0_learner;
typedef struct a0_learner_desc {
    int A, dueling, double_q;
    int B, n_step;
    double discount, lr, adam_eps;
    int target_update_freq;
    int algo;
    int num_atoms; double vmin, vmax;
    int noisy;
    unsigned long long seed;
    int iqn_K, iqn_N, iqn_N_dash;
    int fqf_F;
    double mdqn_tau, mdqn_lo;
    double max_grad_norm;
} a0_learner_desc;
int a0_learner_create(const a0_learner_desc* desc, a0_learner** out);
typedef struct a0_learner_buffers {
    float *online, *target, *grads, *adam_m, *adam_v;
// ... 194 lines not shown
```

Before: 2.337 million.

## Fuse conv1 weight-gradient into encoder data-gradient kernel, skipping d1 round-trip

Adds a combined kernel that computes the conv2 data gradient and feeds the resulting d1 tile, split into three bf16 terms, straight into LDS for the conv1 weight-gradient MFMA. The d1 tensor never goes to global memory and one kernel launch disappears. The learner now calls the fused path when supported, then runs conv2/conv3 weight gradients separately, reusing the precomputed conv1 slabs. It adds LDS pressure and aliased shared-memory regions, plus a deferred-emit variant of the conv stage.

```diff
diff --git a/agent0_amd/csrc/conv1_wgrad.h b/agent0_amd/csrc/conv1_wgrad.h
--- /dev/null
+++ b/agent0_amd/csrc/conv1_wgrad.h
@@ -0,0 +1,90 @@
+#pragma once
+#include "a0_internal.h"
+
+#include <cstdint>
+
+typedef __bf16 a0w_bf16x8 __attribute__((ext_vector_type(8)));
+typedef uint32_t a0w_u32x4 __attribute__((ext_vector_type(4)));
+typedef float a0w_acc4 __attribute__((ext_vector_type(4)));
+
+constexpr int A0W_THREADS = 512;
+constexpr int A0W_XP_ROW = 24, A0W_XP_PLANE = 21 * 24;
+constexpr int A0W_XP_ELEMS = 64 * A0W_XP_PLANE;
+constexpr int A0W_GROUPS = 60;
+constexpr int A0W_STEPS = 15;
+constexpr int A0W_NDW = 4 * 84 * 21, A0W_TR = (A0W_NDW + A0W_THREADS - 1) / A0W_THREADS;
+constexpr int A0W_SLAB = 32 * 256 + 32;
+
+A0_D uint32_t a0w_trunc(float f) { return __float_as_uint(f) >> 16; }
+A0_D float a0w_up(uint32_t h) { return __uint_as_float(h << 16); }
+
+A0_D void a0w_taps(int wave, int r16, int (&bbase)[2], int (&bshift)[2]) {
+#pragma unroll
+    for (int t = 0; t < 2; ++t) {
+        const int k = (2 * wave + t) * 16 + r16;
+        const int c = k >> 6, kh = (k >> 3) & 7, kw = k & 7;
+        const int plane = (c * 4 + (kh & 3)) * 4 + (kw & 3);
+        bbase[t] = plane * A0W_XP_PLANE + (kh >> 2) * A0W_XP_ROW;
+        bshift[t] = 2 * (kw >> 2);
+    }
+}
+
+A0_D void a0w_load_pixels(uint32_t (&w)[A0W_TR], const uint8_t* frames, const int* slot, long long sample_stride, int chan_off, int b, int tid) {
+    const long long s = slot ? (long long)slot[b] : (long long)b;
+    const uint32_t* src = (const uint32_t*)(frames + s * sample_stride + chan_off);
+#pragma unroll
+    for (int j = 0; j < A0W_TR; ++j) { const int i = tid + j * A0W_THREADS; w[j] = src[i < A0W_NDW ? i : A0W_NDW - 1]; }
+}
+
+A0_D void a0w_stage_planes(uint16_t* Xp, const uint32_t (&w)[A0W_TR], int tid) {
+#pragma unroll
+    for (int j = 0; j < A0W_TR; ++j) {
+        int i = tid + j * A0W_THREADS;
+        i = i < A0W_NDW ? i : A0W_NDW - 1;
+        const int c = i / (84 * 21), rem = i - c * (84 * 21), y = rem / 21, xc = rem - y * 21;
+        uint16_t* d = Xp + ((c * 4 + (y & 3)) * 4) * A0W_XP_PLANE + (y >> 2) * A0W_XP_ROW + xc;
+        d[0 * A0W_XP_PLANE] = (uint16_t)(__float_as_uint((float)(w[j] & 0xffu)) >> 16);
+        d[1 * A0W_XP_PLANE] = (uint16_t)(__float_as_uint((float)((w[j] >> 8) & 0xffu)) >> 16);
+        d[2 * A0W_XP_PLANE] = (uint16_t)(__float_as_uint((float)((w[j] >> 16) & 0xffu)) >> 16);
+        d[3 * A0W_XP_PLANE] = (uint16_t)(__float_as_uint((float)(w[j] >> 24)) >> 16);
+    }
+}
+
+A0_D void a0w_mfma_step(a0w_acc4 (&acc)[2][2], const a0w_u32x4 (&a)[2][3], const uint16_t* bp0, const uint16_t* bp1, const int (&bshift)[2]) {
+    a0w_u32x4 bf[2];
+#pragma unroll
+    for (int t = 0; t < 2; ++t) {
+        const uint16_t* bp = t == 0 ? bp0 : bp1;
+        const uint4 lo = *(const uint4*)bp;
+        const uint32_t hi = *(const uint32_t*)(bp + 8);
+        const int sh = bshift[t];
+        bf[t] = a0w_u32x4{__builtin_amdgcn_alignbyte(lo.y, lo.x, sh), __builtin_amdgcn_alignbyte(lo.z, lo.y, sh),
+                          __builtin_amdgcn_alignbyte(lo.w, lo.z, sh), __builtin_amdgcn_alignbyte(hi, lo.w, sh)};
+    }
+#pragma unroll
+    for (int s3 = 0; s3 < 3; ++s3)
+#pragma unroll
+        for (int i = 0; i < 2; ++i)
+#pragma unroll
+            for (int t = 0; t < 2; ++t)
+                acc[i][t] = __builtin_amdgcn_mfma_f32_16x16x32_bf16(__builtin_bit_cast(a0w_bf16x8, a[i][s3]), __builtin_bit_cast(a0w_bf16x8, bf[t]), acc[i][t], 0, 0, 0);
+}
+
+A0_D int a0w_slab_index(int i, int t, int r, int wave, int q, int r16) { return (i * 16 + 4 * q + r) * 256 + (2 * wave + t) * 16 + r16; }
+
+A0_D void a0w_write_slab(float* out, const a0w_acc4 (&acc)[2][2], float bsum, float* red, int tid, int wave, int q, int r16) {
+#pragma unroll
+    for (int i = 0; i < 2; ++i)
+#pragma unroll
+        for (int t = 0; t < 2; ++t)
+#pragma unroll
+            for (int r = 0; r < 4; ++r) out[a0w_slab_index(i, t, r, wave, q, r16)] = acc[i][t][r] / 255.0f;
+    red[tid] = bsum;
+    __syncthreads();
+    if (tid < 32) {
+        float s = 0.f;
+#pragma unroll
+        for (int j = 0; j < A0W_THREADS / 32; ++j) s += red[j * 32 + tid];
+        out[32 * 256 + tid] = s;
+    }
+}
diff --git a/agent0_amd/csrc/conv1_wgrad.hip b/agent0_amd/csrc/conv1_wgrad.hip
--- a/agent0_amd/csrc/conv1_wgrad.hip
+++ b/agent0_amd/csrc/conv1_wgrad.hip
@@ -1,17 +1,6 @@
-#include "a0_internal.h"
+#include "conv1_wgrad.h"
 
-#include <cstdint>
-
-typedef __bf16 a0w_bf16x8 __attribute__((ext_vector_type(8)));
-typedef uint32_t a0w_u32x4 __attribute__((ext_vector_type(4)));
-typedef float a0w_acc4 __attribute__((ext_vector_type(4)));
-
-constexpr int A0W_THREADS = 512;
-constexpr int A0W_XP_ROW = 24, A0W_XP_PLANE = 21 * 24;
-constexpr int A0W_XP_ELEMS = 64 * A0W_XP_PLANE;
 constexpr int A0W_T_PITCH = 488, A0W_T_TERM = 32 * A0W_T_PITCH;
-constexpr int A0W_GROUPS = 60;
-constexpr int A0W_STEPS = 15;
 
 struct a0_c1w_args {
     const uint8_t* frames; const int* slot; long long sample_stride; int chan_off;
@@ -19,9 +8,6 @@
     float* slabs;
     int B;
 };
-
-A0_D uint32_t a0w_trunc(float f) { return __float_as_uint(f) >> 16; }
-A0_D float a0w_up(uint32_t h) { return __uint_as_float(h << 16); }
 
 __global__ __launch_bounds__(A0W_THREADS) void a0_conv1_wgrad_fused_kernel(a0_c1w_args P) {
     extern __shared__ __attribute__((aligned(16))) unsigned char smem[];
@@ -32,14 +18,7 @@
     const int q = lane >> 4, r16 = lane & 15;
     for (int i = tid; i < (A0W_XP_ELEMS + 3 * A0W_T_TERM) / 2; i += A0W_THREADS) ((uint32_t*)smem)[i] = 0u;
     int bbase[2], bshift[2];
-#pragma unroll
-    for (int t = 0; t < 2; ++t) {
-        const int k = (2 * wave + t) * 16 + r16;
-        const int c = k >> 6, kh = (k >> 3) & 7, kw = k & 7;
-        const int plane = (c * 4 + (kh & 3)) * 4 + (kw & 3);
-        bbase[t] = plane * A0W_XP_PLANE + (kh >> 2) * A0W_XP_ROW;
-        bshift[t] = 2 * (kw >> 2);
-    }
+    a0w_taps(wave, r16, bbase, bshift);
     a0w_acc4 acc[2][2];
 #pragma unroll
     for (int i = 0; i < 2; ++i)
@@ -47,15 +26,11 @@
         for (int t = 0; t < 2; ++t) acc[i][t] = a0w_acc4{0.f, 0.f, 0.f, 0.f};
     float bsum = 0.f;
     __syncthreads();
-    constexpr int NDW = 4 * 84 * 21, TR = (NDW + A0W_THREADS - 1) / A0W_THREADS;
     constexpr int GT = (A0W_GROUPS + A0W_THREADS / 32 - 1) / (A0W_THREADS / 32);
-    uint32_t w[TR];
+    uint32_t w[A0W_TR];
     float v[GT][8];
     auto load_raw = [&](int b) {
-        const long long s = P.slot ? (long long)P.slot[b] : (long long)b;
-        const uint32_t* src = (const uint32_t*)(P.frames + s * P.sample_stride + P.chan_off);
-#pragma unroll
-        for (int j = 0; j < TR; ++j) { const int i = tid + j * A0W_THREADS; w[j] = src[i < NDW ? i : NDW - 1]; }
+        a0w_load_pixels(w, P.frames, P.slot, P.sample_stride, P.chan_off, b, tid);
         const float* g = P.d1 + (long long)b * 400 * 32 + (tid & 31);
 #pragma unroll
         for (int t = 0; t < GT; ++t) {
@@ -68,17 +43,7 @@
     };
     load_raw(blockIdx.x);
     for (int b = blockIdx.x; b < P.B; b += gridDim.x) {
-#pragma unroll
-        for (int j = 0; j < TR; ++j) {
-            int i = tid + j * A0W_THREADS;
-            i = i < NDW ? i : NDW - 1;
-            const int c = i / (84 * 21), rem = i - c * (84 * 21), y = rem / 21, xc = rem - y * 21;
-            uint16_t* d = Xp + ((c * 4 + (y & 3)) * 4) * A0W_XP_PLANE + (y >> 2) * A0W_XP_ROW + xc;
-            d[0 * A0W_XP_PLANE] = (uint16_t)(__float_as_uint((float)(w[j] & 0xffu)) >> 16);
-            d[1 * A0W_XP_PLANE] = (uint16_t)(__float_as_uint((float)((w[j] >> 8) & 0xffu)) >> 16);
-            d[2 * A0W_XP_PLANE] = (uint16_t)(__float_as_uint((float)((w[j] >> 16) & 0xffu)) >> 16);
-            d[3 * A0W_XP_PLANE] = (uint16_t)(__float_as_uint((float)(w[j] >> 24)) >> 16);
-        }
+        a0w_stage_planes(Xp, w, tid);
         {
             const int n = tid & 31;
 #pragma unroll
@@ -116,7 +81,7 @@
             const uint16_t* bp1 = Xp + bbase[1] + 8 * q;
 #pragma unroll 3
             for (int st = 0; st < A0W_STEPS; ++st) {
-                a0w_u32x4 a[2][3], bf[2];
+                a0w_u32x4 a[2][3];
 #pragma unroll
                 for (int i = 0; i < 2; ++i)
 #pragma unroll
@@ -124,44 +89,12 @@
                         const uint4 x = *(const uint4*)(ap + s3 * A0W_T_TERM + i * 16 * A0W_T_PITCH + 32 * st);
                         a[i][s3] = a0w_u32x4{x.x, x.y, x.z, x.w};
                     }
-#pragma unroll
-                for (int t = 0; t < 2; ++t) {
-                    const uint16_t* bp = (t == 0 ? bp0 : bp1) + 32 * st;
-                    const uint4 lo = *(const uint4*)bp;
-                    const uint32_t hi = *(const uint32_t*)(bp + 8);
-                    const int sh = bshift[t];
-                    bf[t] = a0w_u32x4{__builtin_amdgcn_alignbyte(lo.y, lo.x, sh), __builtin_amdgcn_alignbyte(lo.z, lo.y, sh),
-                                      __builtin_amdgcn_alignbyte(lo.w, lo.z, sh), __builtin_amdgcn_alignbyte(hi, lo.w, sh)};
-                }
-#pragma unroll
-                for (int s3 = 0; s3 < 3; ++s3)
-#pragma unroll
-                    for (int i = 0; i < 2; ++i)
-#pragma unroll
-                        for (int t = 0; t < 2; ++t)
-                            acc[i][t] = __builtin_amdgcn_mfma_f32_16x16x32_bf16(__builtin_bit_cast(a0w_bf16x8, a[i][s3]), __builtin_bit_cast(a0w_bf16x8, bf[t]), acc[i][t], 0, 0, 0);
+                a0w_mfma_step(acc, a, bp0 + 32 * st, bp1 + 32 * st, bshift);
             }
         }
         __syncthreads();
     }
-    float* out = P.slabs + (long long)blockIdx.x * (32 * 256 + 32);
-#pragma unroll
-    for (int i = 0; i < 2; ++i)
-#pragma unroll
-        for (int t = 0; t < 2; ++t) {
-            const int k = (2 * wave + t) * 16 + r16;
-#pragma unroll
-            for (int r = 0; r < 4; ++r) out[(i * 16 + 4 * q + r) * 256 + k] = acc[i][t][r] / 255.0f;
-        }
-    float* red = (float*)smem;
-    red[tid] = bsum;
-    __syncthreads();
-    if (tid < 32) {
-        float s = 0.f;
-#pragma unroll
-        for (int j = 0; j < A0W_THREADS / 32; ++j) s += red[j * 32 + tid];
-        out[32 * 256 + tid] = s;
-    }
+    a0w_write_slab(P.slabs + (long long)blockIdx.x * A0W_SLAB, acc, bsum, (float*)smem, tid, wave, q, r16);
 }
 
 int a0_conv1_wgrad_fused_launch(const a0_frames_arg* f, int C, int H, int W, int B, const float* d1, float* slabs, hipStream_t st) {
diff --git a/agent0_amd/csrc/encoder_fused.hip b/agent0_amd/csrc/encoder_fused.hip
--- a/agent0_amd/csrc/encoder_fused.hip
+++ b/agent0_amd/csrc/encoder_fused.hip
@@ -1,4 +1,5 @@
 #include "a0_internal.h"
+#include "conv1_wgrad.h"
 #include "net_tables.h"
 #include "operands.h"
 
@@ -503,7 +504,7 @@
     }
     __syncthreads();
 }
-template <int ORD, int N, int WN, int MBT, int R, int LR, class AFX, class EPI, class Between>
+template <int ORD, int N, int WN, int MBT, int R, int LR, bool DEFER = false, class AFX, class EPI, class Between>
 A0_D void a0_conv_stage_x9k(const AFX& af, int M, a0_wring9<N, WN, R, A0_FUSED_WAVES / WN>& ring, const EPI& epi, float* xch0, float* xch1, Between&& between) {
     constexpr int WK = A0_FUSED_WAVES / WN, HB0 = (MBT + 1) / 2, HB1 = MBT / 2;
     static_assert(WK == 2 && N == 16 * WN && HB1 >= 1 && EPI::TR && LR >= 1 && LR <= 16, "tile shape");
@@ -599,6 +600,14 @@
                 if (i < HB1 - 1) acc[mb] += x1[wn * P1 + i * 64 + lane];
                 else if (r16 < LR) acc[mb] += x1[wn * P1 + (HB1 - 1) * 64 + last];
             }
+            if (!DEFER && mb < MB && m < M) epi.emit_n4(m, n0, acc[mb], EPI::PER_ELEM ? pe[EPI::PER_ELEM ? i : 0] : nullptr);
+        }
+    };
+    auto emit = [&](auto mine) {
+        constexpr int H = decltype(mine)::value;
+#pragma unroll
+        for (int i = 0; i < (H == 0 ? HB0 : HB1); ++i) {
+            const int mb = H * HB0 + i, m = mb * 16 + r16;
             if (mb < MB && m < M) epi.emit_n4(m, n0, acc[mb], EPI::PER_ELEM ? pe[EPI::PER_ELEM ? i : 0] : nullptr);
         }
     };
@@ -608,6 +617,10 @@
     if (wk == 0) recv(std::integral_constant<int, 0>{});
     else recv(std::integral_constant<int, 1>{});
     __syncthreads();
+    if constexpr (DEFER) {
+        if (wk == 0) emit(std::integral_constant<int, 0>{});
+        else emit(std::integral_constant<int, 1>{});
+    }
 }
 constexpr int A0_P1X = 40, A0_P2X = 80;
 #ifndef A0_PADS
@@ -1319,6 +1332,193 @@
     }
 }
 
+constexpr int A0C_TP = 248;
+constexpr int A0C_TERM = 32 * A0C_TP, A0C_HALF = 3 * A0C_TERM;
+constexpr int A0C_TE = 0, A0C_TO = A0C_TE + 2 * A0C_HALF, A0C_XP = A0C_TO + 2 * A0C_HALF;
+constexpr int A0C_DG_BYTES = 3 * (A0_DTERMA + A0_DTERMB) * 2 + (4 * 4 + 4 * 3) * 1024;
+constexpr int A0C_LDS_BYTES = A0C_XP + 2 * A0W_XP_ELEMS + 16;
+static_assert(A0C_TO <= 3 * A0_DTERMA * 2, "Te is written while d2pad and the exchange regions are live: it must fit in the d3pad planes");
+static_assert(A0C_XP + 2 * A0W_XP_ELEMS >= A0C_DG_BYTES, "the zero bytes behind Xp lie beyond everything the data-gradient stages write");
+static_assert(A0C_LDS_BYTES <= 160 * 1024, "LDS per CU");
+static_assert(A0C_TO % 16 == 0 && A0C_XP % 16 == 0 && (2 * A0C_TP) % 32 == 16 && A0C_TP >= 240, "16-byte fragments, odd 16-byte channel pitch");
+static_assert(A0W_THREADS == A0_FUSED_THREADS, "one thread layout for both phases");
+struct EpiBwdPairT {
+    static constexpr bool PER_ELEM = true;
+    static constexpr bool ROW4 = false;
+    static constexpr bool TR = true;
+    const float* mask; int p0; uint16_t* T;
+    A0_D unsigned gi(int m, int n0) const {
+        const int p = p0 + (n0 >> 5), oh = m / 10, ow = m - oh * 10;
+        return (unsigned)(((oh * 2 + (p >> 1)) * 20 + ow * 2 + (p & 1)) * 32 + (n0 & 31));
+    }
+    A0_D float pre_col(int) const { return 0.f; }
+    A0_D a0_f4 pre_elem4(int m, int n0) const { return *(const a0_f4*)(mask + gi(m, n0)); }
+    A0_D void emit_n4(int m, int n0, const a0_acc4& acc, const float* pre) const {
+        float v[4];
+#pragma unroll
+        for (int r = 0; r < 4; ++r) v[r] = pre[r] > 0.f ? acc[r] : 0.f;
+        const int oh = m / 10, ow = 2 * (m - oh * 10) + ((p0 + (n0 >> 5)) & 1);
+        uint16_t* d = T + (n0 & 31) * A0C_TP + 24 * oh + ow;
+#pragma unroll
+        for (int r = 0; r < 4; ++r) {
+            const uint32_t h = a0w_trunc(v[r]);
+            const float r1 = v[r] - a0w_up(h);
+            const uint32_t md = a0w_trunc(r1);
+            d[r * A0C_TP] = (uint16_t)h;
+            d[r * A0C_TP + A0C_TERM] = (uint16_t)md;
+            d[r * A0C_TP + 2 * A0C_TERM] = (uint16_t)a0w_trunc(r1 - a0w_up(md));
+            if (ow == 19) {
+#pragma unroll
+                for (int s3 = 0; s3 < 3; ++s3) *(uint2*)(d + r * A0C_TP + s3 * A0C_TERM + 1) = uint2{0u, 0u};
+            }
+        }
+    }
+};
+struct a0_dgrad_c1w_args {
+    a0_dgrad_args g;
+    const uint8_t* frames;
+    const int* slot; int sample_stride;
+    float* slabs;
+};
+
+A0_D int a0c_tid() { int t = threadIdx.x; asm volatile("" : "+v"(t)); return t; }
+
+template <int ORD>
+__global__ __launch_bounds__(A0_FUSED_THREADS) void a0_encoder_dgrad_c1w_kernel(a0_dgrad_c1w_args A) {
+    extern __shared__ __attribute__((aligned(16))) unsigned char smem[];
+    const a0_dgrad_args& P = A.g;
+    uint16_t* plA = (uint16_t*)smem;
+    uint16_t* plB = plA + 3 * A0_DTERMA;
+    uint16_t* const Tl = (uint16_t*)(smem + A0C_TE);
+    uint16_t* const Xp = (uint16_t*)(smem + A0C_XP);
+    float* const xch0 = (float*)(smem + 3 * (A0_DTERMA + A0_DTERMB) * 2);
+    float* const xch1 = xch0 + 4 * 4 * 256;
+    const int tid = threadIdx.x, lane = tid & 63, wave = __builtin_amdgcn_readfirstlane(tid >> 6), wn = wave & 3, wk = wave >> 2;
+    const int q = lane >> 4, r16 = lane & 15;
+    if (tid < 4) ((uint32_t*)(Xp + A0W_XP_ELEMS))[tid] = 0u;
+    a0_wring9<64, 4, 3, 2> ring3;
+    a0_wring9<64, 4, 2, 2> ringq[2];
+    ring3.init(P.wd3, 576);
+    ring3.prologue();
+    const uint4* const wq = (const uint4*)P.wd2 + (((wn & 1) * 16 + (lane & 15)) * 4 + (lane >> 4)) * 3 + (wn >> 1) * 3072 + wk * 384;
+    a0w_acc4 acc[2][2];
+    float bsum = 0.f;
+    uint32_t px[A0W_TR];
+    float* const slab = A.slabs + (long long)blockIdx.x * A0W_SLAB;
+    __syncthreads();
+    for (int b = blockIdx.x; b < P.B; b += gridDim.x) {
+        for (int i = threadIdx.x; i < (121 + 40) * 16; i += A0_FUSED_THREADS) {
+            const int pos = i >> 4, c4 = (i & 15) * 4;
+            uint2 hi{0u, 0u}, mid{0u, 0u}, lo{0u, 0u};
+            uint16_t* d;
+            int term;
+            if (pos < 121) {
+                const int h = pos / 11, w = pos - h * 11;
+                d = plA + h * A0_RPDA + w * A0_P2X + c4;
+                term = A0_DTERMA;
+                if (h >= 2 && h < 9 && w >= 2 && w < 9) {
+                    const a0_f4 v = *(const a0_f4*)(P.d3 + (long long)b * 49 * 64 + ((h - 2) * 7 + (w - 2)) * 64 + c4);
+                    const float x[4] = {v.x, v.y, v.z, v.w};
+                    a0_split4(x, hi, mid, lo);
+                }
+            } else {
+                const int e = pos - 121;
+                const int h = e < 11 ? 0 : e < 22 ? 10 : e < 31 ? e - 21 : e - 30, w = e < 11 ? e : e < 22 ? e - 11 : e < 31 ? 0 : 10;
+                d = plB + h * A0_RPDB + w * A0_P2X + c4;
+                term = A0_DTERMB;
+            }
+            *(uint2*)(d) = hi; *(uint2*)(d + term) = mid; *(uint2*)(d + 2 * term) = lo;
+        }
+        __syncthreads();
+        const AFD3X f3{plA};
+        const AFD2X f2{plB};
+        const EpiBwd3X e3{P.act2 + (long long)b * 81 * 64, P.d2 + (long long)b * 81 * 64, plB};
+        const EpiBwdPairT e2a{P.act1 + (long long)b * 400 * 32, 0, Tl};
+        const EpiBwdPairT e2b{P.act1 + (long long)b * 400 * 32, 2, Tl + A0C_HALF};
+        a0_conv_stage_x9k<ORD, 64, 4, 6, 3, 1>(f3, 81, ring3, e3, xch0, xch1, [&] { ringq[0].init_at(wq, 4, 768); ringq[0].prologue(); });
+        a0_conv_stage_x9k<ORD, 64, 4, 7, 2, 4>(f2, 100, ringq[0], e2a, xch0, xch1, [&] { ringq[1].init_at(wq + 2 * 3072, 4, 768); ringq[1].prologue(); });
+        a0_conv_stage_x9k<ORD, 64, 4, 7, 2, 4, true>(f2, 100, ringq[1], e2b, xch0, xch1, [&] {
+            ring3.prologue();
+            const int lt = a0c_tid(), ll = lt & 63;
+            a0w_load_pixels(px, A.frames, A.slot, A.sample_stride, 0, b, lt);
+#pragma unroll
+            for (int i = 0; i < 2; ++i)
+#pragma unroll
+                for (int t = 0; t < 2; ++t)
+#pragma unroll
+                    for (int r = 0; r < 4; ++r) acc[i][t][r] = b == (int)blockIdx.x ? 0.f : slab[a0w_slab_index(i, t, r, wave, ll >> 4, ll & 15)];
+        });
+        a0w_stage_planes(Xp, px, a0c_tid());
+#pragma unroll
+        for (int j = 0; j < (64 * 21 + A0_FUSED_THREADS - 1) / A0_FUSED_THREADS; ++j) {
+            const int i = a0c_tid() + j * A0_FUSED_THREADS;
+            if (i < 64 * 21) {
+                uint16_t* d = Xp + i * A0W_XP_ROW + 21;
+                d[0] = 0; *(uint32_t*)(d + 1) = 0u;
+            }
+        }
+        __syncthreads();
+        const int lt = a0c_tid(), ll = lt & 63, lq = ll >> 4, lr = ll & 15;
+        {
+            const int n = lt & 31;
+#pragma unroll
+            for (int t = 0; t < 4; ++t) {
+                const int G = (lt >> 5) + t * (A0W_THREADS / 32);
+                if (G < A0W_GROUPS) {
+                    const int oh1 = G / 3;
+                    const uint16_t* s = Tl + (oh1 & 1) * A0C_HALF + n * A0C_TP + 24 * (oh1 >> 1) + 8 * (G - 3 * oh1);
+                    const uint4 h = *(const uint4*)s, md = *(const uint4*)(s + A0C_TERM), l = *(const uint4*)(s + 2 * A0C_TERM);
+                    const uint32_t hw[4] = {h.x, h.y, h.z, h.w}, mw[4] = {md.x, md.y, md.z, md.w}, lw[4] = {l.x, l.y, l.z, l.w};
+#pragma unroll
+                    for (int e = 0; e < 8; ++e) {
+                        const int sh = (e & 1) ? 0 : 16;
+                        bsum += (__uint_as_float((hw[e >> 1] << sh) & 0xffff0000u) + __uint_as_float((mw[e >> 1] << sh) & 0xffff0000u)) +
+                                __uint_as_float((lw[e >> 1] << sh) & 0xffff0000u);
+                    }
+                }
+            }
+        }
+        {
+            int bbase[2], bshift[2];
+            a0w_taps(wave, lr, bbase, bshift);
+            int aoff[3];
+#pragma unroll
+            for (int u = 0; u < 3; ++u) {
+                const int j = 4 * u + lq, r = j / 3;
+                aoff[u] = (r & 1) * A0C_HALF + lr * A0C_TP + 24 * (r >> 1) + 8 * (j - 3 * r);
+            }
+            const uint16_t* bp0 = Xp + bbase[0] + 8 * lq;
+            const uint16_t* bp1 = Xp + bbase[1] + 8 * lq;
+#pragma unroll 1
+            for (int kk = 0; kk < A0W_STEPS / 3; ++kk) {
+#pragma unroll
+                for (int u = 0; u < 3; ++u) {
+                    const int st = 3 * kk + u;
+                    a0w_u32x4 a[2][3];
+#pragma unroll
+                    for (int i = 0; i < 2; ++i)
+#pragma unroll
+                        for (int s3 = 0; s3 < 3; ++s3) {
+                            const uint4 x = *(const uint4*)(Tl + aoff[u] + s3 * A0C_TERM + i * 16 * A0C_TP + 48 * kk);
+                            a[i][s3] = a0w_u32x4{x.x, x.y, x.z, x.w};
+                        }
+                    a0w_mfma_step(acc, a, bp0 + 32 * st, bp1 + 32 * st, bshift);
+                }
+            }
+        }
+        if (b + (int)gridDim.x < P.B) {
+#pragma unroll
+            for (int i = 0; i < 2; ++i)
+#pragma unroll
+                for (int t = 0; t < 2; ++t)
+#pragma unroll
+                    for (int r = 0; r < 4; ++r) slab[a0w_slab_index(i, t, r, wave, lq, lr)] = acc[i][t][r];
+        }
+        __syncthreads();
+    }
+    a0w_write_slab(slab, acc, bsum, (float*)smem, tid, wave, q, r16);
+}
+
 A0_HD uint32_t a0_bf16_trunc(float f) { return __float_as_uint(f) >> 16; }
 A0_HD float a0_bf16_up(uint32_t h) { return __uint_as_float(h << 16); }
 __global__ void a0_conv_wt_kernel(const float* __restrict__ w1, const float* __restrict__ w2, const float* __restrict__ w3, float* __restrict__ wt, int K1,
@@ -1575,3 +1775,34 @@
     return A0_OK;
     A0_CATCH
 }
+
+extern "C" int a0_net_encoder_dgrad_c1w_supported(int C, int H, int W, const a0_frames_arg* f) {
+    return (C == 4 && H == 84 && W == 84 && f && f->frames && f->sample_stride <= 0x7fffffff && !(f->sample_stride & 3) && !(f->chan_off & 3) &&
+            !(((uintptr_t)f->frames) & 3)) ? 1 : 0;
+}
+
+extern "C" int a0_net_encoder_dgrad_c1w(int C, int H, int W, const float* wt, const float* d3, const float* act1, const float* act2, const a0_frames_arg* f,
+                                        int B, float* d2, float* c1_slabs, void* stream) {
+    A0_TRY
+    if (!wt || !d3 || !act1 || !act2 || !f || !d2 || !c1_slabs || B < 1) return a0_fail(A0_EINVAL, "a0_net_encoder_dgrad_c1w: bad argument");
+    if (!a0_net_encoder_dgrad_c1w_supported(C, H, W, f)) return a0_fail(A0_EINVAL, "a0_net_encoder_dgrad_c1w: 84x84x4 observations, 4-byte aligned, only");
+    a0_dgrad_c1w_args A;
+    A.g.d3 = d3; A.g.act1 = act1; A.g.act2 = act2; A.g.d2 = d2; A.g.d1 = nullptr; A.g.B = B;
+    A.g.wd3 = wt + 48LL * C * 64 + 64LL * 512 + 64LL * 576 + 64LL * 576 + 4LL * 32 * 256 + 96LL * 512 + 96LL * 576;
+    A.g.wd2 = A.g.wd3 + 96LL * 576;
+    A.frames = f->frames + f->chan_off; A.slot = f->slot; A.sample_stride = (int)f->sample_stride; A.slabs = c1_slabs;
+    const size_t lds = A0C_LDS_BYTES;
+    static bool configured[2] = {false, false};
+    const int six = a0_x9_products_now() == 6;
+    auto fn = six ? a0_encoder_dgrad_c1w_kernel<2> : a0_encoder_dgrad_c1w_kernel<4>;
+    if (!configured[six]) {
+        A0_HIP_THROW(hipFuncSetAttribute((const void*)fn, hipFuncAttributeMaxDynamicSharedMemorySize, (int)lds));
+        configured[six] = true;
+    }
+    const int gridx = B > 256 ? 256 : B;
+    A0_LAUNCH_PROBED(A0_TAG_ENCODER_DGRAD_FUSED, 2.0 * (81.0 * 64 * 576 + 400.0 * 32 * 256 + 400.0 * 32 * 256) * B, fn, dim3(gridx), dim3(A0_FUSED_THREADS), lds,
+                     (hipStream_t)stream, A);
+    A0_HIP_THROW(hipGetLastError());
+    return A0_OK;
+    A0_CATCH
+}
diff --git a/agent0_amd/csrc/learner.hip b/agent0_amd/csrc/learner.hip
--- a/agent0_amd/csrc/learner.hip
+++ b/agent0_amd/csrc/learner.hip
@@ -587,9 +587,17 @@
             A0_CHECK(a0_dp_allreduce(L->dp_comm, L->grads + conv_end, L->n_pad + 1 - conv_end, L->dp_side));
         }
     }
-    A0_CHECK(a0_net_encoder_dgrad_fused(L->C, L->H, L->W, L->wt_on, L->d3, L->act1, L->act2, B, L->d2, L->d1, stream));
-    A0_CHECK(a0_net_encoder_wgrad(L->net, &w_on, &f_obs, B, L->act1, L->act2, L->d3, L->d2, L->d1, L->grads + L->conv1.off, L->grads + L->conv2.off, L->grads + L->conv3.off,
-                                  L->slabs + L->enc_slab_off, &pend, stream));
+    if (a0_net_encoder_dgrad_c1w_supported(L->C, L->H, L->W, &f_obs)) {
+        float* enc_slabs = L->slabs + L->enc_slab_off;
+        A0_CHECK(a0_net_encoder_dgrad_c1w(L->C, L->H, L->W, L->wt_on, L->d3, L->act1, L->act2, &f_obs, B, L->d2,
+                                          enc_slabs + a0_net_encoder_conv1_slab_offset(L->net, B), stream));
+        A0_CHECK(a0_net_encoder_wgrad23(L->net, &w_on, B, L->act1, L->act2, L->d3, L->d2, L->grads + L->conv1.off, L->grads + L->conv2.off, L->grads + L->conv3.off,
+                                        enc_slabs, &pend, stream));
+    } else {
+        A0_CHECK(a0_net_encoder_dgrad_fused(L->C, L->H, L->W, L->wt_on, L->d3, L->act1, L->act2, B, L->d2, L->d1, stream));
+        A0_CHECK(a0_net_encoder_wgrad(L->net, &w_on, &f_obs, B, L->act1, L->act2, L->d3, L->d2, L->d1, L->grads + L->conv1.off, L->grads + L->conv2.off, L->grads + L->conv3.off,
+                                      L->slabs + L->enc_slab_off, &pend, stream));
+    }
     if (dp) {
         if (dp_inline) {
             A0_CHECK(a0_dp_allreduce(L->dp_comm, L->grads, conv_end, stream));
diff --git a/agent0_amd/csrc/net.hip b/agent0_amd/csrc/net.hip
--- a/agent0_amd/csrc/net.hip
+++ b/agent0_amd/csrc/net.hip
@@ -817,6 +817,21 @@
     A0_CATCH
 }
 
+extern "C" long long a0_net_encoder_conv1_slab_offset(const a0_net* n, int B) { return n && B >= 1 ? a0_encoder_slab_plan(n->core, B).off[0] : -1; }
+
+extern "C" int a0_net_encoder_wgrad23(const a0_net* n, const a0_encoder_weights* w, int B, const float* act1, const float* act2, const float* d3, const float* d2,
+                                      float* g1, float* g2, float* g3, float* slabs, const a0_pending_reduce* pend, void* stream) {
+    A0_TRY
+    if (!n || !w || !act1 || !act2 || !d3 || !d2 || !g1 || !g2 || !g3 || !slabs || B < 1) return a0_fail(A0_EINVAL, "a0_net_encoder_wgrad23: null argument");
+    if (n->core.C != 4 || n->core.H != 84 || n->core.W != 84) return a0_fail(A0_EINVAL, "a0_net_encoder_wgrad23: 84x84x4 observations only (a0_net_encoder_dgrad_c1w)");
+    if (pend && (pend->n < 0 || pend->n > 4)) return a0_fail(A0_EINVAL, "a0_net_encoder_wgrad23: bad pending reductions");
+    a0_hip_backend bk{(hipStream_t)stream};
+    const a0_frames_arg none{nullptr, nullptr, 0, 0};
+    a0_encoder_bwd_impl(bk, n->core, *w, none, B, act1, act2, d3, const_cast<float*>(d2), nullptr, g1, g2, g3, slabs, false, pend, B < 256 ? B : 256);
+    return A0_OK;
+    A0_CATCH
+}
+
 extern "C" long long a0_net_encoder_bwd_scratch(const a0_net* n, int B) { return n ? a0_encoder_bwd_scratch_impl(n->core, B) : 0; }
 
 extern "C" int a0_net_encoder_bwd(const a0_net* n, const a0_encoder_weights* w, const a0_frames_arg* f, int B,
diff --git a/agent0_amd/csrc/net_impl.h b/agent0_amd/csrc/net_impl.h
--- a/agent0_amd/csrc/net_impl.h
+++ b/agent0_amd/csrc/net_impl.h
@@ -246,7 +246,8 @@
 template <class BK>
 static void a0_encoder_bwd_impl(BK& bk, const a0_net_core& n, const a0_encoder_weights& w, const a0_frames_arg& f, int B,
                                 const float* act1, const float* act2, const float* d3, float* d2, float* d1,
-                                float* g1, float* g2, float* g3, float* slabs, bool with_dgrad = true, const a0_pending_reduce* pend = nullptr) {
+                                float* g1, float* g2, float* g3, float* slabs, bool with_dgrad = true, const a0_pending_reduce* pend = nullptr,
+                                int c1_slabs = 0) {
     const int M3 = B * n.H3 * n.W3, M2 = B * n.H2 * n.W2, M1 = B * n.H1 * n.W1;
     const a0_enc_slab_plan plan = a0_encoder_slab_plan(n, B);
     a0_reduce_seg segs[8];
@@ -302,7 +303,7 @@
         const long long wc = 32LL * n.K1;
         float* sl = slabs + plan.off[0];
         bk.tag = A0_TAG_CONV1_WGRAD;
-        const int fused_slabs = bk.conv1_wgrad_fused(n, f, B, d1, sl);
+        const int fused_slabs = c1_slabs > 0 ? c1_slabs : bk.conv1_wgrad_fused(n, f, B, d1, sl);
         if (fused_slabs > 0) {
             segs[nseg++] = a0_reduce_seg{sl, wc + 32, fused_slabs, g1, wc + 32};
         } else {
diff --git a/agent0_amd/ops.py b/agent0_amd/ops.py
--- a/agent0_amd/ops.py
+++ b/agent0_amd/ops.py
@@ -227,6 +227,33 @@
                                                   _req(act2, torch.float32, B * net.H2 * net.W2 * 64, "act2"), B,
                                                   _req(d2, torch.float32, B * net.H2 * net.W2 * 64, "d2"), _req(d1, torch.float32, B * net.H1 * net.W1 * 32, "d1"),
                                                   _stream()), "a0_net_encoder_dgrad_fused")
+
+    def dgrad_c1w_supported(self, net, frames, slot, sample_stride, chan_off, B) -> bool:
+        fa = self._frames(net, frames, slot, sample_stride, chan_off, B)
+        return bool(self.lib.a0_net_encoder_dgrad_c1w_supported(net.C, net.H, net.W, C.addressof(fa)))
+
+    def encoder_conv1_slab_offset(self, net, B) -> int:
+        return int(self.lib.a0_net_encoder_conv1_slab_offset(net.h, B))
+
+    def encoder_dgrad_c1w(self, net, wt, d3, act1, act2, frames, slot, sample_stride, chan_off, B, d2, slabs):
+        fa = self._frames(net, frames, slot, sample_stride, chan_off, B)
+        need = self.encoder_bwd_scratch(net, B)
+        off = self.encoder_conv1_slab_offset(net, B)
+        check(self.lib.a0_net_encoder_dgrad_c1w(net.C, net.H, net.W, _req(wt, torch.float32, self.conv_wt_floats(net.C), "wt"),
+                                                _req(d3, torch.float32, B * net.feat, "d3"), _req(act1, torch.float32, B * net.H1 * net.W1 * 32, "act1"),
+                                                _req(act2, torch.float32, B * net.H2 * net.W2 * 64, "act2"), C.addressof(fa), B,
+                                                _req(d2, torch.float32, B * net.H2 * net.W2 * 64, "d2"), _req(slabs, torch.float32, need, "slabs") + 4 * off,
+                                                _stream()), "a0_net_encoder_dgrad_c1w")
+
+    def encoder_wgrad23(self, net, w, B, act1, act2, d3, d2, g1, g2, g3, slabs, pend=None):
+        ew = self._enc_w(w)
+        need = self.encoder_bwd_scratch(net, B)
+        check(self.lib.a0_net_encoder_wgrad23(
+            net.h, C.addressof(ew), B,
+            _req(act1, torch.float32, B * net.H1 * net.W1 * 32, "act1"), _req(act2, torch.float32, B * net.H2 * net.W2 * 64, "act2"),
+            _req(d3, torch.float32, B * net.feat, "d3"), _req(d2, torch.float32, B * net.H2 * net.W2 * 64, "d2"),
+            _req(g1, torch.float32, 32 * net.K1 + 32, "g1"), _req(g2, torch.float32, 64 * net.K2 + 64, "g2"), _req(g3, torch.float32, 64 * net.K3 + 64, "g3"),
+            _req(slabs, torch.float32, need, "slabs"), None if pend is None else C.addressof(pend), _stream()), "a0_net_encoder_wgrad23")
 
     def pending_reduce(self):
         from ._abi import PendingReduce
diff --git a/include/agent0_hip.h b/include/agent0_hip.h
--- a/include/agent0_hip.h
+++ b/include/agent0_hip.h
@@ -75,6 +75,12 @@
 int a0_net_encoder_wgrad(const a0_net* net, const a0_encoder_weights* w, const a0_frames_arg* frames, int B, const float* act1, const float* act2,
                          const float* d3, const float* d2, const float* d1, float* g1, float* g2, float* g3, float* slabs, const a0_pending_reduce* pend,
                          void* stream);
+int a0_net_encoder_dgrad_c1w_supported(int C, int H, int W, const a0_frames_arg* frames);
+int a0_net_encoder_dgrad_c1w(int C, int H, int W, const float* wt, const float* d3, const float* act1, const float* act2, const a0_frames_arg* frames,
+                             int B, float* d2, float* c1_slabs, void* stream);
+long long a0_net_encoder_conv1_slab_offset(const a0_net* net, int B);
+int a0_net_encoder_wgrad23(const a0_net* net, const a0_encoder_weights* w, int B, const float* act1, const float* act2, const float* d3, const float* d2,
+                           float* g1, float* g2, float* g3, float* slabs, const a0_pending_reduce* pend, void* stream);
 
 long long a0_dense_fwd_scratch(int R, int N, int K);
 int a0_dense_fwd(const float* X, int ldx, const float* W, const float* b, float* Y, int R, int N, int K, int relu,
```

Result: no change. 2.338 million (median of 6 runs) (+0.1%).
